# SingleRust/SingleRust

Measured on AMD Instinct MI355X. Metric: cells/sec end-to-end normalise->HVG->50-PC PCA; SpMM achieved HBM GB/s vs peak, higher is better.
Workload: dtype f32

## Files before the change

### include/srx.h

```cpp
#ifndef SRX_H
#define SRX_H

#include <stddef.h>
#include <stdint.h>

#ifdef __cplusplus
extern "C" {
#endif

#define SRX_ABI_VERSION 6

typedef struct srx_ctx srx_ctx;
typedef struct srx_mat srx_mat;

typedef enum srx_status {
    SRX_OK = 0,
    SRX_E_ARG = -1,
    SRX_E_DTYPE = -2,
    SRX_E_FORMAT = -3,
    SRX_E_BOUNDS = -4,
    SRX_E_HIP = -5,
    SRX_E_RCCL = -6,
    SRX_E_OOM = -7,
    SRX_E_NAN = -8,
    SRX_E_SHAPE = -9,
    SRX_E_NOCONV = -10
} srx_status;

typedef enum srx_dtype {
    SRX_I8 = 0, SRX_I16 = 1, SRX_I32 = 2, SRX_U8 = 3, SRX_U16 = 4, SRX_U32 = 5,
    SRX_F32 = 6, SRX_F64 = 7
} srx_dtype;

typedef enum srx_direction { SRX_ROW = 0, SRX_COLUMN = 1 } srx_direction;

typedef struct srx_csr {
    uint64_t n_rows, n_cols, nnz;
    const uint64_t* indptr;
    const uint64_t* indices;
    void* values;
    int32_t dtype;
} srx_csr;

typedef enum srx_store { SRX_STORE_AUTO = 0, SRX_STORE_F32 = 1, SRX_STORE_F64 = 2 } srx_store;

int32_t srx_abi_version(void);
int32_t srx_device_count(int32_t* n_out);
int32_t srx_ctx_create(int32_t device_id, srx_ctx** out);
void    srx_ctx_destroy(srx_ctx* ctx);
int32_t srx_ctx_synchronize(srx_ctx* ctx);
const char* srx_last_error(const srx_ctx* ctx);

#define SRX_UNIQUE_ID_BYTES 128
int32_t srx_comm_unique_id(void* id_out_128);
int32_t srx_comm_init(srx_ctx* ctx, int32_t n_ranks, int32_t rank, const void* id_128);
typedef int32_t (*srx_host_allreduce_fn)(void* user, double* buf, uint64_t count);
int32_t srx_comm_init_host(srx_ctx* ctx, int32_t n_ranks, int32_t rank, srx_host_allreduce_fn fn, void* user);
int32_t srx_comm_destroy(srx_ctx* ctx);
int32_t srx_comm_info(srx_ctx* ctx, int32_t* kind_out, int32_t* n_ranks_out, int32_t* rccl_version_out,
                      int32_t* ranks_seen_out);
int32_t srx_comm_overlap_info(srx_ctx* ctx, int32_t* split_exchanges_out, int32_t* cu_masked_out);
int32_t srx_gram_mode_info(srx_ctx* ctx, int32_t* mode_out);
int32_t srx_gram_exchange_ranges(uint64_t k, uint64_t* offsets_out);
int32_t srx_partition_rows(const uint64_t* indptr, uint64_t n_rows, int32_t n_ranks,
                           uint64_t* cut_out);

int32_t srx_matrix_upload(srx_ctx* ctx, const srx_csr* host, int32_t store, srx_mat** out);
int32_t srx_matrix_upload_csc(srx_ctx* ctx, const srx_csr* host, int32_t store, srx_mat** out);
enum { SRX_FORMAT_CSR = 0, SRX_FORMAT_CSC = 1 };
int32_t srx_matrix_format(const srx_mat* m, int32_t* format_out);
int32_t srx_matrix_to_csr(srx_mat* m, srx_mat** out);
int32_t srx_matrix_to_csc(srx_mat* m, srx_mat** out);
int32_t srx_matrix_alloc(srx_ctx* ctx, uint64_t n_rows, uint64_t n_cols, uint64_t nnz,
                         int32_t dtype, int32_t store, srx_mat** out);
int32_t srx_matrix_device_ptrs(srx_mat* m, void** indptr, void** indices, void** values);
typedef struct srx_mat_info {
    uint64_t n_rows, n_cols, nnz;
    int32_t dtype;
    int32_t store;
    uint64_t row_offset;
    uint64_t n_rows_global;
} srx_mat_info;
int32_t srx_matrix_info(const srx_mat* m, srx_mat_info* out);
int32_t srx_matrix_set_shard(srx_mat* m, uint64_t row_offset);
int32_t srx_matrix_download_values(srx_mat* m, void* values_out, int32_t dtype_out);
int32_t srx_matrix_prepare(srx_mat* m);
int32_t srx_matrix_reserve_results(srx_mat* m, uint64_t n_selected, int32_t n_components);
int32_t srx_matrix_clone(srx_mat* m, srx_mat** out);
int32_t srx_matrix_copy_values(srx_mat* dst, const srx_mat* src);
void    srx_matrix_free(srx_mat* m);

int32_t srx_compute_number(srx_mat* m, int32_t direction, uint32_t* out);
int32_t srx_compute_sum(srx_mat* m, int32_t direction, double* out);
int32_t srx_compute_variance(srx_mat* m, int32_t direction, double* out);
int32_t srx_compute_std_dev(srx_mat* m, int32_t direction, double* out);
int32_t srx_compute_min_max(srx_mat* m, int32_t direction, double* min_out, double* max_out);
int32_t srx_compute_qc_variables(srx_mat* m, uint32_t* num_per_cell, uint32_t* num_per_gene, double* expr_per_gene,
                                 double* expr_per_cell, double* variance_per_gene, double* variance_per_cell,
                                 double* std_dev_per_cell, double* std_dev_per_gene);
int32_t srx_gene_moments(srx_mat* m, uint64_t* cnt, double* sum, double* sumsq);

enum { SRX_FLEX_NONE = 0, SRX_FLEX_ABSOLUTE = 1, SRX_FLEX_RELATIVE = 2 };
typedef struct srx_flex {
    int32_t kind;
    uint32_t absolute;
    double relative;
} srx_flex;
int32_t srx_filter_cells(srx_mat* m, srx_flex lower, srx_flex upper, srx_mat** out, uint8_t* mask_out);
int32_t srx_filter_genes(srx_mat* m, srx_flex lower, srx_flex upper, srx_mat** out, uint8_t* mask_out);
int32_t srx_subset(srx_mat* m, const uint8_t* row_mask, const uint8_t* col_mask, srx_mat** out);
int32_t srx_matrix_download_pattern(srx_mat* m, uint64_t* indptr_out, uint64_t* indices_out);

int32_t srx_normalize_total_inplace(srx_mat* m, double target_sum, int32_t direction);
int32_t srx_log1p_inplace(srx_mat* m);
int32_t srx_normalize_log1p_inplace(srx_mat* m, double target_sum, double* row_sums_out);

int32_t srx_select_hvg(srx_mat* m, uint64_t n, uint64_t* idx_out, uint64_t* n_out);

typedef enum srx_pca_solver {
    SRX_SOLVER_AUTO = 0,
    SRX_SOLVER_GRAM = 1,
    SRX_SOLVER_SPMM = 2
} srx_pca_solver;

typedef struct srx_pca_opts {
    int32_t n_components;
    int32_t center;
    int32_t scale;
    int32_t n_threads;
    int32_t block;
    int32_t max_iter;
    int32_t solver;
    double  tol;
    uint64_t seed;
} srx_pca_opts;

typedef struct srx_pca_info {
    uint64_t n_cells_global;
    uint32_t k;
    uint32_t n_pc;
    uint32_t block;
    uint32_t n_iter;
    double residual;
    uint64_t nnz_selected;
    uint32_t solver;
    uint32_t reserved_;
} srx_pca_info;

int32_t srx_pca(srx_mat* m, const uint64_t* sel, uint64_t k, const srx_pca_opts* opts,
                double* scores, double* components, double* evr, double* mean, double* std_,
                srx_pca_info* info);
int32_t srx_pca_loadings(const double* components, const double* std_, const uint64_t* sel,
                         uint64_t k, uint64_t n_pc, uint64_t n_vars, double* out);

typedef struct srx_pca_model srx_pca_model;
int32_t srx_pca_model_from_result(srx_mat* m, srx_pca_model** out);
int32_t srx_pca_model_create(srx_ctx* ctx, uint64_t k, uint64_t n_pc, const double* components, const double* mean,
                             const double* std_, const uint64_t* sel, int32_t center, int32_t scale, srx_pca_model** out);
int32_t srx_pca_model_info(const srx_pca_model* p, uint64_t* k_out, uint64_t* n_pc_out, uint64_t* sel_out);
void    srx_pca_model_free(srx_pca_model* p);
int32_t srx_pca_transform(srx_pca_model* p, srx_mat* q, const uint64_t* feat, double target_sum, int32_t transform,
                          double* scores_out);

#define SRX_KNN_MAX_DIMS 128
typedef struct srx_knn_opts {
    int32_t k;
    int32_t n_dims;
    int32_t include_self;
    int32_t reserved_;
} srx_knn_opts;
typedef struct srx_knn_info {
    uint64_t n_ref, n_query;
    uint32_t d, k;
    uint32_t n_candidates;
    uint32_t reserved_;
    uint64_t rows_certified;
    uint64_t rows_recomputed;
} srx_knn_info;
int32_t srx_knn_result(srx_mat* m, const srx_knn_opts* opts, uint32_t* indices_out, double* distances_out,
                       srx_knn_info* info);
int32_t srx_knn_points(srx_ctx* ctx, const double* ref, uint64_t n_ref, const double* query, uint64_t n_query,
                       uint64_t d, const srx_knn_opts* opts, uint32_t* indices_out, double* distances_out,
                       srx_knn_info* info);

typedef struct srx_graph srx_graph;
typedef struct srx_graph_info {
    uint64_t n;
    uint32_t k, reserved_;
    uint64_t nnz_distances, nnz_connectivities;
    uint64_t n_mutual;
    uint64_t rows_no_root, rows_clamped, rows_all_zero;
    uint64_t entries_dropped;
    uint64_t max_row_nnz;
} srx_graph_info;
int32_t srx_neighbors_result(srx_mat* m, const srx_knn_opts* opts, srx_knn_info* knn_info, srx_graph** out);
int32_t srx_neighbors_from_knn(srx_ctx* ctx, const uint32_t* indices, const double* distances, uint64_t n, uint32_t k,
                               srx_graph** out);
int32_t srx_graph_info_get(const srx_graph* g, srx_graph_info* info);
enum { SRX_GRAPH_DISTANCES = 0, SRX_GRAPH_CONNECTIVITIES = 1 };
int32_t srx_graph_fetch(srx_graph* g, int32_t which, uint64_t* indptr, uint32_t* indices, double* data);
int32_t srx_graph_fetch_scales(srx_graph* g, double* rho, double* sigma);
void    srx_graph_free(srx_graph* g);

int32_t srx_spmm(srx_mat* m, const uint64_t* sel, uint64_t k, const double* panel, double* y_out,
                 double* t_out, double* gram_out);

typedef struct srx_pipeline_result {
    srx_pca_info pca;
    double ms_normalize, ms_moments, ms_select, ms_compact, ms_pca;
} srx_pipeline_result;
int32_t srx_pipeline(srx_mat* m, double target_sum, uint64_t n_hvg, const srx_pca_opts* opts,
                     srx_pipeline_result* res);
int32_t srx_result_fetch(srx_mat* m, double* scores, double* components, double* evr,
                         double* mean, double* std_, uint64_t* hvg_idx);

typedef struct srx_backed srx_backed;
enum { SRX_BACKED_NORMALIZE = 1, SRX_BACKED_LOG1P = 2 };
int32_t srx_backed_create(srx_ctx* ctx, uint64_t n_cols, int32_t store, srx_backed** out);
void    srx_backed_destroy(srx_backed* b);
int32_t srx_backed_stats_tile(srx_backed* b, const srx_csr* tile, double target_sum, int32_t transform,
                              uint32_t* row_number_out, double* row_sum_out);
int32_t srx_backed_moments(srx_backed* b, uint64_t* cnt, double* sum, double* sumsq, uint64_t* n_rows_global);
int32_t srx_backed_select(srx_backed* b, uint64_t n_hvg, const uint64_t* sel, uint64_t n_sel,
                          const srx_pca_opts* opts, uint64_t* sel_out, uint64_t* n_out);
int32_t srx_backed_gram_tile(srx_backed* b, const srx_csr* tile, double target_sum, int32_t transform);
int32_t srx_backed_solve(srx_backed* b, srx_pca_info* info);
int32_t srx_backed_fetch(srx_backed* b, double* scores, double* components, double* evr, double* mean,
                         double* std_, uint64_t* sel);

typedef enum srx_kernel_class {
    SRX_K_NORMALIZE = 0,
    SRX_K_MOMENTS = 1,
    SRX_K_COMPACT = 2,
    SRX_K_SPMM_FWD = 3,
    SRX_K_SPMM_T = 4,
    SRX_K_GRAM = 5,
    SRX_K_DENSE = 6,
    SRX_K_ROWSUM = 7,
    SRX_K_ITERATE = 8,
    SRX_K_SELECT = 9,
    SRX_K_BUCKET = 10,
    SRX_K_KNN = 11,
    SRX_K_GRAPH = 12,
    SRX_K_COUNT_ = 13
} srx_kernel_class;
int32_t srx_prof_enable(srx_ctx* ctx, uint32_t class_mask);
int32_t srx_prof_reset(srx_ctx* ctx);
int32_t srx_prof_get(srx_ctx* ctx, int32_t kernel_class, double* total_ms, uint64_t* launches,
                     double* algorithmic_bytes);
int32_t srx_prof_get_aux(srx_ctx* ctx, int32_t kernel_class, double* aux_bytes);

#ifdef __cplusplus
}
#endif
#endif
```

### rust/srx_sys.rs

```rust
#![allow(non_camel_case_types, dead_code)]
use std::os::raw::{c_char, c_void};

pub const SRX_ABI_VERSION: i32 = 6;
pub const SRX_UNIQUE_ID_BYTES: usize = 128;
pub const SRX_KNN_MAX_DIMS: i32 = 128;
pub const SRX_OK: i32 = 0;
pub const SRX_E_ARG: i32 = -1;
pub const SRX_E_DTYPE: i32 = -2;
pub const SRX_E_FORMAT: i32 = -3;
pub const SRX_E_BOUNDS: i32 = -4;
pub const SRX_E_HIP: i32 = -5;
pub const SRX_E_RCCL: i32 = -6;
pub const SRX_E_OOM: i32 = -7;
pub const SRX_E_NAN: i32 = -8;
pub const SRX_E_SHAPE: i32 = -9;
pub const SRX_E_NOCONV: i32 = -10;
pub const SRX_I8: i32 = 0;
pub const SRX_I16: i32 = 1;
pub const SRX_I32: i32 = 2;
pub const SRX_U8: i32 = 3;
pub const SRX_U16: i32 = 4;
pub const SRX_U32: i32 = 5;
pub const SRX_F32: i32 = 6;
pub const SRX_F64: i32 = 7;
// ... 101 lines not shown
    pub k: i32,
    pub n_dims: i32,
    pub include_self: i32,
    pub reserved: i32,
}

#[repr(C)]
#[derive(Clone, Copy)]
pub struct SrxKnnInfo {
    pub n_ref: u64,
    pub n_query: u64,
    pub d: u32,
    pub k: u32,
    pub n_candidates: u32,
    pub reserved: u32,
    pub rows_certified: u64,
    pub rows_recomputed: u64,
}

#[repr(C)]
#[derive(Clone, Copy)]
pub struct SrxGraphInfo {
    pub n: u64,
    pub k: u32,
    pub reserved: u32,
    pub nnz_distances: u64,
    pub nnz_connectivities: u64,
    pub n_mutual: u64,
    pub rows_no_root: u64,
    pub rows_clamped: u64,
    pub rows_all_zero: u64,
    pub entries_dropped: u64,
    pub max_row_nnz: u64,
}

#[repr(C)]
#[derive(Clone, Copy)]
pub struct SrxPipelineResult {
    pub pca: SrxPcaInfo,
    pub ms_normalize: f64,
    pub ms_moments: f64,
    pub ms_select: f64,
    pub ms_compact: f64,
    pub ms_pca: f64,
}

pub type SrxHostAllreduceFn = extern "C" fn(user: *mut c_void, buf: *mut f64, count: u64) -> i32;

#[link(name = "srx_hip")]
extern "C" {
    pub fn srx_abi_version() -> i32;
    pub fn srx_device_count(n_out: *mut i32) -> i32;
    pub fn srx_ctx_create(device_id: i32, out: *mut *mut SrxCtx) -> i32;
    pub fn srx_ctx_destroy(ctx: *mut SrxCtx);
    pub fn srx_ctx_synchronize(ctx: *mut SrxCtx) -> i32;
    pub fn srx_last_error(ctx: *const SrxCtx) -> *const c_char;
    pub fn srx_comm_unique_id(id_out_128: *mut c_void) -> i32;
    pub fn srx_comm_init(ctx: *mut SrxCtx, n_ranks: i32, rank: i32, id_128: *const c_void) -> i32;
    pub fn srx_comm_init_host(ctx: *mut SrxCtx, n_ranks: i32, rank: i32, fn_: SrxHostAllreduceFn, user: *mut c_void) -> i32;
    pub fn srx_comm_destroy(ctx: *mut SrxCtx) -> i32;
    pub fn srx_comm_info(ctx: *mut SrxCtx, kind_out: *mut i32, n_ranks_out: *mut i32, rccl_version_out: *mut i32,
                         ranks_seen_out: *mut i32) -> i32;
    pub fn srx_comm_overlap_info(ctx: *mut SrxCtx, split_exchanges_out: *mut i32, cu_masked_out: *mut i32) -> i32;
    pub fn srx_gram_mode_info(ctx: *mut SrxCtx, mode_out: *mut i32) -> i32;
    pub fn srx_gram_exchange_ranges(k: u64, offsets_out: *mut u64) -> i32;
    pub fn srx_partition_rows(indptr: *const u64, n_rows: u64, n_ranks: i32, cut_out: *mut u64) -> i32;
    pub fn srx_matrix_upload(ctx: *mut SrxCtx, host: *const SrxCsr, store: i32, out: *mut *mut SrxMat) -> i32;
    pub fn srx_matrix_upload_csc(ctx: *mut SrxCtx, host: *const SrxCsr, store: i32, out: *mut *mut SrxMat) -> i32;
    pub fn srx_matrix_format(m: *const SrxMat, format_out: *mut i32) -> i32;
    pub fn srx_matrix_to_csr(m: *mut SrxMat, out: *mut *mut SrxMat) -> i32;
    pub fn srx_matrix_to_csc(m: *mut SrxMat, out: *mut *mut SrxMat) -> i32;
    pub fn srx_matrix_alloc(ctx: *mut SrxCtx, n_rows: u64, n_cols: u64, nnz: u64, dtype: i32, store: i32,
                            out: *mut *mut SrxMat) -> i32;
    pub fn srx_matrix_device_ptrs(m: *mut SrxMat, indptr: *mut *mut c_void, indices: *mut *mut c_void,
                                  values: *mut *mut c_void) -> i32;
    pub fn srx_matrix_info(m: *const SrxMat, out: *mut SrxMatInfo) -> i32;
    pub fn srx_matrix_set_shard(m: *mut SrxMat, row_offset: u64) -> i32;
    pub fn srx_matrix_download_values(m: *mut SrxMat, values_out: *mut c_void, dtype_out: i32) -> i32;
    pub fn srx_matrix_prepare(m: *mut SrxMat) -> i32;
    pub fn srx_matrix_reserve_results(m: *mut SrxMat, n_selected: u64, n_components: i32) -> i32;
    pub fn srx_matrix_clone(m: *mut SrxMat, out: *mut *mut SrxMat) -> i32;
    pub fn srx_matrix_copy_values(dst: *mut SrxMat, src: *const SrxMat) -> i32;
    pub fn srx_matrix_free(m: *mut SrxMat);
    pub fn srx_compute_number(m: *mut SrxMat, direction: i32, out: *mut u32) -> i32;
    pub fn srx_compute_sum(m: *mut SrxMat, direction: i32, out: *mut f64) -> i32;
    pub fn srx_compute_variance(m: *mut SrxMat, direction: i32, out: *mut f64) -> i32;
    pub fn srx_compute_std_dev(m: *mut SrxMat, direction: i32, out: *mut f64) -> i32;
    pub fn srx_compute_min_max(m: *mut SrxMat, direction: i32, min_out: *mut f64, max_out: *mut f64) -> i32;
    pub fn srx_compute_qc_variables(m: *mut SrxMat, num_per_cell: *mut u32, num_per_gene: *mut u32,
                                    expr_per_gene: *mut f64, expr_per_cell: *mut f64, variance_per_gene: *mut f64,
                                    variance_per_cell: *mut f64, std_dev_per_cell: *mut f64,
                                    std_dev_per_gene: *mut f64) -> i32;
    pub fn srx_gene_moments(m: *mut SrxMat, cnt: *mut u64, sum: *mut f64, sumsq: *mut f64) -> i32;
    pub fn srx_filter_cells(m: *mut SrxMat, lower: SrxFlex, upper: SrxFlex, out: *mut *mut SrxMat, mask_out: *mut u8) -> i32;
    pub fn srx_filter_genes(m: *mut SrxMat, lower: SrxFlex, upper: SrxFlex, out: *mut *mut SrxMat, mask_out: *mut u8) -> i32;
    pub fn srx_subset(m: *mut SrxMat, row_mask: *const u8, col_mask: *const u8, out: *mut *mut SrxMat) -> i32;
    pub fn srx_matrix_download_pattern(m: *mut SrxMat, indptr_out: *mut u64, indices_out: *mut u64) -> i32;
    pub fn srx_normalize_total_inplace(m: *mut SrxMat, target_sum: f64, direction: i32) -> i32;
    pub fn srx_log1p_inplace(m: *mut SrxMat) -> i32;
    pub fn srx_normalize_log1p_inplace(m: *mut SrxMat, target_sum: f64, row_sums_out: *mut f64) -> i32;
    pub fn srx_select_hvg(m: *mut SrxMat, n: u64, idx_out: *mut u64, n_out: *mut u64) -> i32;
    pub fn srx_pca(m: *mut SrxMat, sel: *const u64, k: u64, opts: *const SrxPcaOpts, scores: *mut f64,
                   components: *mut f64, evr: *mut f64, mean: *mut f64, std: *mut f64, info: *mut SrxPcaInfo) -> i32;
    pub fn srx_pca_loadings(components: *const f64, std: *const f64, sel: *const u64, k: u64, n_pc: u64,
                            n_vars: u64, out: *mut f64) -> i32;
    pub fn srx_pca_model_from_result(m: *mut SrxMat, out: *mut *mut SrxPcaModel) -> i32;
    pub fn srx_pca_model_create(ctx: *mut SrxCtx, k: u64, n_pc: u64, components: *const f64, mean: *const f64,
                                std: *const f64, sel: *const u64, center: i32, scale: i32,
                                out: *mut *mut SrxPcaModel) -> i32;
    pub fn srx_pca_model_info(p: *const SrxPcaModel, k_out: *mut u64, n_pc_out: *mut u64, sel_out: *mut u64) -> i32;
    pub fn srx_pca_model_free(p: *mut SrxPcaModel);
    pub fn srx_pca_transform(p: *mut SrxPcaModel, q: *mut SrxMat, feat: *const u64, target_sum: f64,
                             transform: i32, scores_out: *mut f64) -> i32;
    pub fn srx_knn_result(m: *mut SrxMat, opts: *const SrxKnnOpts, indices_out: *mut u32, distances_out: *mut f64,
                          info: *mut SrxKnnInfo) -> i32;
    pub fn srx_knn_points(ctx: *mut SrxCtx, ref_: *const f64, n_ref: u64, query: *const f64, n_query: u64, d: u64,
                          opts: *const SrxKnnOpts, indices_out: *mut u32, distances_out: *mut f64,
                          info: *mut SrxKnnInfo) -> i32;
    pub fn srx_neighbors_result(m: *mut SrxMat, opts: *const SrxKnnOpts, knn_info: *mut SrxKnnInfo,
                                out: *mut *mut SrxGraph) -> i32;
    pub fn srx_neighbors_from_knn(ctx: *mut SrxCtx, indices: *const u32, distances: *const f64, n: u64, k: u32,
                                  out: *mut *mut SrxGraph) -> i32;
    pub fn srx_graph_info_get(g: *const SrxGraph, info: *mut SrxGraphInfo) -> i32;
    pub fn srx_graph_fetch(g: *mut SrxGraph, which: i32, indptr: *mut u64, indices: *mut u32, data: *mut f64) -> i32;
    pub fn srx_graph_fetch_scales(g: *mut SrxGraph, rho: *mut f64, sigma: *mut f64) -> i32;
    pub fn srx_graph_free(g: *mut SrxGraph);
    pub fn srx_spmm(m: *mut SrxMat, sel: *const u64, k: u64, panel: *const f64, y_out: *mut f64, t_out: *mut f64,
                    gram_out: *mut f64) -> i32;
    pub fn srx_pipeline(m: *mut SrxMat, target_sum: f64, n_hvg: u64, opts: *const SrxPcaOpts,
                        res: *mut SrxPipelineResult) -> i32;
    pub fn srx_result_fetch(m: *mut SrxMat, scores: *mut f64, components: *mut f64, evr: *mut f64, mean: *mut f64,
                            std: *mut f64, hvg_idx: *mut u64) -> i32;
    pub fn srx_backed_create(ctx: *mut SrxCtx, n_cols: u64, store: i32, out: *mut *mut SrxBacked) -> i32;
    pub fn srx_backed_destroy(b: *mut SrxBacked);
    pub fn srx_backed_stats_tile(b: *mut SrxBacked, tile: *const SrxCsr, target_sum: f64, transform: i32,
                                 row_number_out: *mut u32, row_sum_out: *mut f64) -> i32;
    pub fn srx_backed_moments(b: *mut SrxBacked, cnt: *mut u64, sum: *mut f64, sumsq: *mut f64,
                              n_rows_global: *mut u64) -> i32;
    pub fn srx_backed_select(b: *mut SrxBacked, n_hvg: u64, sel: *const u64, n_sel: u64, opts: *const SrxPcaOpts,
                             sel_out: *mut u64, n_out: *mut u64) -> i32;
    pub fn srx_backed_gram_tile(b: *mut SrxBacked, tile: *const SrxCsr, target_sum: f64, transform: i32) -> i32;
    pub fn srx_backed_solve(b: *mut SrxBacked, info: *mut SrxPcaInfo) -> i32;
    pub fn srx_backed_fetch(b: *mut SrxBacked, scores: *mut f64, components: *mut f64, evr: *mut f64,
                            mean: *mut f64, std: *mut f64, sel: *mut u64) -> i32;
    pub fn srx_prof_enable(ctx: *mut SrxCtx, class_mask: u32) -> i32;
    pub fn srx_prof_reset(ctx: *mut SrxCtx) -> i32;
    pub fn srx_prof_get(ctx: *mut SrxCtx, kernel_class: i32, total_ms: *mut f64, launches: *mut u64,
                        algorithmic_bytes: *mut f64) -> i32;
    pub fn srx_prof_get_aux(ctx: *mut SrxCtx, kernel_class: i32, aux_bytes: *mut f64) -> i32;
}
```

### singlerust_amd/_ffi.py

```python
from __future__ import annotations

import ctypes as C
import os

_HERE = os.path.dirname(os.path.abspath(__file__))
LIB_PATH = os.path.join(_HERE, "lib", "libsrx_hip.so")

OK, E_ARG, E_DTYPE, E_FORMAT, E_BOUNDS, E_HIP, E_RCCL, E_OOM, E_NAN, E_SHAPE, E_NOCONV = (
    0, -1, -2, -3, -4, -5, -6, -7, -8, -9, -10)
STATUS_NAMES = {0: "SRX_OK", -1: "SRX_E_ARG", -2: "SRX_E_DTYPE", -3: "SRX_E_FORMAT",
                -4: "SRX_E_BOUNDS", -5: "SRX_E_HIP", -6: "SRX_E_RCCL", -7: "SRX_E_OOM",
                -8: "SRX_E_NAN", -9: "SRX_E_SHAPE", -10: "SRX_E_NOCONV"}
I8, I16, I32, U8, U16, U32, F32, F64 = range(8)
ROW, COLUMN = 0, 1
STORE_AUTO, STORE_F32, STORE_F64 = 0, 1, 2
K_NORMALIZE, K_MOMENTS, K_COMPACT, K_SPMM_FWD, K_SPMM_T, K_GRAM, K_DENSE, K_ROWSUM, K_ITERATE, K_SELECT, K_BUCKET = range(11)
K_KNN = 11
K_GRAPH = 12
GRAPH_DISTANCES, GRAPH_CONNECTIVITIES = 0, 1
KNN_MAX_DIMS = 128
SOLVER_AUTO, SOLVER_GRAM, SOLVER_SPMM = 0, 1, 2
UNIQUE_ID_BYTES = 128


# ... 47 lines not shown
    _fields_ = [("n", C.c_uint64), ("k", C.c_uint32), ("reserved_", C.c_uint32), ("nnz_distances", C.c_uint64),
                ("nnz_connectivities", C.c_uint64), ("n_mutual", C.c_uint64), ("rows_no_root", C.c_uint64),
                ("rows_clamped", C.c_uint64), ("rows_all_zero", C.c_uint64), ("entries_dropped", C.c_uint64),
                ("max_row_nnz", C.c_uint64)]


class SynthParams(C.Structure):
    _fields_ = [("seed", C.c_uint64), ("n_rows_global", C.c_uint64), ("n_cols", C.c_uint64),
                ("density", C.c_double), ("lib_sigma", C.c_double), ("type_decay", C.c_double),
                ("n_types", C.c_uint32), ("marker_genes", C.c_uint32), ("expr_boost", C.c_uint32),
                ("value_boost", C.c_uint32), ("skew", C.c_uint32), ("reserved_", C.c_uint32)]


class Flex(C.Structure):
    _fields_ = [("kind", C.c_int32), ("absolute", C.c_uint32), ("relative", C.c_double)]


HOST_ALLREDUCE_FN = C.CFUNCTYPE(C.c_int32, C.c_void_p, C.POINTER(C.c_double), C.c_uint64)
FLEX_NONE, FLEX_ABSOLUTE, FLEX_RELATIVE = 0, 1, 2
BACKED_NORMALIZE, BACKED_LOG1P = 1, 2
P = C.c_void_p
_SIGS = {
    "srx_abi_version": (C.c_int32, []),
    "srx_device_count": (C.c_int32, [C.POINTER(C.c_int32)]),
    "srx_ctx_create": (C.c_int32, [C.c_int32, C.POINTER(P)]),
    "srx_ctx_destroy": (None, [P]),
    "srx_ctx_synchronize": (C.c_int32, [P]),
    "srx_last_error": (C.c_char_p, [P]),
    "srx_comm_unique_id": (C.c_int32, [P]),
    "srx_comm_init": (C.c_int32, [P, C.c_int32, C.c_int32, P]),
    "srx_comm_init_host": (C.c_int32, [P, C.c_int32, C.c_int32, C.c_void_p, P]),
    "srx_comm_destroy": (C.c_int32, [P]),
    "srx_comm_info": (C.c_int32, [P, C.POINTER(C.c_int32), C.POINTER(C.c_int32), C.POINTER(C.c_int32), C.POINTER(C.c_int32)]),
    "srx_comm_overlap_info": (C.c_int32, [P, C.POINTER(C.c_int32), C.POINTER(C.c_int32)]),
    "srx_gram_mode_info": (C.c_int32, [P, C.POINTER(C.c_int32)]),
    "srx_gram_exchange_ranges": (C.c_int32, [C.c_uint64, P]),
    "srx_partition_rows": (C.c_int32, [P, C.c_uint64, C.c_int32, P]),
    "srx_matrix_upload": (C.c_int32, [P, C.POINTER(Csr), C.c_int32, C.POINTER(P)]),
    "srx_matrix_upload_csc": (C.c_int32, [P, C.POINTER(Csr), C.c_int32, C.POINTER(P)]),
    "srx_matrix_format": (C.c_int32, [P, C.POINTER(C.c_int32)]),
    "srx_matrix_to_csr": (C.c_int32, [P, C.POINTER(P)]),
    "srx_matrix_to_csc": (C.c_int32, [P, C.POINTER(P)]),
    "srx_matrix_alloc": (C.c_int32, [P, C.c_uint64, C.c_uint64, C.c_uint64, C.c_int32, C.c_int32, C.POINTER(P)]),
    "srx_matrix_device_ptrs": (C.c_int32, [P, C.POINTER(P), C.POINTER(P), C.POINTER(P)]),
    "srx_matrix_info": (C.c_int32, [P, C.POINTER(MatInfo)]),
    "srx_matrix_set_shard": (C.c_int32, [P, C.c_uint64]),
    "srx_matrix_download_values": (C.c_int32, [P, P, C.c_int32]),
    "srx_matrix_prepare": (C.c_int32, [P]),
    "srx_matrix_reserve_results": (C.c_int32, [P, C.c_uint64, C.c_int32]),
    "srx_matrix_clone": (C.c_int32, [P, C.POINTER(P)]),
    "srx_matrix_copy_values": (C.c_int32, [P, P]),
    "srx_matrix_free": (None, [P]),
    "srx_compute_number": (C.c_int32, [P, C.c_int32, P]),
    "srx_compute_sum": (C.c_int32, [P, C.c_int32, P]),
    "srx_compute_variance": (C.c_int32, [P, C.c_int32, P]),
    "srx_compute_std_dev": (C.c_int32, [P, C.c_int32, P]),
    "srx_compute_min_max": (C.c_int32, [P, C.c_int32, P, P]),
    "srx_compute_qc_variables": (C.c_int32, [P, P, P, P, P, P, P, P, P]),
    "srx_filter_cells": (C.c_int32, [P, Flex, Flex, C.POINTER(C.c_void_p), P]),
    "srx_filter_genes": (C.c_int32, [P, Flex, Flex, C.POINTER(C.c_void_p), P]),
    "srx_subset": (C.c_int32, [P, P, P, C.POINTER(C.c_void_p)]),
    "srx_matrix_download_pattern": (C.c_int32, [P, P, P]),
    "srx_gene_moments": (C.c_int32, [P, P, P, P]),
    "srx_normalize_total_inplace": (C.c_int32, [P, C.c_double, C.c_int32]),
    "srx_log1p_inplace": (C.c_int32, [P]),
    "srx_normalize_log1p_inplace": (C.c_int32, [P, C.c_double, P]),
    "srx_select_hvg": (C.c_int32, [P, C.c_uint64, P, C.POINTER(C.c_uint64)]),
    "srx_pca": (C.c_int32, [P, P, C.c_uint64, C.POINTER(PcaOpts), P, P, P, P, P, C.POINTER(PcaInfo)]),
    "srx_pca_loadings": (C.c_int32, [P, P, P, C.c_uint64, C.c_uint64, C.c_uint64, P]),
    "srx_pca_model_from_result": (C.c_int32, [P, C.POINTER(P)]),
    "srx_pca_model_create": (C.c_int32, [P, C.c_uint64, C.c_uint64, P, P, P, P, C.c_int32, C.c_int32, C.POINTER(P)]),
    "srx_pca_model_info": (C.c_int32, [P, C.POINTER(C.c_uint64), C.POINTER(C.c_uint64), P]),
    "srx_pca_model_free": (None, [P]),
    "srx_pca_transform": (C.c_int32, [P, P, P, C.c_double, C.c_int32, P]),
    "srx_knn_result": (C.c_int32, [P, C.POINTER(KnnOpts), P, P, C.POINTER(KnnInfo)]),
    "srx_knn_points": (C.c_int32, [P, P, C.c_uint64, P, C.c_uint64, C.c_uint64, C.POINTER(KnnOpts), P, P, C.POINTER(KnnInfo)]),
    "srx_neighbors_result": (C.c_int32, [P, C.POINTER(KnnOpts), C.POINTER(KnnInfo), C.POINTER(P)]),
    "srx_neighbors_from_knn": (C.c_int32, [P, P, P, C.c_uint64, C.c_uint32, C.POINTER(P)]),
    "srx_graph_info_get": (C.c_int32, [P, C.POINTER(GraphInfo)]),
    "srx_graph_fetch": (C.c_int32, [P, C.c_int32, P, P, P]),
    "srx_graph_fetch_scales": (C.c_int32, [P, P, P]),
    "srx_graph_free": (None, [P]),
    "srx_spmm": (C.c_int32, [P, P, C.c_uint64, P, P, P, P]),
    "srx_pipeline": (C.c_int32, [P, C.c_double, C.c_uint64, C.POINTER(PcaOpts), C.POINTER(PipelineResult)]),
    "srx_result_fetch": (C.c_int32, [P, P, P, P, P, P, P]),
    "srx_backed_create": (C.c_int32, [P, C.c_uint64, C.c_int32, C.POINTER(P)]),
    "srx_backed_destroy": (None, [P]),
    "srx_backed_stats_tile": (C.c_int32, [P, C.POINTER(Csr), C.c_double, C.c_int32, P, P]),
    "srx_backed_moments": (C.c_int32, [P, P, P, P, C.POINTER(C.c_uint64)]),
    "srx_backed_select": (C.c_int32, [P, C.c_uint64, P, C.c_uint64, C.POINTER(PcaOpts), P, C.POINTER(C.c_uint64)]),
    "srx_backed_gram_tile": (C.c_int32, [P, C.POINTER(Csr), C.c_double, C.c_int32]),
    "srx_backed_solve": (C.c_int32, [P, C.POINTER(PcaInfo)]),
    "srx_backed_fetch": (C.c_int32, [P, P, P, P, P, P, P]),
    "srx_prof_enable": (C.c_int32, [P, C.c_uint32]),
    "srx_prof_reset": (C.c_int32, [P]),
    "srx_prof_get": (C.c_int32, [P, C.c_int32, C.POINTER(C.c_double), C.POINTER(C.c_uint64), C.POINTER(C.c_double)]),
    "srx_prof_get_aux": (C.c_int32, [P, C.c_int32, C.POINTER(C.c_double)]),
    "srx_synth_defaults": (None, [C.POINTER(SynthParams), C.c_uint64, C.c_uint64, C.c_uint64, C.c_double]),
    "srx_synth_indptr": (C.c_int32, [C.POINTER(SynthParams), C.c_uint64, C.c_uint64, P]),
    "srx_synth_fill_host": (C.c_int32, [C.POINTER(SynthParams), C.c_uint64, C.c_uint64, P, P, P]),
    "srx_synth_generate": (C.c_int32, [P, C.POINTER(SynthParams), C.c_uint64, C.c_uint64, C.c_int32, C.c_int32, C.POINTER(P)]),
}
EXPORTS = tuple(_SIGS)

_lib = None


def lib() -> C.CDLL:
    global _lib
    if _lib is None:
        if not os.path.exists(LIB_PATH):
            raise SrxError(E_HIP, f"{LIB_PATH} is missing: run `python -m singlerust_amd.build` "
                                  "(hipcc --offload-arch=gfx950); there is no CPU fallback")
        l = C.CDLL(LIB_PATH)
        for name, (res, args) in _SIGS.items():
            fn = getattr(l, name)
            fn.restype = res
            fn.argtypes = args
        _lib = l
    return _lib


def check(rc: int, ctx=None) -> None:
    if rc != OK:
        msg = lib().srx_last_error(ctx)
        raise SrxError(rc, msg.decode() if msg else "")


def ptr(a):
    return None if a is None else C.c_void_p(a.ctypes.data)
```

### singlerust_amd/csrc/common.hpp

```cpp
#pragma once

#include <hip/hip_runtime.h>

#include <cstdarg>
#include <cstdint>
#include <cstdio>
#include <cstring>
#include <map>
#include <string>
#include <utility>
#include <vector>

#include "../../include/srx.h"

struct ncclComm;

namespace srx {

constexpr int kWave = 64;

__device__ __forceinline__ int lane_id() { return threadIdx.x & (kWave - 1); }
__device__ __forceinline__ uint64_t global_wave_id() {
    return (uint64_t)blockIdx.x * (blockDim.x / kWave) + (uint32_t)__builtin_amdgcn_readfirstlane((int)(threadIdx.x / kWave));
}

template <typename T>
__device__ __forceinline__ T wave_sum(T v) {
#pragma unroll
    for (int off = kWave / 2; off > 0; off >>= 1) v += __shfl_xor(v, off, kWave);
    return v;
}
__device__ __forceinline__ void wave_lds_sync() {
    __builtin_amdgcn_fence(__ATOMIC_ACQ_REL, "wavefront");
    __builtin_amdgcn_wave_barrier();
}
template <typename T>
__device__ __forceinline__ T wave_min(T v) {
#pragma unroll
    for (int off = kWave / 2; off > 0; off >>= 1) {
        T o = __shfl_xor(v, off, kWave);
        v = o < v ? o : v;
    }
    return v;
}
template <typename T>
__device__ __forceinline__ T wave_max(T v) {
#pragma unroll
    for (int off = kWave / 2; off > 0; off >>= 1) {
        T o = __shfl_xor(v, off, kWave);
        v = o > v ? o : v;
    }
    return v;
}

struct ProfAcc {
    double ms = 0.0;
    uint64_t launches = 0;
    double bytes = 0.0, aux_bytes = 0.0;
    std::vector<std::pair<hipEvent_t, hipEvent_t>> pending;
};

}

struct srx_ctx {
    int device = 0;
    int n_cus = 256;
    hipStream_t stream = nullptr;
    hipStream_t comm_stream = nullptr;
    hipEvent_t comm_fork = nullptr, comm_join = nullptr;
    hipStream_t gram_stream = nullptr;
    bool gram_stream_masked = false;
    uint32_t* d_gram_mode = nullptr;
    int gram_mode_state = 0;
    bool gram_mode_f32 = false;
    uint32_t gram_splits = 0;
    hipEvent_t gram_fork = nullptr, gram_join = nullptr;
    std::string err;
    ncclComm* comm = nullptr;
    int n_ranks = 1, rank = 0;
    srx_host_allreduce_fn host_allreduce = nullptr;
    void* host_allreduce_user = nullptr;
    uint32_t prof_mask = 0;
    srx::ProfAcc prof[SRX_K_COUNT_];
    std::vector<hipEvent_t> event_pool;
    struct Scratch { void* p = nullptr; size_t bytes = 0; };
    std::map<std::string, Scratch> scratch;
    int pool_on = 0;
    std::vector<std::pair<void*, size_t>> pool;
    void* pinned = nullptr;
    size_t pinned_bytes = 0;
    static constexpr int kAsyncSlots = 4;
    std::map<std::string, hipGraphExec_t> graphs;
    bool graphs_off = false;
    bool capturing = false;
    double* pin_async = nullptr;
    struct UpWorker {
        hipStream_t stream = nullptr;
        void* pin[2] = {nullptr, nullptr};
        hipEvent_t ev[2] = {nullptr, nullptr};
    };
    std::vector<UpWorker> up_workers;
    hipStream_t direct_stream = nullptr;
    hipEvent_t async_ev[kAsyncSlots] = {nullptr, nullptr, nullptr, nullptr};
    hipEvent_t d2h_ev = nullptr;
    void* pin_d2h = nullptr;
    bool d2h_pending = false;
};

struct srx_pca_state {
    bool valid = false;
    uint32_t k = 0, n_pc = 0;
    int center = 1, scale = 1;
    std::vector<int> round_counts;
    double* d_scores = nullptr;
    size_t scores_cap = 0;
    std::vector<double> components;
    std::vector<double> evr, mean, std_;
    std::vector<uint64_t> sel;
    srx_pca_info info{};
    double* d_small = nullptr;
    bool host_pending = false;
};

struct srx_mat {
    srx_ctx* ctx = nullptr;
    uint64_t n_rows = 0, n_cols = 0, nnz = 0;
    int32_t dtype = SRX_F32;
    int32_t store = SRX_STORE_F32;
    bool pooled = false;
    bool store_auto = false;
    int64_t* d_indptr = nullptr;
    int32_t* d_indices = nullptr;
    void* d_values = nullptr;
    uint64_t row_offset = 0;
    int n_tiles = 0;
    int tile_genes = 0;
    int64_t* d_tile_ptr = nullptr;
    uint16_t* d_idx16 = nullptr;
    uint32_t* d_cnt_pat = nullptr;
    bool cnt_pat_valid = false;
    uint64_t version = 1;
    uint64_t moments_version = 0;
    uint64_t* d_cnt = nullptr;
    double* d_sum = nullptr;
    double* d_sq = nullptr;
    uint64_t n_rows_global = 0;
    double* d_row_sum = nullptr;
    bool csc = false;
    srx_pca_state pca;
};

namespace srx {

extern thread_local std::string g_tls_err;

inline int32_t fail(srx_ctx* ctx, int32_t code, const char* fmt, ...) {
    char buf[512];
    va_list ap;
    va_start(ap, fmt);
    vsnprintf(buf, sizeof buf, fmt, ap);
    va_end(ap);
    g_tls_err = buf;
    if (ctx) ctx->err = buf;
    return code;
}

#define SRX_HIP(ctx, expr)                                                                   \
    do {                                                                                     \
        hipError_t e__ = (expr);                                                             \
        if (e__ != hipSuccess)                                                               \
            return srx::fail((ctx), e__ == hipErrorOutOfMemory ? SRX_E_OOM : SRX_E_HIP,      \
                             "%s failed: %s (%s:%d)", #expr, hipGetErrorString(e__),         \
                             __FILE__, __LINE__);                                            \
    } while (0)

#define SRX_TRY(expr)                          \
    do {                                       \
        int32_t rc__ = (expr);                 \
        if (rc__ != SRX_OK) return rc__;       \
    } while (0)

int32_t scratch(srx_ctx* ctx, const char* name, size_t bytes, void** out);
int32_t pinned(srx_ctx* ctx, size_t bytes, void** out);
int32_t d2h(srx_ctx* ctx, void* host, const void* dev, size_t bytes);
int32_t d2h_begin(srx_ctx* ctx, const void* dev, size_t bytes);
int32_t d2h_end(srx_ctx* ctx, void* host, size_t bytes);
int32_t h2d(srx_ctx* ctx, void* dev, const void* host, size_t bytes);
int32_t d2h_rows(srx_ctx* ctx, void* host, const void* dev, uint64_t rows, size_t width, size_t dev_pitch);

struct ProfScope {
    srx_ctx* ctx;
    int cls;
    hipStream_t stream;
    hipEvent_t e0 = nullptr, e1 = nullptr;
    ProfScope(srx_ctx* c, int cls_, double alg_bytes, hipStream_t stream_ = nullptr, double aux_bytes = 0.0);
    ~ProfScope();
};

struct Range {
    bool on;
    explicit Range(const char* name);
    ~Range();
};

int32_t allreduce_f64(srx_ctx* ctx, double* d_buf, size_t count);
int32_t allreduce_f64_on(srx_ctx* ctx, double* d_buf, size_t count, hipStream_t stream);
bool comm_is_rccl(const srx_ctx* ctx);

struct RowXf {
    const double* row_sum = nullptr;
    double target = 0.0;
    bool write_back = false;
};
int32_t upload_on(srx_ctx* ctx, const srx_csr* h, int32_t store, hipStream_t stream, srx_mat** out);
int32_t tiles_from_idx16(srx_mat* m, hipStream_t stream);
inline uint64_t at_least_one(uint64_t n) { return n ? n : 1; }
hipError_t dev_malloc(srx_ctx* ctx, void** p, size_t bytes);
void pool_clear(srx_ctx* ctx);
int32_t ensure_tiles(srx_mat* m);
int32_t promote_to_f64(srx_mat* m);
int32_t ensure_pattern_counts(srx_mat* m);
int32_t ensure_moments(srx_mat* m);
int32_t moments_accumulate(srx_mat* m, double* d_acc, RowXf xf);
int32_t moments_install(srx_mat* m, double* d_packed);
int32_t ensure_moments_xf(srx_mat* m, RowXf xf, bool* stored);
void moments_adopt(srx_mat* m);
void moments_retire(srx_mat* m);
int32_t launch_row_apply(srx_mat* m, double target, hipStream_t stream);
int32_t launch_normalize(srx_mat* m, double target, bool do_norm, bool do_log, hipStream_t stream = nullptr,
                         bool precise = false, int wgs_per_cu = 0);
int32_t launch_row_sums(srx_mat* m, double* out = nullptr);
int32_t row_number(srx_mat* m, uint32_t* out);
int32_t row_stat(srx_mat* m, int which, double* out0, double* out1);
int32_t row_qc(srx_mat* m, uint32_t* num, double* sum, double* var);
int32_t scan_exclusive(srx_ctx* ctx, const int64_t* d_in, uint64_t n, int64_t* d_out, int64_t** total_dev);
inline void touch(srx_mat* m) { m->version++; m->pca.valid = false; }

inline bool is_f32(const srx_mat* m) { return m->store == SRX_STORE_F32; }
inline int32_t eff_dir(const srx_mat* m, int32_t d) { return (m->csc && (d == SRX_ROW || d == SRX_COLUMN)) ? 1 - d : d; }
int32_t transpose_device(srx_mat* m, srx_mat** out);
inline size_t val_bytes(const srx_mat* m) { return is_f32(m) ? 4 : 8; }

}
```

### singlerust_amd/csrc/ctx.hip

```cpp
#include "common.hpp"
#include <chrono>

#include <dlfcn.h>

#include <algorithm>
#include <thread>

namespace srx {

thread_local std::string g_tls_err;

int32_t scratch(srx_ctx* ctx, const char* name, size_t bytes, void** out) {
    auto& s = ctx->scratch[name];
    if (s.bytes < bytes) {
        if (s.p) SRX_HIP(ctx, hipFree(s.p));
        s.p = nullptr;
        s.bytes = 0;
        size_t want = bytes + bytes / 8 + 256;
        SRX_HIP(ctx, hipMalloc(&s.p, want));
        s.bytes = want;
    }
    *out = s.p;
    return SRX_OK;
}
// ... 185 lines not shown
        if (lo > hi || lo < 0 || (uint64_t)hi > nnz) { bad = true; continue; }
        for (int64_t p = lo + lane; p + 1 < hi; p += kWave) bad |= !(idx[p] < idx[p + 1]);
    }
    if (bad) atomicOr(flag, 2);
}

static int grid_for(uint64_t n, int block, int cap) {
    uint64_t g = (n + block - 1) / block;
    if (g < 1) g = 1;
    if (g > (uint64_t)cap) g = cap;
    return (int)g;
}

template <typename S>
static int32_t convert_chunked(srx_ctx* ctx, hipStream_t stream, const char* tmp_tag, const void* host, void* d_dst,
                               uint64_t n, bool to_f32) {
    const uint64_t chunk = 32ull << 20;
    void* d_tmp;
    SRX_TRY(scratch(ctx, tmp_tag, (n < chunk ? n : chunk) * sizeof(S) + 16, &d_tmp));
    for (uint64_t off = 0; off < n; off += chunk) {
        uint64_t cnt = n - off < chunk ? n - off : chunk;
        SRX_HIP(ctx, hipMemcpy(d_tmp, (const S*)host + off, cnt * sizeof(S), hipMemcpyHostToDevice));
        int g = grid_for(cnt, 256, 4096);
        if (to_f32)
            hipLaunchKernelGGL((k_convert_values<S, float>), dim3(g), dim3(256), 0, stream,
                               (const S*)d_tmp, (float*)d_dst + off, cnt);
        else
            hipLaunchKernelGGL((k_convert_values<S, double>), dim3(g), dim3(256), 0, stream,
                               (const S*)d_tmp, (double*)d_dst + off, cnt);
        SRX_HIP(ctx, hipStreamSynchronize(stream));
    }
    return SRX_OK;
}

constexpr size_t kPoolCapBytes = 24ull << 30;
static size_t pool_bytes(const srx_ctx* ctx) {
    size_t t = 0;
    for (auto& b : ctx->pool) t += b.second;
    return t;
}
hipError_t dev_malloc(srx_ctx* ctx, void** p, size_t bytes) {
    if (ctx->pool_on) {
        int best = -1;
        for (size_t i = 0; i < ctx->pool.size(); ++i) {
            const size_t cap = ctx->pool[i].second;
            if (cap >= bytes && cap <= bytes + bytes / 4 + (1u << 20) && (best < 0 || cap < ctx->pool[(size_t)best].second)) best = (int)i;
        }
        if (best >= 0) {
            *p = ctx->pool[(size_t)best].first;
            ctx->pool.erase(ctx->pool.begin() + best);
            return hipSuccess;
        }
    }
    const size_t want = (ctx->pool_on && bytes >= (1u << 20)) ? bytes + bytes / 32 + 65536 : bytes;
    hipError_t e = hipMalloc(p, want);
    if (e != hipSuccess && !ctx->pool.empty()) {
        (void)hipGetLastError();
        pool_clear(ctx);
        e = hipMalloc(p, want);
    }
    return e;
}
static void dev_release(srx_mat* m, void* p) {
    if (!p) return;
    srx_ctx* ctx = m->ctx;
    size_t cap = 0;
    if (m->pooled && ctx && ctx->pool_on > 0 && hipMemPtrGetInfo(p, &cap) == hipSuccess && cap > 0) {
        ctx->pool.emplace_back(p, cap);
        while (ctx->pool.size() > 1 && pool_bytes(ctx) > kPoolCapBytes) {
            (void)hipFree(ctx->pool.front().first);
            ctx->pool.erase(ctx->pool.begin());
        }
    } else {
        (void)hipFree(p);
    }
}
void pool_clear(srx_ctx* ctx) {
    for (auto& b : ctx->pool) (void)hipFree(b.first);
    ctx->pool.clear();
}

static void free_mat_buffers(srx_mat* m) {
    if (!m) return;
    dev_release(m, m->d_indptr);
    dev_release(m, m->d_indices);
    dev_release(m, m->d_values);
    dev_release(m, m->d_tile_ptr);
    dev_release(m, m->d_idx16);
    dev_release(m, m->d_cnt);
    dev_release(m, m->d_cnt_pat);
    dev_release(m, m->d_sum);
    dev_release(m, m->d_sq);
    dev_release(m, m->d_row_sum);
    (void)hipFree(m->pca.d_scores);
}

static int32_t resolve_store(int32_t dtype, int32_t store) {
    if (store == SRX_STORE_F32 || store == SRX_STORE_F64) return store;
    switch (dtype) {
        case SRX_I32: case SRX_U32: case SRX_F64: return SRX_STORE_F64;
        default: return SRX_STORE_F32;
    }
}


__global__ void k_rebase_indptr(int64_t* __restrict__ indptr, uint64_t n, int64_t base) {
    uint64_t i = (uint64_t)blockIdx.x * blockDim.x + threadIdx.x;
    if (i < n) indptr[i] -= base;
}

static const int kUpWorkers = [] {
    const char* e = getenv("SRX_UP_WORKERS");
    const int v = e ? atoi(e) : 8;
    return v < 1 ? 1 : v > 64 ? 64 : v;
}();
constexpr size_t kUpChunkBytes = 4u << 20;

static int32_t ensure_up_workers(srx_ctx* ctx) {
    if (!ctx->up_workers.empty()) return SRX_OK;
    std::vector<srx_ctx::UpWorker> ws(kUpWorkers);
    for (auto& w : ws) {
        SRX_HIP(ctx, hipStreamCreateWithFlags(&w.stream, hipStreamNonBlocking));
        for (int b = 0; b < 2; ++b) {
            SRX_HIP(ctx, hipHostMalloc(&w.pin[b], kUpChunkBytes, hipHostMallocDefault));
            SRX_HIP(ctx, hipEventCreateWithFlags(&w.ev[b], hipEventDisableTiming));
        }
    }
    ctx->up_workers = std::move(ws);
    return SRX_OK;
}

static int32_t parallel_h2d(srx_ctx* ctx, const void* src, void* dst, uint64_t n, bool narrow, size_t elem_bytes,
                            uint64_t n_cols, bool* bad) {
    if (n == 0) return SRX_OK;
    SRX_TRY(ensure_up_workers(ctx));
    const int device = ctx->device;
    const uint64_t per_chunk = kUpChunkBytes / elem_bytes;
    int nw = (int)std::min<uint64_t>(kUpWorkers, (n + per_chunk - 1) / per_chunk);
    if (nw < 1) nw = 1;
    const uint64_t share = ((n + nw - 1) / nw + 15) & ~(uint64_t)15;
    std::vector<hipError_t> err(nw, hipSuccess);
    std::vector<int> oob(nw, 0);
    auto run = [&](int t) {
        srx_ctx::UpWorker& w = ctx->up_workers[t];
        hipError_t e = hipSetDevice(device);
        const uint64_t e0 = std::min<uint64_t>(n, (uint64_t)t * share), e1 = std::min<uint64_t>(n, e0 + share);
        int buf = 0;
        bool used[2] = {false, false};
        int bad_local = 0;
        for (uint64_t off = e0; off < e1 && e == hipSuccess; off += per_chunk, buf ^= 1) {
            const uint64_t cnt = std::min<uint64_t>(per_chunk, e1 - off);
            if (used[buf]) e = hipEventSynchronize(w.ev[buf]);
            if (e != hipSuccess) break;
            if (narrow && elem_bytes == sizeof(uint16_t)) {
                const uint64_t* s = static_cast<const uint64_t*>(src) + off;
                uint16_t* d = static_cast<uint16_t*>(w.pin[buf]);
                uint64_t over = 0;
                for (uint64_t i = 0; i < cnt; ++i) {
                    const uint64_t v = s[i];
                    over |= (uint64_t)(v >= n_cols);
                    d[i] = (uint16_t)v;
                }
                bad_local |= (int)over;
            } else if (narrow) {
                const uint64_t* s = static_cast<const uint64_t*>(src) + off;
                int32_t* d = static_cast<int32_t*>(w.pin[buf]);
// ... 589 lines not shown
```

### singlerust_amd/csrc/genes.hip

```cpp
#include "pca_internal.hpp"
#include "log1p64.hpp"

#include <algorithm>
#include <cmath>

namespace srx {

constexpr int kMaxTileGenes = 10000;
constexpr int kMomThreads = 1024;

__device__ __forceinline__ int32_t entry_column(int32_t c) { return c; }
template <typename T>
__device__ __forceinline__ int32_t entry_column(const GramPk<T>& e) { return e.j; }
template <typename E>
__global__ void k_tile_ptr(const int64_t* __restrict__ indptr, const E* __restrict__ idx,
                           uint64_t n_rows, int n_tiles, int tile_genes, int64_t* __restrict__ tp) {
    uint64_t i = (uint64_t)blockIdx.x * blockDim.x + threadIdx.x;
    uint64_t total = (uint64_t)(n_tiles - 1) * n_rows;
    uint64_t stride = (uint64_t)gridDim.x * blockDim.x;
    for (; i < total; i += stride) {
        uint64_t t = i / n_rows + 1, r = i % n_rows;
        int32_t bound = (int32_t)(t * (uint64_t)tile_genes);
        int64_t lo = indptr[r], hi = indptr[r + 1];
        while (lo < hi) {
// ... 247 lines not shown

template <typename I>
__global__ __launch_bounds__(kMomThreads) void k_gene_count(const int64_t* __restrict__ indptr, const int64_t* __restrict__ tp,
                                                            const I* __restrict__ idx, uint64_t n_rows, uint64_t n_cols, int n_tiles,
                                                            int tile_genes, uint64_t rows_per_block, uint32_t* __restrict__ cnt) {
    extern __shared__ double lds[];
    uint32_t* s_cnt = reinterpret_cast<uint32_t*>(lds);
    for (int g = threadIdx.x; g < tile_genes; g += kMomThreads) s_cnt[g] = 0u;
    __syncthreads();
    const int tile = blockIdx.x % n_tiles;
    const uint64_t rb = blockIdx.x / n_tiles;
    const int32_t gbase = tile * tile_genes;
    const uint64_t r0 = rb * rows_per_block;
    const uint64_t r1 = r0 + rows_per_block < n_rows ? r0 + rows_per_block : n_rows;
    const int lane = lane_id();
    const int wave = __builtin_amdgcn_readfirstlane(threadIdx.x / kWave);
    constexpr int kWaves = kMomThreads / kWave;
    constexpr int kU = 2, kR = 4;
    auto load4 = [&](int64_t e0, int32_t (&g)[4]) {
        if constexpr (sizeof(I) == 4) {
            const int4 g4 = *reinterpret_cast<const int4*>(idx + e0);
            g[0] = g4.x; g[1] = g4.y; g[2] = g4.z; g[3] = g4.w;
        } else {
            const uint2 g2 = *reinterpret_cast<const uint2*>(idx + e0);
            g[0] = (int)(g2.x & 0xffffu); g[1] = (int)(g2.x >> 16);
            g[2] = (int)(g2.y & 0xffffu); g[3] = (int)(g2.y >> 16);
        }
    };
    auto add4 = [&](int64_t e0, int64_t lo, int64_t hi, const int32_t (&g)[4]) {
#pragma unroll
        for (int j = 0; j < 4; ++j)
            if (e0 + j >= lo && e0 + j < hi)
                __hip_atomic_fetch_add(&s_cnt[g[j] - gbase], 1u, __ATOMIC_RELAXED, __HIP_MEMORY_SCOPE_WORKGROUP);
    };
    for (uint64_t rb4 = r0 + wave; rb4 < r1; rb4 += (uint64_t)kWaves * kR) {
        int64_t lo[kR], hi[kR];
#pragma unroll
        for (int q = 0; q < kR; ++q) {
            const uint64_t r = rb4 + (uint64_t)q * kWaves;
            lo[q] = hi[q] = 0;
            if (r < r1) seg_bounds(indptr, tp, n_rows, n_tiles, tile, r, lo[q], hi[q]);
        }
        int32_t g[kR][kU][4];
#pragma unroll
        for (int q = 0; q < kR; ++q)
#pragma unroll
            for (int u = 0; u < kU; ++u) {
                const int64_t b0 = lo[q] & ~(int64_t)3, e0 = b0 + 4 * (u * kWave + lane);
                load4(e0 < hi[q] ? e0 : b0, g[q][u]);
            }
#pragma unroll
        for (int q = 0; q < kR; ++q) {
            const int64_t b0 = lo[q] & ~(int64_t)3;
#pragma unroll
            for (int u = 0; u < kU; ++u) {
                const int64_t e0 = b0 + 4 * (u * kWave + lane);
                if (e0 < hi[q]) add4(e0, lo[q], hi[q], g[q][u]);
            }
            for (int64_t e0 = b0 + 4 * (kU * kWave + lane); e0 < hi[q]; e0 += 4 * kWave) {
                int32_t gt[4];
                load4(e0, gt);
                add4(e0, lo[q], hi[q], gt);
            }
        }
    }
    __syncthreads();
    for (int g = threadIdx.x; g < tile_genes; g += kMomThreads) {
        const uint64_t gene = (uint64_t)gbase + g;
        if (gene < n_cols) cnt[rb * n_cols + gene] = s_cnt[g];
    }
}
__global__ void k_gene_count_reduce(const uint32_t* __restrict__ part, uint64_t n_cols, uint64_t n_blocks, uint32_t* __restrict__ cnt) {
    const uint64_t j = (uint64_t)blockIdx.x * blockDim.x + threadIdx.x;
    if (j >= n_cols) return;
    uint32_t c = 0;
    for (uint64_t b = 0; b < n_blocks; ++b) c += part[b * n_cols + j];
    cnt[j] = c;
}

constexpr int kRedSlices = 8;
__global__ __launch_bounds__(64 * kRedSlices) void k_moments_reduce(
    const double* __restrict__ part_sum, const double* __restrict__ part_sq, uint64_t n_cols, uint64_t n_blocks, uint64_t n_rows,
    const uint32_t* __restrict__ cnt, double inv_fx_sum, double inv_fx_sq, const uint32_t* __restrict__ poison,
    double* __restrict__ packed) {
    __shared__ unsigned long long red[2][kRedSlices][64];
    const int lane = threadIdx.x & 63, slice = threadIdx.x >> 6;
    const uint64_t j = (uint64_t)blockIdx.x * 64 + lane;
    if (blockIdx.x == 0 && threadIdx.x == 0) packed[3 * n_cols] = (double)n_rows;
    const bool live = j < n_cols;
    double s = 0.0, q = 0.0;
    if (inv_fx_sum != 0.0) {
        unsigned long long is = 0, iq = 0;
        if (live) {
            uint64_t b = slice;
            for (; b + 3 * kRedSlices < n_blocks; b += 4 * kRedSlices) {
                unsigned long long xs[4], xq[4];
#pragma unroll
                for (int u = 0; u < 4; ++u) {
                    xs[u] = (unsigned long long)__double_as_longlong(part_sum[(b + u * kRedSlices) * n_cols + j]);
                    xq[u] = (unsigned long long)__double_as_longlong(part_sq[(b + u * kRedSlices) * n_cols + j]);
                }
#pragma unroll
                for (int u = 0; u < 4; ++u) {
                    is += xs[u];
                    iq += xq[u];
                }
            }
            for (; b < n_blocks; b += kRedSlices) {
                is += (unsigned long long)__double_as_longlong(part_sum[b * n_cols + j]);
                iq += (unsigned long long)__double_as_longlong(part_sq[b * n_cols + j]);
            }
        }
        red[0][slice][lane] = is;
        red[1][slice][lane] = iq;
        __syncthreads();
        if (slice != 0 || !live) return;
#pragma unroll
        for (int u = 1; u < kRedSlices; ++u) {
            is += red[0][u][lane];
            iq += red[1][u][lane];
        }
        const unsigned long long cn = (unsigned long long)cnt[j];
        const unsigned long long magic_bits = (unsigned long long)__double_as_longlong(6755399441055744.0);
        s = (double)(long long)(is - cn * magic_bits) * inv_fx_sum;
        q = (double)(long long)(iq - cn * magic_bits) * inv_fx_sq;
        if (poison[j]) s = q = __builtin_nan("");
    } else {
        if (slice != 0 || !live) return;
        for (uint64_t b = 0; b < n_blocks; ++b) {
            s += part_sum[b * n_cols + j];
            q += part_sq[b * n_cols + j];
        }
    }
    packed[j] = (double)cnt[j];
    packed[n_cols + j] = s;
    packed[2 * n_cols + j] = q;
}

__global__ void k_moments_unpack(const double* __restrict__ packed, uint64_t n_cols, uint64_t* __restrict__ cnt,
                                 double* __restrict__ sum, double* __restrict__ sq) {
    uint64_t j = (uint64_t)blockIdx.x * blockDim.x + threadIdx.x;
    if (j >= n_cols) return;
    cnt[j] = (uint64_t)packed[j];
    sum[j] = packed[n_cols + j];
    sq[j] = packed[2 * n_cols + j];
}

__device__ __host__ __forceinline__ uint64_t f64_key(double x) {
    uint64_t b;
    memcpy(&b, &x, 8);
    return (b >> 63) ? ~b : (b | 0x8000000000000000ull);
}
__device__ __host__ __forceinline__ double key_f64(uint64_t k) {
    uint64_t b = (k >> 63) ? (k & 0x7fffffffffffffffull) : ~k;
    double x;
    memcpy(&x, &b, 8);
    return x;
}

template <typename T>
__global__ __launch_bounds__(kMomThreads) void k_gene_minmax(
    const int64_t* __restrict__ indptr, const int64_t* __restrict__ tp, const int32_t* __restrict__ idx,
    const T* __restrict__ vals, uint64_t n_rows, uint64_t n_cols, int n_tiles, int tile_genes,
    uint64_t rows_per_block, unsigned long long* __restrict__ g_min, unsigned long long* __restrict__ g_max) {
    extern __shared__ double lds[];
    unsigned long long* s_min = reinterpret_cast<unsigned long long*>(lds);
    unsigned long long* s_max = s_min + tile_genes;
    const unsigned long long kInf = f64_key(INFINITY), kNinf = f64_key(-INFINITY);
    for (int g = threadIdx.x; g < tile_genes; g += kMomThreads) { s_min[g] = kInf; s_max[g] = kNinf; }
    __syncthreads();
    const int tile = blockIdx.x % n_tiles;
    const uint64_t rb = blockIdx.x / n_tiles;
    const int32_t gbase = tile * tile_genes;
    const uint64_t r0 = rb * rows_per_block;
    const uint64_t r1 = r0 + rows_per_block < n_rows ? r0 + rows_per_block : n_rows;
    const int lane = lane_id();
    const int wave = __builtin_amdgcn_readfirstlane(threadIdx.x / kWave);
    constexpr int kWaves = kMomThreads / kWave;
    for (uint64_t r = r0 + wave; r < r1; r += kWaves) {
        int64_t lo, hi;
        seg_bounds(indptr, tp, n_rows, n_tiles, tile, r, lo, hi);
        for (int64_t p = lo + lane; p < hi; p += kWave) {
            double x = (double)vals[p];
            if (x != x) continue;
            int32_t g = idx[p] - gbase;
            unsigned long long k = f64_key(x);
            atomicMin(&s_min[g], k);
            atomicMax(&s_max[g], k);
        }
    }
    __syncthreads();
    for (int g = threadIdx.x; g < tile_genes; g += kMomThreads) {
        uint64_t gene = (uint64_t)gbase + g;
        if (gene < n_cols) {
            if (s_min[g] != kInf) atomicMin(&g_min[gene], s_min[g]);
            if (s_max[g] != kNinf) atomicMax(&g_max[gene], s_max[g]);
        }
    }
}

__global__ void k_fill_u64(unsigned long long* p, uint64_t n, unsigned long long v) {
    uint64_t i = (uint64_t)blockIdx.x * blockDim.x + threadIdx.x;
    if (i < n) p[i] = v;
}

template <typename T>
__global__ void k_col_scale(const int32_t* __restrict__ idx, T* __restrict__ vals, uint64_t nnz,
                            const double* __restrict__ sum, double target) {
    uint64_t i = (uint64_t)blockIdx.x * blockDim.x + threadIdx.x;
    uint64_t stride = (uint64_t)gridDim.x * blockDim.x;
    for (; i < nnz; i += stride) {
        double s = sum[idx[i]];
        double sc = s == 0.0 ? 0.0 : target / s;
        vals[i] = (T)((double)vals[i] * sc);
    }
}

static void tile_geometry(const srx_mat* m, int& n_tiles, int& tile_genes) {
    const uint64_t G = at_least_one(m->n_cols);
// ... 92 lines not shown
        }
        return SRX_OK;
    };
    int32_t rc;
    switch (nt - 1) {
        case 0: rc = go(std::integral_constant<int, 0>{}); break;
        case 1: rc = go(std::integral_constant<int, 1>{}); break;
        case 2: rc = go(std::integral_constant<int, 2>{}); break;
        case 3: rc = go(std::integral_constant<int, 3>{}); break;
        case 4: rc = go(std::integral_constant<int, 4>{}); break;
        case 5: rc = go(std::integral_constant<int, 5>{}); break;
        case 6: rc = go(std::integral_constant<int, 6>{}); break;
        case 7: rc = go(std::integral_constant<int, 7>{}); break;
        default: rc = go(std::integral_constant<int, 8>{}); break;
    }
    SRX_TRY(rc);
    if (count) {
        hipLaunchKernelGGL(k_gene_count_reduce, dim3((unsigned)((m->n_cols + 255) / 256)), dim3(256), 0, stream, (const uint32_t*)part, m->n_cols,
                           (uint64_t)g, m->d_cnt_pat);
        m->cnt_pat_valid = true;
    }
    SRX_HIP(ctx, hipGetLastError());
    return SRX_OK;
}

int32_t tiles_from_idx16(srx_mat* m, hipStream_t stream) {
    srx_ctx* ctx = m->ctx;
    int nt, tg;
    tile_geometry(m, nt, tg);
    if (nt > 9 || !m->d_idx16 || m->d_tile_ptr) return fail(ctx, SRX_E_ARG, "tiles_from_idx16: %d gene tiles", nt);
    if (m->n_rows == 0) return SRX_OK;
    if (nt > 1) SRX_HIP(ctx, dev_malloc(ctx, (void**)&m->d_tile_ptr, (size_t)(nt - 1) * m->n_rows * sizeof(int64_t)));
    SRX_TRY(launch_narrow16_tiles<true>(m, nt, tg, stream));
    m->n_tiles = nt;
    m->tile_genes = tg;
    return SRX_OK;
}

int32_t ensure_tiles(srx_mat* m) {
    srx_ctx* ctx = m->ctx;
    if (m->n_tiles) return SRX_OK;
    int nt, tg;
    tile_geometry(m, nt, tg);
    if (nt > 1) SRX_HIP(ctx, dev_malloc(ctx, (void**)&m->d_tile_ptr, (size_t)(nt - 1) * at_least_one(m->n_rows) * sizeof(int64_t)));
    if (m->n_rows > 0 && m->n_cols <= 65536) {
        SRX_HIP(ctx, dev_malloc(ctx, (void**)&m->d_idx16, (m->nnz + 16) * sizeof(uint16_t)));
        SRX_TRY(launch_narrow16_tiles<false>(m, nt, tg, ctx->stream));
    } else if (m->n_rows > 0) {
        SRX_TRY(launch_tile_ptr(ctx, m->d_indptr, m->d_indices, m->n_rows, nt, tg, m->d_tile_ptr));
    }
    m->n_tiles = nt;
    m->tile_genes = tg;
    return SRX_OK;
}

static int32_t block_geometry(const srx_mat* m, uint64_t& n_blocks, uint64_t& rows_per_block) {
    uint64_t want = (uint64_t)(4 * m->ctx->n_cus) / (uint64_t)m->n_tiles;
    if (want < 1) want = 1;
    uint64_t by_rows = (m->n_rows + 63) / 64;
    if (by_rows < 1) by_rows = 1;
    n_blocks = want < by_rows ? want : by_rows;
    rows_per_block = (m->n_rows + n_blocks - 1) / n_blocks;
    if (rows_per_block < 1) rows_per_block = 1;
    const uint64_t cap = std::max<uint64_t>(1, 0x7fffffffull / std::max<uint64_t>(m->n_cols, 1));
    if (rows_per_block > cap) {
        rows_per_block = cap;
        n_blocks = (m->n_rows + rows_per_block - 1) / rows_per_block;
        if ((double)n_blocks * (double)std::max<uint64_t>(m->n_cols, 1) * 16.0 > 8.0 * 1024 * 1024 * 1024)
            return fail(m->ctx, SRX_E_ARG, "gene statistics: %llu columns x %llu row blocks exceed the partial-sum budget (matrix too wide)",
                        (unsigned long long)m->n_cols, (unsigned long long)n_blocks);
    }
    return SRX_OK;
}

template <typename F>
static int32_t by_values(const srx_mat* m, F&& f) {
    return is_f32(m) ? f((float*)m->d_values) : f((double*)m->d_values);
}
template <typename F>
static int32_t by_indices(const srx_mat* m, F&& f) {
    return m->d_idx16 ? f((const uint16_t*)m->d_idx16) : f((const int32_t*)m->d_indices);
}

static int32_t local_moments(srx_mat* m, double** packed_out, RowXf xf = RowXf{}) {
    srx_ctx* ctx = m->ctx;
    SRX_TRY(ensure_tiles(m));
    const uint64_t G = m->n_cols;
    uint64_t nb, rpb;
    SRX_TRY(block_geometry(m, nb, rpb));
    double *p_sum, *p_sq, *packed;
    SRX_TRY(scratch(ctx, "mom_part_sum", nb * at_least_one(G) * sizeof(double), (void**)&p_sum));
    SRX_TRY(scratch(ctx, "mom_part_sq", nb * at_least_one(G) * sizeof(double), (void**)&p_sq));
    SRX_TRY(scratch(ctx, "mom_packed", (3 * G + 1) * sizeof(double), (void**)&packed));
    SRX_TRY(ensure_pattern_counts(m));
    const size_t lds = (size_t)m->tile_genes * 16 + (xf.row_sum ? (size_t)kLog1pTabBytes : 0);
    const double bytes = (double)m->nnz * ((m->n_cols <= 65536 ? 2.0 : 4.0) + val_bytes(m)) + (double)(m->n_rows + 1) * 8.0 +
                         (double)G * 24.0 + (xf.row_sum ? (double)m->n_rows * 8.0 : 0.0) +
                         (xf.write_back ? (double)m->nnz * val_bytes(m) : 0.0);
    double fx_sum = 0.0, fx_sq = 0.0;
    if (xf.row_sum) {
        int lg = 0;
        while ((1ull << lg) < at_least_one(m->n_rows)) ++lg;
        fx_sum = std::ldexp(1.0, std::min(62 - 6 - lg, 44));
        fx_sq = std::ldexp(1.0, std::min(62 - 12 - lg, 38));
    }
    uint32_t* d_poison = nullptr;
    if (xf.row_sum) {
        SRX_TRY(scratch(ctx, "mom_poison", at_least_one(G) * sizeof(uint32_t), (void**)&d_poison));
        SRX_HIP(ctx, hipMemsetAsync(d_poison, 0, at_least_one(G) * sizeof(uint32_t), ctx->stream));
    }
    {
        ProfScope ps(ctx, SRX_K_MOMENTS, bytes);
        dim3 grid((unsigned)(nb * m->n_tiles));
        auto launch = [&](auto kern, const auto* idxp, auto* valp) -> int32_t {
            SRX_HIP(ctx, hipFuncSetAttribute((const void*)kern, hipFuncAttributeMaxDynamicSharedMemorySize, (int)lds));
            hipLaunchKernelGGL(kern, grid, dim3(kMomThreads), lds, ctx->stream, m->d_indptr, m->d_tile_ptr, idxp, valp,
                               m->n_rows, G, m->n_tiles, m->tile_genes, rpb, xf.row_sum, xf.target, fx_sum, fx_sq, d_poison, p_sum, p_sq);
            return SRX_OK;
        };
        SRX_TRY(by_values(m, [&](auto* vals) {
            return by_indices(m, [&](const auto* idx) {
                using T = std::remove_pointer_t<decltype(vals)>;
                using I = std::remove_cv_t<std::remove_pointer_t<decltype(idx)>>;
                if (xf.row_sum && xf.write_back) return launch(k_gene_moments<T, I, true, true>, idx, vals);
                if (xf.row_sum) return launch(k_gene_moments<T, I, true>, idx, (const T*)vals);
                return launch(k_gene_moments<T, I, false>, idx, (const T*)vals);
            });
        }));
        hipLaunchKernelGGL(k_moments_reduce, dim3((unsigned)at_least_one((G + 63) / 64)), dim3(64 * kRedSlices), 0, ctx->stream, p_sum, p_sq, G, nb,
                           m->n_rows, (const uint32_t*)m->d_cnt_pat, fx_sum != 0.0 ? 1.0 / fx_sum : 0.0,
                           fx_sq != 0.0 ? 1.0 / fx_sq : 0.0, (const uint32_t*)d_poison, packed);
    }
    SRX_HIP(ctx, hipGetLastError());
    *packed_out = packed;
    return SRX_OK;
}

int32_t ensure_pattern_counts(srx_mat* m) {
    if (m->cnt_pat_valid && m->d_cnt_pat) return SRX_OK;
    srx_ctx* ctx = m->ctx;
    SRX_TRY(ensure_tiles(m));
    const uint64_t G = m->n_cols;
    if (!m->d_cnt_pat) SRX_HIP(ctx, dev_malloc(ctx, (void**)&m->d_cnt_pat, at_least_one(G) * sizeof(uint32_t)));
    SRX_HIP(ctx, hipMemsetAsync(m->d_cnt_pat, 0, at_least_one(G) * sizeof(uint32_t), ctx->stream));
    if (m->n_rows && m->nnz) {
        uint64_t nb, rpb;
        SRX_TRY(block_geometry(m, nb, rpb));
        uint32_t* part;
        SRX_TRY(scratch(ctx, "mom_part_cnt", nb * G * sizeof(uint32_t), (void**)&part));
        const dim3 grid((unsigned)(nb * m->n_tiles));
        const size_t lds = (size_t)m->tile_genes * 4;
        ProfScope ps(ctx, SRX_K_MOMENTS, (double)m->nnz * (m->d_idx16 ? 2.0 : 4.0) + (double)(m->n_rows + 1) * 8.0 + (double)G * 4.0);
        by_indices(m, [&](const auto* idx) {
            using I = std::remove_cv_t<std::remove_pointer_t<decltype(idx)>>;
            hipLaunchKernelGGL(k_gene_count<I>, grid, dim3(kMomThreads), lds, ctx->stream, m->d_indptr, m->d_tile_ptr, idx, m->n_rows, G,
                               m->n_tiles, m->tile_genes, rpb, part);
            return SRX_OK;
        });
        hipLaunchKernelGGL(k_gene_count_reduce, dim3((unsigned)((G + 255) / 256)), dim3(256), 0, ctx->stream, (const uint32_t*)part, G, nb,
                           m->d_cnt_pat);
        SRX_HIP(ctx, hipGetLastError());
    }
    m->cnt_pat_valid = true;
    return SRX_OK;
}

__global__ void k_add_f64(double* __restrict__ acc, const double* __restrict__ x, uint64_t n) {
    uint64_t i = (uint64_t)blockIdx.x * blockDim.x + threadIdx.x;
    if (i < n) acc[i] += x[i];
}

int32_t moments_accumulate(srx_mat* m, double* d_acc, RowXf xf) {
    srx_ctx* ctx = m->ctx;
    SRX_HIP(ctx, hipSetDevice(ctx->device));
    double* packed;
    SRX_TRY(local_moments(m, &packed, xf));
    const uint64_t n = 3 * m->n_cols + 1;
    hipLaunchKernelGGL(k_add_f64, dim3((unsigned)((n + 255) / 256)), dim3(256), 0, ctx->stream, d_acc, packed, n);
    SRX_HIP(ctx, hipGetLastError());
    return SRX_OK;
}

static int32_t alloc_moments(srx_mat* m) {
    srx_ctx* ctx = m->ctx;
    SRX_HIP(ctx, hipSetDevice(ctx->device));
    const uint64_t G = at_least_one(m->n_cols);
    if (!m->d_cnt) {
        SRX_HIP(ctx, hipMalloc((void**)&m->d_cnt, G * sizeof(uint64_t)));
        SRX_HIP(ctx, hipMalloc((void**)&m->d_sum, G * sizeof(double)));
        SRX_HIP(ctx, hipMalloc((void**)&m->d_sq, G * sizeof(double)));
    }
    return SRX_OK;
}

static int32_t reduce_unpack_moments(srx_mat* m, double* d_packed, bool n_is_local) {
    srx_ctx* ctx = m->ctx;
    const uint64_t G = m->n_cols;
    SRX_TRY(allreduce_f64(ctx, d_packed, 3 * G + 1));
    hipLaunchKernelGGL(k_moments_unpack, dim3((unsigned)((G + 255) / 256 + 1)), dim3(256), 0, ctx->stream, d_packed, G,
                       m->d_cnt, m->d_sum, m->d_sq);
    SRX_HIP(ctx, hipGetLastError());
    if (n_is_local && !ctx->comm && !ctx->host_allreduce) {
        m->n_rows_global = m->n_rows;
    } else {
        double ng = 0.0;
        SRX_TRY(d2h(ctx, &ng, d_packed + 3 * G, sizeof(double)));
        m->n_rows_global = (uint64_t)ng;
    }
    return SRX_OK;
}

void moments_adopt(srx_mat* m) { m->moments_version = m->version; }
void moments_retire(srx_mat* m) { m->moments_version = 0; }

int32_t moments_install(srx_mat* m, double* d_packed) {
    SRX_TRY(alloc_moments(m));
    SRX_TRY(reduce_unpack_moments(m, d_packed, false));
    moments_adopt(m);
    return SRX_OK;
}

int32_t ensure_moments(srx_mat* m) {
    if (m->moments_version == m->version) return SRX_OK;
    SRX_TRY(alloc_moments(m));
    double* packed;
    SRX_TRY(local_moments(m, &packed));
    SRX_TRY(reduce_unpack_moments(m, packed, true));
    moments_adopt(m);
    return SRX_OK;
}

int32_t ensure_moments_xf(srx_mat* m, RowXf xf, bool* stored) {
    *stored = false;
    SRX_TRY(alloc_moments(m));
    double* packed;
    SRX_TRY(local_moments(m, &packed, xf));
    if (xf.write_back) {
        m->dtype = SRX_F64;
        touch(m);
        *stored = true;
    }
    return reduce_unpack_moments(m, packed, true);
}

static int32_t fetch_moments(srx_mat* m, uint64_t* cnt, double* sum, double* sq) {
    SRX_TRY(ensure_moments(m));
    const uint64_t G = m->n_cols;
    if (cnt) SRX_TRY(d2h(m->ctx, cnt, m->d_cnt, G * sizeof(uint64_t)));
    if (sum) SRX_TRY(d2h(m->ctx, sum, m->d_sum, G * sizeof(double)));
    if (sq) SRX_TRY(d2h(m->ctx, sq, m->d_sq, G * sizeof(double)));
    return SRX_OK;
}

#pragma clang fp contract(off)
void finalize_variance(const uint64_t* cnt, const double* sum, const double* sq, uint64_t G, double* out) {
    for (uint64_t j = 0; j < G; ++j) {
        out[j] = 0.0;
        if (cnt[j] > 0) {
            double c = (double)(uint32_t)cnt[j];
            double mean = sum[j] / c;
            out[j] = sq[j] / c - mean * mean;
        }
    }
}

int32_t gene_variances(srx_mat* m, std::vector<double>& var) {
    const uint64_t G = m->n_cols;
    std::vector<uint64_t> cnt(G);
    std::vector<double> sum(G), sq(G);
    SRX_TRY(fetch_moments(m, cnt.data(), sum.data(), sq.data()));
    var.resize(G);
    finalize_variance(cnt.data(), sum.data(), sq.data(), G, var.data());
    return SRX_OK;
}

}

using namespace srx;

extern "C" {

int32_t srx_gene_moments(srx_mat* m, uint64_t* cnt, double* sum, double* sumsq) {
    if (!m) return fail(nullptr, SRX_E_ARG, "null matrix");
    if (m->csc) return fail(m->ctx, SRX_E_FORMAT, "srx_gene_moments walks cells: convert the CSC matrix with srx_matrix_to_csr");
    return fetch_moments(m, cnt, sum, sumsq);
}

int32_t srx_compute_number(srx_mat* m, int32_t direction, uint32_t* out) {
    if (!m || !out) return fail(m ? m->ctx : nullptr, SRX_E_ARG, "null argument");
    SRX_HIP(m->ctx, hipSetDevice(m->ctx->device));
    direction = eff_dir(m, direction);
    if (direction == SRX_ROW) return row_number(m, out);
    if (direction != SRX_COLUMN) return fail(m->ctx, SRX_E_ARG, "bad direction %d", direction);
    std::vector<uint64_t> cnt(m->n_cols);
    SRX_TRY(fetch_moments(m, cnt.data(), nullptr, nullptr));
    for (uint64_t j = 0; j < m->n_cols; ++j) out[j] = (uint32_t)cnt[j];
    return SRX_OK;
}

int32_t srx_compute_sum(srx_mat* m, int32_t direction, double* out) {
    if (!m || !out) return fail(m ? m->ctx : nullptr, SRX_E_ARG, "null argument");
    SRX_HIP(m->ctx, hipSetDevice(m->ctx->device));
    direction = eff_dir(m, direction);
    if (direction == SRX_ROW) return row_stat(m, 0, out, nullptr);
    if (direction != SRX_COLUMN) return fail(m->ctx, SRX_E_ARG, "bad direction %d", direction);
    return fetch_moments(m, nullptr, out, nullptr);
}

int32_t srx_compute_variance(srx_mat* m, int32_t direction, double* out) {
    if (!m || !out) return fail(m ? m->ctx : nullptr, SRX_E_ARG, "null argument");
    SRX_HIP(m->ctx, hipSetDevice(m->ctx->device));
    direction = eff_dir(m, direction);
    if (direction == SRX_ROW) return row_stat(m, 1, out, nullptr);
    if (direction != SRX_COLUMN) return fail(m->ctx, SRX_E_ARG, "bad direction %d", direction);
    std::vector<double> var;
    SRX_TRY(gene_variances(m, var));
    memcpy(out, var.data(), var.size() * sizeof(double));
    return SRX_OK;
}

int32_t srx_compute_std_dev(srx_mat* m, int32_t direction, double* out) {
    SRX_TRY(srx_compute_variance(m, direction, out));
    uint64_t n = eff_dir(m, direction) == SRX_ROW ? m->n_rows : m->n_cols;
    for (uint64_t i = 0; i < n; ++i) out[i] = std::sqrt(out[i]);
    return SRX_OK;
}

int32_t srx_compute_qc_variables(srx_mat* m, uint32_t* num_per_cell, uint32_t* num_per_gene, double* expr_per_gene,
                                 double* expr_per_cell, double* variance_per_gene, double* variance_per_cell,
                                 double* std_dev_per_cell, double* std_dev_per_gene) {
    if (!m) return fail(nullptr, SRX_E_ARG, "null matrix");
    srx_ctx* ctx = m->ctx;
    SRX_HIP(ctx, hipSetDevice(ctx->device));
    if (m->csc) {
        std::swap(num_per_cell, num_per_gene);
        std::swap(expr_per_cell, expr_per_gene);
        std::swap(variance_per_cell, variance_per_gene);
        std::swap(std_dev_per_cell, std_dev_per_gene);
    }
    if (num_per_cell || expr_per_cell || variance_per_cell || std_dev_per_cell) {
        std::vector<double> var;
        double* vp = variance_per_cell;
        if (!vp && std_dev_per_cell) { var.resize(m->n_rows); vp = var.data(); }
        SRX_TRY(row_qc(m, num_per_cell, expr_per_cell, vp));
        if (std_dev_per_cell)
            for (uint64_t i = 0; i < m->n_rows; ++i) std_dev_per_cell[i] = std::sqrt(vp[i]);
    }
    if (num_per_gene || expr_per_gene || variance_per_gene || std_dev_per_gene) {
        const uint64_t G = m->n_cols;
        std::vector<uint64_t> cnt(G);
        std::vector<double> sum(G), sq(G);
        SRX_TRY(fetch_moments(m, cnt.data(), sum.data(), sq.data()));
        if (num_per_gene) for (uint64_t j = 0; j < G; ++j) num_per_gene[j] = (uint32_t)cnt[j];
        if (expr_per_gene) memcpy(expr_per_gene, sum.data(), G * sizeof(double));
        if (variance_per_gene || std_dev_per_gene) {
            std::vector<double> var(G);
            finalize_variance(cnt.data(), sum.data(), sq.data(), G, var.data());
            if (variance_per_gene) memcpy(variance_per_gene, var.data(), G * sizeof(double));
            if (std_dev_per_gene) for (uint64_t j = 0; j < G; ++j) std_dev_per_gene[j] = std::sqrt(var[j]);
        }
    }
    return SRX_OK;
}

int32_t srx_compute_min_max(srx_mat* m, int32_t direction, double* mn, double* mx) {
    if (!m || !mn || !mx) return fail(m ? m->ctx : nullptr, SRX_E_ARG, "null argument");
    srx_ctx* ctx = m->ctx;
    SRX_HIP(ctx, hipSetDevice(ctx->device));
// ... 56 lines not shown
```

### singlerust_amd/csrc/pca_form.hip

```cpp
#include "pca_internal.hpp"
#include "log1p64.hpp"

namespace srx {

#include "compact.inl"

#include "gram.inl"

static void gram_stripes_of(int k, GramPlan& g) {
    g.k = k;
    int sr = 8;
    while (sr > 1 && (size_t)sr * (size_t)(k + sr) * 8 > 65536) sr >>= 1;
    g.sr_shift = sr == 8 ? 3 : sr == 4 ? 2 : sr == 2 ? 1 : 0;
    g.n_stripes = (k + sr - 1) / sr;
    g.n_stripes += g.n_stripes & 1;
    g.n_wg = g.n_stripes / 2;
}
static void gram_exchange_rows(const GramPlan& g, int& r_lo, int& r_hi) {
    const int SR = 1 << g.sr_shift, h = g.n_wg / 2;
    r_lo = std::min(g.k, h * SR);
    r_hi = std::min(g.k, std::max(r_lo, (g.n_stripes - h) * SR));
}
static size_t packed_row_offset(int row, int k) { return (size_t)row * (size_t)k - (size_t)row * (size_t)(row - 1) / 2; }

int32_t gram_plan(srx_ctx* ctx, int k, uint64_t n_rows, GramPlan& g, double entries_per_cell, int entry_bytes) {
    gram_stripes_of(k, g);
    const int sr = 1 << g.sr_shift;
    size_t widest = 0;
    for (int w = 0; w < g.n_wg; ++w) {
        const int a0 = w * sr, b0 = (g.n_stripes - 1 - w) * sr;
        const size_t wd = (size_t)(k - a0) + (size_t)(k - b0 > 0 ? k - b0 : 0);
        widest = std::max(widest, wd);
    }
    g.lds_bytes = (size_t)sr * widest * 8;
    if (g.lds_bytes > 163840) return fail(ctx, SRX_E_ARG, "pca: %d selected features exceed the Gram kernel's LDS stripes", k);
    g.rblk = 512u;
    if ((uint64_t)g.rblk * (uint64_t)k * 16u >= (1ull << 31))
        return fail(ctx, SRX_E_ARG, "pca: %d selected features exceed the owner records' 32-bit offsets", k);
    g.n_rblk = (n_rows + g.rblk - 1) / g.rblk;
    const int per_cu = g.lds_bytes <= 65536 ? 2 : 1;
    uint64_t chunk = 16384 / g.rblk;
    if (entries_per_cell > 0.0 && entry_bytes > 0) {
        const double m = entries_per_cell;
        double cells = 9.0e7 / (0.5 * m * (m + 1.0));
        cells = std::min(cells, 18.9e6 / (m * (double)entry_bytes));
        chunk = (uint64_t)(cells / g.rblk + 0.5);
        if (chunk > 65536 / g.rblk) chunk = 65536 / g.rblk;
    }
    static_assert(65536ull * (1ull << 47) <= (1ull << 63), "chunk cap x product bound must fit the accumulator");
    if (chunk * g.rblk > 65536) chunk = 65536 / g.rblk;
    chunk = std::max<uint64_t>(chunk, kGramWaves);
    const uint64_t want_wgs = (uint64_t)ctx->n_cus * per_cu;
    while (chunk > kGramWaves && ((g.n_rblk + chunk - 1) / chunk) * (uint64_t)g.n_wg < want_wgs) chunk /= 2;
    g.n_chunk = (uint32_t)chunk;
    int z = (int)((g.n_rblk + chunk - 1) / chunk);
    if (z < 1) z = 1;
    g.n_z = z;
    return SRX_OK;
}
int grid_rows(const srx_ctx* ctx, uint64_t n_rows, int rows_per_block) {
    uint64_t want = (n_rows + rows_per_block - 1) / rows_per_block;
    uint64_t cap = (uint64_t)ctx->n_cus * 8;
    if (want < 1) want = 1;
    return (int)(want < cap ? want : cap);
}

int32_t scan_exclusive(srx_ctx* ctx, const int64_t* d_in, uint64_t n, int64_t* d_out, int64_t** total_dev) {
    const uint64_t per_block = (uint64_t)kScanBlock * kScanItems;
    const uint64_t nb = (n + per_block - 1) / per_block > 0 ? (n + per_block - 1) / per_block : 1;
    int64_t* d_bsum;
    SRX_TRY(scratch(ctx, "scan_bsum", (nb + 1) * sizeof(int64_t), (void**)&d_bsum));
    int64_t* d_total = d_bsum + nb;
    hipLaunchKernelGGL(k_scan_block_sums, dim3((unsigned)nb), dim3(kScanBlock), 0, ctx->stream, d_in, n, d_bsum);
    hipLaunchKernelGGL(k_scan_serial, dim3(1), dim3(kScanBlock), 0, ctx->stream, d_bsum, nb, d_total);
    hipLaunchKernelGGL(k_scan_apply, dim3((unsigned)nb), dim3(kScanBlock), 0, ctx->stream, d_in, n, d_bsum, d_total,
                       d_out);
    SRX_HIP(ctx, hipGetLastError());
    if (total_dev) *total_dev = d_total;
    return SRX_OK;
}

int32_t retile(srx_mat* m, const RowMajor& rm, Tiled& t) {
    srx_ctx* ctx = m->ctx;
    const uint64_t N = rm.n_rows;
    t.n_rows = N;
    t.nnz = rm.nnz;
    t.k = rm.k;
    t.nt = (rm.k + KT - 1) / KT;
    int64_t* d_tp = nullptr;
    if (t.nt > 1) {
        SRX_TRY(scratch(ctx, "pca_tp", (size_t)(t.nt - 1) * (N ? N : 1) * sizeof(int64_t), (void**)&d_tp));
        if (is_f32(m)) SRX_TRY(launch_tile_ptr(ctx, rm.ptr, (const GramPk<float>*)rm.pk, N, t.nt, KT, d_tp));
        else SRX_TRY(launch_tile_ptr(ctx, rm.ptr, (const GramPk<double>*)rm.pk, N, t.nt, KT, d_tp));
    }
    const uint64_t nseg = (uint64_t)t.nt * N;
    int64_t* d_seglen;
    SRX_TRY(scratch(ctx, "pca_seglen", (nseg ? nseg : 1) * sizeof(int64_t), (void**)&d_seglen));
    SRX_TRY(scratch(ctx, "pca_t256_ptr", (nseg + 1) * sizeof(int64_t), (void**)&t.tptr));
    uint64_t g = (nseg + 255) / 256;
    if (g < 1) g = 1;
    if (g > 16384) g = 16384;
    hipLaunchKernelGGL(k_seglen, dim3((unsigned)g), dim3(256), 0, ctx->stream, rm.ptr, d_tp, N, t.nt, d_seglen);
    SRX_TRY(scan_exclusive(ctx, d_seglen, nseg, t.tptr, nullptr));
    const size_t pb = is_f32(m) ? sizeof(GramPk<float>) : sizeof(GramPk<double>);
    SRX_TRY(scratch(ctx, "pca_t256_pk", (rm.nnz + 64) * pb, &t.tpk));
    SRX_HIP(ctx, hipMemsetAsync((char*)t.tpk + rm.nnz * pb, 0, 64 * pb, ctx->stream));
    if (is_f32(m))
        hipLaunchKernelGGL((k_retile<float>), dim3(grid_rows(ctx, N, 4)), dim3(256), 0, ctx->stream, rm.ptr, d_tp,
                           (const GramPk<float>*)rm.pk, N, t.nt, t.tptr, (GramPk<float>*)t.tpk);
    else
        hipLaunchKernelGGL((k_retile<double>), dim3(grid_rows(ctx, N, 4)), dim3(256), 0, ctx->stream, rm.ptr, d_tp,
                           (const GramPk<double>*)rm.pk, N, t.nt, t.tptr, (GramPk<double>*)t.tpk);
    SRX_HIP(ctx, hipGetLastError());
    return SRX_OK;
}

int32_t compact_selection(srx_mat* m, const uint32_t* d_sel, int n_words, int k, RowMajor& rm, RowXf xf, bool want_recs) {
    srx_ctx* ctx = m->ctx;
    const uint64_t N = m->n_rows;
    int64_t *cntrow, *d_total;
    const size_t sel_lds = 2 * (size_t)n_words * sizeof(uint32_t);
    const bool sel_in_lds = sel_lds <= 60000;
    SRX_TRY(scratch(ctx, "pca_cntrow", (N ? N : 1) * sizeof(int64_t), (void**)&cntrow));
    SRX_TRY(scratch(ctx, "pca_rm_ptr", (N + 1) * sizeof(int64_t), (void**)&rm.ptr));
    const double s_i = m->d_idx16 ? 2.0 : 4.0;
    const size_t pb = is_f32(m) ? sizeof(GramPk<float>) : sizeof(GramPk<double>);
    const bool list = m->n_cols <= 65536 && m->d_idx16 && k < 0xffff + 1;
    ProfScope ps(ctx, SRX_K_COMPACT, (double)m->nnz * s_i * (list ? 1.0 : 2.0) + (double)(N + 1) * 8.0 * 2.0);
    uint32_t* kept = nullptr;
    if (list) {
        SRX_TRY(scratch(ctx, "pca_keptlist", (m->nnz + 64) * sizeof(uint32_t), (void**)&kept));
        const size_t col_lds = ((size_t)n_words * 32 + 1) * sizeof(uint16_t);
        const int per_cu = std::max(1, std::min(2, (int)(160 * 1024 / (col_lds + 1024))));
        const uint64_t visits = (N + (uint64_t)kCompactRows * (kCountThreads / kWave) - 1) / ((uint64_t)kCompactRows * (kCountThreads / kWave));
        const unsigned cgrid = (unsigned)std::max<uint64_t>(1, std::min<uint64_t>(visits, (uint64_t)ctx->n_cus * per_cu));
        SRX_HIP(ctx, hipFuncSetAttribute((const void*)k_rowcount_list, hipFuncAttributeMaxDynamicSharedMemorySize, (int)col_lds));
        hipLaunchKernelGGL(k_rowcount_list, dim3(cgrid), dim3(kCountThreads), col_lds, ctx->stream, m->d_indptr,
                           (const uint16_t*)m->d_idx16, d_sel, d_sel + n_words, n_words, N, m->nnz, k, cntrow, kept);
    } else {
        auto count = [&](auto kern, const auto* idxp, size_t lds) {
            hipLaunchKernelGGL(kern, dim3(grid_rows(ctx, N, 4)), dim3(256), lds, ctx->stream, m->d_indptr, idxp, d_sel, n_words, N, cntrow);
        };
        const size_t bits_lds = (size_t)n_words * sizeof(uint32_t);
        if (m->d_idx16) {
            if (sel_in_lds) count(k_rowcount<uint16_t, true>, (const uint16_t*)m->d_idx16, bits_lds);
            else count(k_rowcount<uint16_t, false>, (const uint16_t*)m->d_idx16, 0);
        } else {
            if (sel_in_lds) count(k_rowcount<int32_t, true>, (const int32_t*)m->d_indices, bits_lds);
            else count(k_rowcount<int32_t, false>, (const int32_t*)m->d_indices, 0);
        }
    }
    SRX_TRY(scan_exclusive(ctx, cntrow, N, rm.ptr, &d_total));
    int64_t* d_nrecs = nullptr;
    rm.n_recs = -1;
    if (want_recs && N > 0) {
        GramPlan g;
        SRX_TRY(gram_plan(ctx, k, N, g));
        int64_t *blk_total, *rec_base;
        SRX_TRY(scratch(ctx, "pca_brtot", g.n_rblk * sizeof(int64_t), (void**)&blk_total));
        SRX_TRY(scratch(ctx, "pca_brbase", (g.n_rblk + 4) * sizeof(int64_t), (void**)&rec_base));
        hipLaunchKernelGGL(k_rec_count, dim3((unsigned)g.n_rblk), dim3(256), 0, ctx->stream, (const int64_t*)rm.ptr, N, g.rblk, blk_total);
        hipLaunchKernelGGL(k_rec_scan, dim3(1), dim3(1024), 0, ctx->stream, (const int64_t*)blk_total, g.n_rblk, rec_base,
                           (const int64_t*)d_total);
        SRX_HIP(ctx, hipGetLastError());
        d_nrecs = rec_base + g.n_rblk;
    }
    int64_t total = 0;
    {
        int64_t both[2] = {0, 0};
        SRX_TRY(d2h_begin(ctx, d_nrecs ? (const void*)d_nrecs : (const void*)d_total, d_nrecs ? sizeof both : sizeof(int64_t)));
        rm.n_rows = N;
        SRX_TRY(build_row_order(ctx, rm));
        SRX_TRY(d2h_end(ctx, both, d_nrecs ? sizeof both : sizeof(int64_t)));
        if (d_nrecs) {
            rm.n_recs = both[0];
            total = both[1];
        } else {
            total = both[0];
        }
    }
    SRX_TRY(scratch(ctx, "pca_rm_pk", ((size_t)total + 64) * pb, &rm.pk));
    if (!list) SRX_HIP(ctx, hipMemsetAsync((char*)rm.pk + (size_t)total * pb, 0, 64 * pb, ctx->stream));
    rm.nnz = (uint64_t)total;
    rm.k = k;
    auto fill = [&](auto kern, const auto* idxp, const auto* valp, auto* rmp) {
        hipLaunchKernelGGL(kern, dim3(grid_rows(ctx, N, 4)), dim3(256), sel_in_lds ? sel_lds : 0, ctx->stream, m->d_indptr, idxp,
                           valp, d_sel, d_sel + n_words, n_words, N, k, rm.ptr, xf.row_sum, xf.target, rmp);
    };
    auto fill_t = [&](auto tval, auto* rmp) {
        using T = decltype(tval);
        const T* valp = (const T*)m->d_values;
        auto by_sel = [&](auto xf_tag, const auto* ip) {
            constexpr bool XF = decltype(xf_tag)::value;
            using I = std::remove_cv_t<std::remove_pointer_t<decltype(ip)>>;
            if (sel_in_lds) fill(k_tfill<T, I, XF, true>, ip, valp, rmp);
            else fill(k_tfill<T, I, XF, false>, ip, valp, rmp);
        };
        auto by_xf = [&](const auto* ip) {
            if (xf.row_sum) by_sel(std::true_type{}, ip);
            else by_sel(std::false_type{}, ip);
        };
        if (m->d_idx16) by_xf((const uint16_t*)m->d_idx16);
        else by_xf((const int32_t*)m->d_indices);
    };
    if (list) {
        const unsigned g2 = (unsigned)grid_rows(ctx, N, 8);
        if (is_f32(m)) {
            if (xf.row_sum) hipLaunchKernelGGL((k_tfill_list<float, true>), dim3(g2), dim3(256), 0, ctx->stream, m->d_indptr, (const float*)m->d_values, kept, N, rm.ptr, xf.row_sum, xf.target, (GramPk<float>*)rm.pk);
            else hipLaunchKernelGGL((k_tfill_list<float, false>), dim3(g2), dim3(256), 0, ctx->stream, m->d_indptr, (const float*)m->d_values, kept, N, rm.ptr, xf.row_sum, xf.target, (GramPk<float>*)rm.pk);
        } else {
            if (xf.row_sum) hipLaunchKernelGGL((k_tfill_list<double, true>), dim3(g2), dim3(256), 0, ctx->stream, m->d_indptr, (const double*)m->d_values, kept, N, rm.ptr, xf.row_sum, xf.target, (GramPk<double>*)rm.pk);
            else hipLaunchKernelGGL((k_tfill_list<double, false>), dim3(g2), dim3(256), 0, ctx->stream, m->d_indptr, (const double*)m->d_values, kept, N, rm.ptr, xf.row_sum, xf.target, (GramPk<double>*)rm.pk);
        }
    } else if (is_f32(m)) fill_t(float{}, (GramPk<float>*)rm.pk);
    else fill_t(double{}, (GramPk<double>*)rm.pk);
    SRX_HIP(ctx, hipGetLastError());
    if (ctx->prof_mask & (1u << SRX_K_COMPACT))
    {
        ctx->prof[SRX_K_COMPACT].bytes += (double)total * (val_bytes(m) + (double)pb);
        if (list) ctx->prof[SRX_K_COMPACT].aux_bytes += (double)total * 4.0 * 2.0;
    }
    return SRX_OK;
}

constexpr int kCommFreeCus = 16;
static int32_t ensure_comm_streams(srx_ctx* ctx) {
    if (!ctx->comm_stream) {
        SRX_HIP(ctx, hipStreamCreateWithFlags(&ctx->comm_stream, hipStreamNonBlocking));
        SRX_HIP(ctx, hipEventCreateWithFlags(&ctx->comm_fork, hipEventDisableTiming));
        SRX_HIP(ctx, hipEventCreateWithFlags(&ctx->comm_join, hipEventDisableTiming));
    }
    if (!ctx->gram_stream) {
        uint32_t mask[8];
        const int n_cus = ctx->n_cus > 256 ? 256 : ctx->n_cus;
        for (int w = 0; w < 8; ++w) mask[w] = 0u;
        for (int c = 0; c < n_cus; ++c)
            if (c >= kCommFreeCus) mask[c >> 5] |= 1u << (c & 31);
        if (n_cus <= 2 * kCommFreeCus ||
            hipExtStreamCreateWithCUMask(&ctx->gram_stream, (uint32_t)((n_cus + 31) / 32), mask) != hipSuccess) {
            (void)hipGetLastError();
            SRX_HIP(ctx, hipStreamCreateWithFlags(&ctx->gram_stream, hipStreamNonBlocking));
            ctx->gram_stream_masked = false;
        } else {
            ctx->gram_stream_masked = true;
        }
        SRX_HIP(ctx, hipEventCreateWithFlags(&ctx->gram_fork, hipEventDisableTiming));
        SRX_HIP(ctx, hipEventCreateWithFlags(&ctx->gram_join, hipEventDisableTiming));
    }
    return SRX_OK;
}

template <typename VT>
int32_t launch_gram(srx_ctx* ctx, const RowMajor& rm, double* Gp, bool* reduce, bool zero_first) {
    if (reduce) *reduce = false;
    GramPlan g;
// ... 17 lines not shown
        if (rm.n_recs >= 0) {
            n_recs = rm.n_recs;
        } else {
            hipLaunchKernelGGL(k_rec_count, dim3((unsigned)g.n_rblk), dim3(256), 0, ctx->stream, rm.ptr, rm.n_rows, g.rblk, blk_total);
            hipLaunchKernelGGL(k_rec_scan, dim3(1), dim3(1024), 0, ctx->stream, blk_total, g.n_rblk, rec_base);
            SRX_HIP(ctx, hipGetLastError());
            SRX_TRY(d2h(ctx, &n_recs, rec_base + g.n_rblk, sizeof(int64_t)));
        }
        SRX_TRY(scratch(ctx, "pca_brecs", ((size_t)n_recs + kGramUnroll) * sizeof(GramRec<VT>), (void**)&recs));
        if (ctx->prof_mask & (1u << SRX_K_BUCKET)) ctx->prof[SRX_K_BUCKET].bytes += (double)n_recs * sizeof(GramRec<VT>);
        hipLaunchKernelGGL((k_bucket<VT>), dim3((unsigned)g.n_rblk), dim3(kBucketThreads),
                           (size_t)(g.n_wg + 1 + g.rblk + 1 + kBucketGroup) * sizeof(uint32_t), ctx->stream, rm.ptr,
                           (const GramPk<VT>*)rm.pk, rm.n_rows, g.rblk, rm.k, g.sr_shift, g.n_wg, g.n_stripes, rec_base, boff, recs,
                           reinterpret_cast<uint32_t*>(rec_base + g.n_rblk + 2), n_recs, zero_first ? Gp : (double*)nullptr,
                           (uint64_t)rm.k * (rm.k + 1) / 2);
        SRX_HIP(ctx, hipGetLastError());
    }
    if (stat_exchange) {
        constexpr int EB = sizeof(VT) == 4 ? 8 : 11;
        constexpr int n_bins = gstat_bins<EB>();
        double* bins = nullptr;
        SRX_TRY(scratch(ctx, "pca_gstat_bins", gstat_bins<11>() * sizeof(double), (void**)&bins));
        SRX_HIP(ctx, hipMemsetAsync(bins, 0, n_bins * sizeof(double), ctx->stream));
        uint32_t* gs = empty ? nullptr : reinterpret_cast<uint32_t*>(rec_base + g.n_rblk + 2);
        if (gs) hipLaunchKernelGGL(k_gstat_onehot<EB>, dim3(1), dim3(64), 0, ctx->stream, (const uint32_t*)gs, bins);
        SRX_TRY(allreduce_f64(ctx, bins, n_bins));
        if (gs) hipLaunchKernelGGL(k_gstat_decode<EB>, dim3(1), dim3(64), 0, ctx->stream, (const double*)bins, gs);
        SRX_HIP(ctx, hipGetLastError());
    }
    if (empty && !split) return SRX_OK;
    const bool force_f64 = getenv("SRX_GRAM_F64_ATOMICS") && atoi(getenv("SRX_GRAM_F64_ATOMICS"));
    ctx->gram_mode_state = empty ? 0 : (force_f64 ? 1 : 2);
    if (!empty && !force_f64) {
        if (!ctx->d_gram_mode) SRX_HIP(ctx, hipMalloc((void**)&ctx->d_gram_mode, 4 * sizeof(uint32_t)));
        SRX_HIP(ctx, hipMemcpyAsync(ctx->d_gram_mode, rec_base + g.n_rblk + 2, 3 * sizeof(uint32_t), hipMemcpyDeviceToDevice, ctx->stream));
        ctx->gram_mode_f32 = sizeof(VT) == 4;
    }
    ProfScope ps(ctx, SRX_K_GRAM, (double)rm.nnz * sizeof(GramPk<VT>) + (double)(rm.n_rows + 1) * 8.0 + (double)rm.k * (rm.k + 1) / 2 * 8.0,
                 nullptr, (double)n_recs * sizeof(GramRec<VT>) + (double)g.n_rblk * (g.n_wg + 1) * 4.0);
    if (!empty) SRX_HIP(ctx, hipFuncSetAttribute((const void*)k_gram_stripes<VT>, hipFuncAttributeMaxDynamicSharedMemorySize, (int)g.lds_bytes));
    auto launch = [&](int w0, int n_w, hipStream_t st) {
        if (empty) return;
        hipLaunchKernelGGL((k_gram_stripes<VT>), dim3((unsigned)(n_w * g.n_z)), dim3(kGramWaves * kWave), g.lds_bytes, st,
                           rm.ptr, (const GramPk<VT>*)rm.pk, boff, rec_base, recs, g.n_rblk, g.rblk, rm.k, g.sr_shift, g.n_wg,
                           g.n_stripes, g.n_chunk, w0, n_w, Gp,
                           (const uint32_t*)(rec_base && !force_f64 ? reinterpret_cast<uint32_t*>(rec_base + g.n_rblk + 2) : nullptr));
    };
    if (split) {
        SRX_TRY(ensure_comm_streams(ctx));
        const int k = rm.k;
        int r_lo, r_hi;
        gram_exchange_rows(g, r_lo, r_hi);
        auto off = [&](int row) { return packed_row_offset(row, k); };
        launch(0, h, ctx->stream);
        SRX_HIP(ctx, hipGetLastError());
        SRX_HIP(ctx, hipEventRecord(ctx->comm_fork, ctx->stream));
        SRX_HIP(ctx, hipStreamWaitEvent(ctx->comm_stream, ctx->comm_fork, 0));
        SRX_TRY(allreduce_f64_on(ctx, Gp, off(r_lo), ctx->comm_stream));
        SRX_TRY(allreduce_f64_on(ctx, Gp + off(r_hi), off(k) - off(r_hi), ctx->comm_stream));
        SRX_HIP(ctx, hipEventRecord(ctx->gram_fork, ctx->stream));
        SRX_HIP(ctx, hipStreamWaitEvent(ctx->gram_stream, ctx->gram_fork, 0));
        launch(h, g.n_wg - h, ctx->gram_stream);
        SRX_HIP(ctx, hipGetLastError());
        SRX_HIP(ctx, hipEventRecord(ctx->gram_join, ctx->gram_stream));
        SRX_HIP(ctx, hipStreamWaitEvent(ctx->stream, ctx->gram_join, 0));
        SRX_HIP(ctx, hipStreamWaitEvent(ctx->comm_stream, ctx->gram_join, 0));
        SRX_TRY(allreduce_f64_on(ctx, Gp + off(r_lo), off(r_hi) - off(r_lo), ctx->comm_stream));
        SRX_HIP(ctx, hipEventRecord(ctx->comm_join, ctx->comm_stream));
        SRX_HIP(ctx, hipStreamWaitEvent(ctx->stream, ctx->comm_join, 0));
        *reduce = true;
        ctx->gram_splits++;
        return SRX_OK;
    }
    launch(0, g.n_wg, ctx->stream);
    SRX_HIP(ctx, hipGetLastError());
    return SRX_OK;
}

template int32_t launch_gram<float>(srx_ctx*, const RowMajor&, double*, bool*, bool);
template int32_t launch_gram<double>(srx_ctx*, const RowMajor&, double*, bool*, bool);

}

extern "C" int32_t srx_gram_mode_info(srx_ctx* ctx, int32_t* mode_out) {
    using namespace srx;
    if (!ctx || !mode_out) return fail(ctx, SRX_E_ARG, "srx_gram_mode_info: null argument");
    *mode_out = 0;
    if (ctx->gram_mode_state == 0) return SRX_OK;
    if (ctx->gram_mode_state == 1) {
        *mode_out = 1;
        return SRX_OK;
    }
    uint32_t w[3] = {0, 0, 0};
    SRX_TRY(d2h(ctx, w, ctx->d_gram_mode, sizeof w));
    int kq;
    *mode_out = (ctx->gram_mode_f32 ? gram_fixed_point_mode(w[0], w[1], w[2], kq) : gram_fixed_point_mode64(w[0], w[1], w[2], kq)) ? 2 : 1;
    return SRX_OK;
}

extern "C" int32_t srx_gram_exchange_ranges(uint64_t k, uint64_t* offsets_out) {
    using namespace srx;
    if (!offsets_out || k < 1 || k > 16384) return fail(nullptr, SRX_E_ARG, "srx_gram_exchange_ranges: bad arguments");
    GramPlan g;
    gram_stripes_of((int)k, g);
    int r_lo, r_hi;
    gram_exchange_rows(g, r_lo, r_hi);
    offsets_out[0] = 0;
    offsets_out[1] = packed_row_offset(r_lo, (int)k);
    offsets_out[2] = packed_row_offset(r_hi, (int)k);
    offsets_out[3] = packed_row_offset((int)k, (int)k);
    return SRX_OK;
}
```

### singlerust_amd/csrc/pca_internal.hpp

```cpp
#pragma once

#include <algorithm>
#include <cmath>
#include <numeric>
#include <string>
#include <type_traits>
#include <vector>

#include "common.hpp"
#include "pca_result.hpp"

namespace srx {

constexpr int L = 64;
constexpr int kTThreads = 1024;

constexpr int KT = 256;
constexpr uint64_t kDevSelMaxK = 8192;

template <typename VT> struct GramPk;
template <> struct __attribute__((aligned(8))) GramPk<float> { int32_t j; float v; };
template <> struct __attribute__((aligned(16))) GramPk<double> { int32_t j; int32_t pad_; double v; };

constexpr int kGramWaves = 16;
// ... 49 lines not shown
}
template <int S>
__device__ __forceinline__ float ror16(float x) {
    return __builtin_bit_cast(float, ror16<S>(__builtin_bit_cast(int, x)));
}
template <int S>
__device__ __forceinline__ double ror16(double x) {
    long long b = __builtin_bit_cast(long long, x);
    int lo = ror16<S>((int)(b & 0xffffffffll)), hi = ror16<S>((int)(b >> 32));
    return __builtin_bit_cast(double, ((long long)hi << 32) | (unsigned int)lo);
}
__device__ __forceinline__ int64_t readlane64(int64_t x, int l) {
    int lo = __builtin_amdgcn_readlane((int)(x & 0xffffffffll), l);
    int hi = __builtin_amdgcn_readlane((int)(x >> 32), l);
    return ((int64_t)hi << 32) | (uint32_t)lo;
}
__device__ __forceinline__ float readlane_v(float x, int l) {
    return __builtin_bit_cast(float, __builtin_amdgcn_readlane(__builtin_bit_cast(int, x), l));
}
__device__ __forceinline__ double readlane_v(double x, int l) {
    return __builtin_bit_cast(double, readlane64(__builtin_bit_cast(long long, x), l));
}

struct Tiled {
    uint64_t n_rows = 0, nnz = 0;
    int k = 0, nt = 0;
    int64_t* tptr = nullptr;
    void* tpk = nullptr;
};
struct GramPlan {
    int k = 0, sr_shift = 0, n_stripes = 0, n_wg = 0;
    int n_z = 1;
    uint32_t rblk = 512;
    uint32_t n_chunk = 0;
    uint64_t n_rblk = 0;
    size_t lds_bytes = 0;
};
struct RowMajor {
    uint64_t n_rows = 0, nnz = 0;
    int k = 0;
    int64_t* ptr = nullptr;
    void* pk = nullptr;
    uint32_t* perm = nullptr;
    int64_t n_recs = -1;
};
struct Resolved {
    int n_pc, center, scale, max_iter, solver;
    double bail_ratio = 0.0;
    bool direct = false;
    bool robust = false;
    int power = 1;
    int warm = 0;
    double tol;
    uint64_t seed;
};


int32_t hvg_list_host(srx_mat* m, uint64_t n, std::vector<uint64_t>& out);
int32_t gene_variances(srx_mat* m, std::vector<double>& var);
constexpr const char* kNanVarianceMsg = "NaN gene variance: called `Option::unwrap()` on a `None` value (partial_cmp)";
struct SelDev {
    int k = 0, n_words = 0;
    int32_t* d_sel_rank = nullptr;
    uint32_t* d_bits = nullptr;
    double *d_mu = nullptr, *d_sd = nullptr, *d_dinv = nullptr, *d_trace = nullptr;
    int* d_status = nullptr;
};
bool hvg_on_device(uint64_t n, uint64_t n_cols);
int32_t select_hvg_device(srx_mat* m, uint64_t n, int center, int scale, SelDev& out);
int32_t select_list(srx_mat* m, const uint64_t* genes, uint64_t k, int center, int scale, SelDev& out, bool vectors = true);
template <typename E>
int32_t launch_tile_ptr(srx_ctx* ctx, const int64_t* indptr, const E* idx, uint64_t n_rows, int n_tiles, int tile_genes,
                        int64_t* tp);

int32_t gram_plan(srx_ctx* ctx, int k, uint64_t n_rows, GramPlan& g, double entries_per_cell = 0.0, int entry_bytes = 0);
int grid_rows(const srx_ctx* ctx, uint64_t n_rows, int rows_per_block);
int32_t compact_selection(srx_mat* m, const uint32_t* d_sel, int n_words, int k, RowMajor& rm, RowXf xf = RowXf{},
                          bool want_recs = false);
int32_t retile(srx_mat* m, const RowMajor& rm, Tiled& t);
template <typename VT>
int32_t launch_gram(srx_ctx* ctx, const RowMajor& rm, double* Gp, bool* reduce = nullptr, bool zero_first = false);
inline size_t gram_packed_count(int k) { return (size_t)k * (size_t)(k + 1) / 2; }

int32_t build_row_order(srx_ctx* ctx, RowMajor& r);
int scores_ld(int n_pc);
void result_layout(uint64_t n_rows, int k, int n_pc, int dim, size_t& score_bytes, size_t& small_doubles,
                   std::vector<int>* plan_a_out = nullptr, std::vector<int>* plan_b_out = nullptr);
int32_t ensure_result_capacity(srx_ctx* ctx, srx_pca_state& st, size_t need);
int32_t resolve_opts(srx_ctx* ctx, const srx_pca_opts* opts, int k, uint64_t Ng, bool f32, Resolved& o, int& l_act);
inline PcaResultLayout result_block(const srx_pca_state& st) { return PcaResultLayout(st.k, L, st.round_counts); }
int32_t solve_and_stash(srx_ctx* ctx, bool f32, const RowMajor* parts, int n_parts, const Tiled* t256p, double* gram_packed,
                        const Resolved& o, const SelDev& sel, int l_act, uint64_t n_cells, uint64_t nnz_selected, srx_pca_state& st);

}
```

### singlerust_amd/csrc/pca_solve.hip

```cpp
#include "pca_internal.hpp"

namespace srx {

#include "spmm.inl"

#include "iterate.inl"

template <typename VT, typename PT>
static int32_t launch_fwd(srx_ctx* ctx, const Tiled& c, const PT* P, const PT* cvec, PT* Y, double* scores = nullptr,
                          int n_pc = 0, int ld = 0) {
    const double out_bytes = scores ? (double)c.n_rows * n_pc * 8.0 : (double)c.n_rows * L * sizeof(PT);
    const double bytes = (double)c.nnz * (4.0 + sizeof(VT)) + (double)((uint64_t)c.nt * c.n_rows + 1) * 8.0 + out_bytes +
                         (double)c.k * L * sizeof(PT);
    const size_t lds = (size_t)KT * L * sizeof(PT);
    constexpr int kRowsPerWg = (kFwdThreads / 16) * FwdCfg<PT>::kRows;
    const uint64_t n_blocks = (c.n_rows + kRowsPerWg - 1) / kRowsPerWg;
    const int per_cu = sizeof(PT) == 4 ? 2 : 1;
    uint64_t grid = (uint64_t)ctx->n_cus * per_cu;
    if (grid > n_blocks) grid = n_blocks;
    if (grid < 1) grid = 1;
    ProfScope ps(ctx, SRX_K_SPMM_FWD, bytes);
    SRX_HIP(ctx, hipFuncSetAttribute((const void*)k_spmm_fwd<VT, PT>, hipFuncAttributeMaxDynamicSharedMemorySize,
                                     (int)lds));
    hipLaunchKernelGGL((k_spmm_fwd<VT, PT>), dim3((unsigned)grid), dim3(kFwdThreads), lds, ctx->stream, c.tptr,
                       (const GramPk<VT>*)c.tpk, c.n_rows, c.nt, c.k, P, cvec, Y, scores, n_pc, ld ? ld : n_pc);
    SRX_HIP(ctx, hipGetLastError());
    return SRX_OK;
}

template <typename PT>
static int fwd_rows_q(int k) {
    const size_t budget = 163840 - 64;
    for (int q = sizeof(PT) == 4 ? 4 : 2; q >= 1; q >>= 1)
        if ((size_t)k * 4 * q * sizeof(PT) <= budget) return q;
    return 0;
}

template <typename VT, typename PT>
static int32_t launch_fwd_rows(srx_ctx* ctx, const RowMajor& r, const PT* P, const PT* cvec, int n_cols, double* scores, PT* Y,
                               int ld) {
    const int Qr = fwd_rows_q<PT>(r.k);
    auto go = [&](auto qtag, auto rtag, auto cltag, int k_lo, int k_hi, int accumulate) -> int32_t {
        constexpr int Q = decltype(qtag)::value;
        constexpr bool RANGE = decltype(rtag)::value;
        constexpr int CL = decltype(cltag)::value;
        constexpr int C = CL * Q;
        const int n_slices = (n_cols + C - 1) / C;
        const int ldp = C;
        const size_t lds = (size_t)(k_hi - k_lo) * ldp * sizeof(PT);
        const uint64_t groups = kFwdRowsThreads / Q;
        uint64_t n_wg = (r.n_rows + groups - 1) / groups;
        uint64_t cap = std::max<uint64_t>(1, (uint64_t)ctx->n_cus * 8 / n_slices);
        if (cap > 8) cap &= ~(uint64_t)7;
        if (n_wg > cap) n_wg = cap;
        if (n_wg < 1) n_wg = 1;
        const double out_bytes = scores ? (double)r.n_rows * n_cols * 8.0 : (double)r.n_rows * L * sizeof(PT);
        ProfScope ps(ctx, SRX_K_SPMM_FWD, (double)r.nnz * sizeof(GramPk<VT>) + (double)(r.n_rows + 1) * 8.0 + out_bytes +
                                              (double)(k_hi - k_lo) * L * sizeof(PT) + (r.perm ? (double)r.n_rows * 4.0 : 0.0));
        SRX_HIP(ctx, hipFuncSetAttribute((const void*)k_spmm_rows<VT, PT, Q, RANGE, CL>, hipFuncAttributeMaxDynamicSharedMemorySize, (int)lds));
        hipLaunchKernelGGL((k_spmm_rows<VT, PT, Q, RANGE, CL>), dim3((unsigned)(n_wg * n_slices)), dim3(kFwdRowsThreads), lds, ctx->stream,
                           r.ptr, (const GramPk<VT>*)r.pk, (const uint32_t*)r.perm, r.n_rows, r.k, P, cvec, n_cols, scores, Y, ld, ldp,
                           k_lo, k_hi, accumulate, 0);
        SRX_HIP(ctx, hipGetLastError());
        return SRX_OK;
    };
    using No = std::false_type;
    using Yes = std::true_type;
    using C4 = std::integral_constant<int, 4>;
    using C5 = std::integral_constant<int, 5>;
    constexpr int Qmax = sizeof(PT) == 4 ? 4 : 2;
    const int wide_slices = (n_cols + 5 * Qmax - 1) / (5 * Qmax), narrow_slices = (n_cols + 4 * Qmax - 1) / (4 * Qmax);
    const bool wide = Qr == Qmax && (size_t)r.k * 5 * Qmax * sizeof(PT) <= (size_t)163840 && wide_slices < narrow_slices &&
                      wide_slices * 5 * Qmax <= L && sizeof(PT) == 8;
    if (wide) return go(std::integral_constant<int, Qmax>{}, No{}, C5{}, 0, r.k, 0);
    if (Qr == 4) {
        if constexpr (sizeof(PT) == 4) return go(std::integral_constant<int, 4>{}, No{}, C4{}, 0, r.k, 0);
        else return SRX_E_ARG;
    }
    if (Qr == 2) return go(std::integral_constant<int, 2>{}, No{}, C4{}, 0, r.k, 0);
    if (Qr == 1) return go(std::integral_constant<int, 1>{}, No{}, C4{}, 0, r.k, 0);
    const int per = (int)((163840 - 64) / (4 * sizeof(PT)));
    for (int k_lo = 0, i = 0; k_lo < r.k; k_lo += per, ++i)
        SRX_TRY(go(std::integral_constant<int, 1>{}, Yes{}, C4{}, k_lo, std::min(r.k, k_lo + per), i > 0 ? 1 : 0));
    return SRX_OK;
}

int32_t build_row_order(srx_ctx* ctx, RowMajor& r) {
    uint32_t* hist;
    SRX_TRY(scratch(ctx, "pca_rm_lenhist", kLenBins * sizeof(uint32_t), (void**)&hist));
    SRX_TRY(scratch(ctx, "pca_rm_perm", (r.n_rows ? r.n_rows : 1) * sizeof(uint32_t), (void**)&r.perm));
    SRX_HIP(ctx, hipMemsetAsync(hist, 0, kLenBins * sizeof(uint32_t), ctx->stream));
    const unsigned g = (unsigned)((r.n_rows + kLenRowsPerWg - 1) / kLenRowsPerWg + (r.n_rows ? 0 : 1));
    hipLaunchKernelGGL(k_len_hist, dim3(g), dim3(256), 0, ctx->stream, r.ptr, r.n_rows, hist);
    hipLaunchKernelGGL(k_len_scan, dim3(1), dim3(kLenBins), 0, ctx->stream, hist);
    hipLaunchKernelGGL(k_len_scatter, dim3(g), dim3(256), 0, ctx->stream, r.ptr, r.n_rows, hist, r.perm);
    SRX_HIP(ctx, hipGetLastError());
    return SRX_OK;
}

template <typename VT, typename YT>
static int32_t launch_t(srx_ctx* ctx, const Tiled& c, const YT* Y, double* T ) {
    uint64_t want = (uint64_t)(2 * ctx->n_cus) / (uint64_t)c.nt;
    if (want < 1) want = 1;
    uint64_t by_rows = (c.n_rows + 255) / 256;
    if (by_rows < 1) by_rows = 1;
    const uint64_t n_rb = want < by_rows ? want : by_rows;
    const uint64_t rpb = (c.n_rows + n_rb - 1) / n_rb > 0 ? (c.n_rows + n_rb - 1) / n_rb : 1;
    double *part, *part_s;
    SRX_TRY(scratch(ctx, "pca_tpart", n_rb * (size_t)c.k * L * sizeof(double), (void**)&part));
    SRX_TRY(scratch(ctx, "pca_tpart_s", n_rb * L * sizeof(double), (void**)&part_s));
    const size_t lds = (size_t)KT * L * sizeof(double);
    const double bytes = (double)c.nnz * (4.0 + sizeof(VT)) + (double)((uint64_t)c.nt * c.n_rows + 1) * 8.0 +
                         (double)c.n_rows * L * sizeof(YT) + (double)c.k * L * 8.0;
    {
        ProfScope ps(ctx, SRX_K_SPMM_T, bytes);
        SRX_HIP(ctx, hipFuncSetAttribute((const void*)k_spmm_t<VT, YT, double>,
                                         hipFuncAttributeMaxDynamicSharedMemorySize, (int)lds));
        hipLaunchKernelGGL((k_spmm_t<VT, YT, double>), dim3((unsigned)(n_rb * c.nt)), dim3(kTThreads), lds, ctx->stream,
                           c.tptr, (const GramPk<VT>*)c.tpk, c.n_rows, c.k, c.nt, rpb, Y, part, part_s);
        uint64_t tot = (uint64_t)c.k * L + L;
        hipLaunchKernelGGL((k_t_reduce<double>), dim3((unsigned)((tot + 255) / 256)), dim3(256), 0, ctx->stream, part,
                           part_s, c.k, n_rb, T);
    }
    SRX_HIP(ctx, hipGetLastError());
    return SRX_OK;
}

static uint64_t mix64(uint64_t x) {
    x += 0x9E3779B97F4A7C15ull;
    x = (x ^ (x >> 30)) * 0xBF58476D1CE4E5B9ull;
    x = (x ^ (x >> 27)) * 0x94D049BB133111EBull;
    return x ^ (x >> 31);
}

struct Work {
    double *W, *Wp, *T, *A1, *A2, *small, *mu, *d, *gpart;
    double *dHG, *dM, *dM2, *dTheta, *dRho, *dColmax, *dSgn, *dDinv, *dXi;
};

static int32_t alloc_work(srx_ctx* ctx, int k, Work& w) {
    const size_t kl = (size_t)k * L;
    SRX_TRY(scratch(ctx, "pca_W", kl * 8, (void**)&w.W));
    SRX_TRY(scratch(ctx, "pca_Wp", kl * 8, (void**)&w.Wp));
    SRX_TRY(scratch(ctx, "pca_T", (kl + L) * 8, (void**)&w.T));
    SRX_TRY(scratch(ctx, "pca_A1", kl * 8, (void**)&w.A1));
    SRX_TRY(scratch(ctx, "pca_A2", kl * 8, (void**)&w.A2));
    SRX_TRY(scratch(ctx, "pca_small", (6 * L * L + 8 * L + 4 * 16 * 16) * 8, (void**)&w.small));
    SRX_TRY(scratch(ctx, "pca_mu", (size_t)k * 8, (void**)&w.mu));
    SRX_TRY(scratch(ctx, "pca_d", (size_t)k * 8, (void**)&w.d));
    SRX_TRY(scratch(ctx, "pca_g2part", (size_t)kGram2Blocks * 2 * L * L * 8, (void**)&w.gpart));
    w.dHG = w.small;
    w.dM = w.small + 2 * L * L;
    w.dM2 = w.small + 3 * L * L;
    w.dTheta = w.small + 4 * L * L;
    w.dRho = w.dTheta + L;
    w.dColmax = w.dRho + L;
    w.dSgn = w.dColmax + L;
    w.dDinv = w.dSgn + L;
    w.dXi = w.small + 6 * L * L + 8 * L;
    return SRX_OK;
}

static int32_t gram2(srx_ctx* ctx, const Work& w, const double* A, const double* B, int k) {
    int nb = (k + 31) / 32;
    if (nb > kGram2Blocks) nb = kGram2Blocks;
    if (nb < 1) nb = 1;
    hipLaunchKernelGGL(k_gram2_part, dim3(nb), dim3(1024), 0, ctx->stream, A, B, k, w.gpart);
    hipLaunchKernelGGL(k_gram2_reduce, dim3((2 * L * L + 255) / 256), dim3(256), 0, ctx->stream, w.gpart, nb, w.dHG);
    SRX_HIP(ctx, hipGetLastError());
    return SRX_OK;
}

template <typename Fn>
static int32_t graphed(srx_ctx* ctx, bool enable, const std::string& key, Fn&& enqueue) {
    if (!enable || ctx->graphs_off) return enqueue();
    auto it = ctx->graphs.find(key);
    if (it == ctx->graphs.end()) {
        if (ctx->graphs.size() >= 32) {
            for (auto& kv : ctx->graphs) (void)hipGraphExecDestroy(kv.second);
// ... 753 lines not shown
```

### singlerust_amd/csrc/rows.hip

```cpp
#include "common.hpp"
#include "log1p64.hpp"

namespace srx {

constexpr int kRowCache = 32;

template <typename T>
struct alignas(16) RowVec {
    T x[16 / sizeof(T)];
};

template <typename T, bool NORM, bool LOG, bool PRECISE = false>
__global__ __launch_bounds__(256) void k_row_pass(const int64_t* __restrict__ indptr, T* __restrict__ vals,
                                                  uint64_t n_rows, double target,
                                                  double* __restrict__ row_sum_out) {
    __shared__ Log1pTabEntry s_tab[PRECISE ? 128 : 1];
    if constexpr (PRECISE) {
        stage_log1p_table(s_tab);
        __syncthreads();
    }
    constexpr int V = 16 / sizeof(T);
    constexpr int NV = kRowCache / V;
    using Vec = RowVec<T>;
    const uint64_t wave = global_wave_id();
    const uint64_t n_waves = ((uint64_t)gridDim.x * blockDim.x) / kWave;
    const int lane = lane_id();
    for (uint64_t r = wave; r < n_rows; r += n_waves) {
        const int64_t lo = indptr[r], hi = indptr[r + 1];
        const int64_t base = lo & ~(int64_t)(V - 1);
        const int64_t tail = base + (int64_t)NV * kWave * V;
        Vec c[NV];
        double s = 0.0;
#pragma unroll
        for (int t = 0; t < NV; ++t) {
            const int64_t e0 = base + ((int64_t)t * kWave + lane) * V;
            if (e0 < hi) c[t] = *reinterpret_cast<const Vec*>(vals + e0);
            else {
#pragma unroll
                for (int j = 0; j < V; ++j) c[t].x[j] = T(0);
            }
        }
        if (NORM) {
#pragma unroll
            for (int t = 0; t < NV; ++t) {
                const int64_t e0 = base + ((int64_t)t * kWave + lane) * V;
#pragma unroll
                for (int j = 0; j < V; ++j) {
                    const int64_t pos = e0 + j;
                    s += (pos >= lo && pos < hi) ? (double)c[t].x[j] : 0.0;
                }
            }
            for (int64_t p = tail + lane; p < hi; p += kWave) s += (double)vals[p];
            s = wave_sum(s);
            if (row_sum_out && lane == 0) row_sum_out[r] = s;
        }
        const double scale = NORM ? (s == 0.0 ? 0.0 : target / s) : 1.0;
        double row_table = 0.0;
        if constexpr (PRECISE) row_table = xf_row_table(scale, s_tab);
        auto f = [&](T v) -> T {
            if constexpr (PRECISE) return (T)xf_apply<T>(v, scale, row_table, s_tab);
            T x = NORM ? (T)((double)v * scale) : v;
            return LOG ? apply_log1p<T>(x) : x;
        };
#pragma unroll
        for (int t = 0; t < NV; ++t) {
            const int64_t e0 = base + ((int64_t)t * kWave + lane) * V;
            Vec o;
            if constexpr (PRECISE) {
                if (__any(e0 < hi)) {
#pragma unroll
                    for (int j = 0; j < V; ++j) o.x[j] = f(c[t].x[j]);
                }
            }
            if (e0 < hi && e0 + V > lo) {
                if constexpr (!PRECISE) {
#pragma unroll
                    for (int j = 0; j < V; ++j) o.x[j] = f(c[t].x[j]);
                }
                if (e0 >= lo && e0 + V <= hi) {
                    *reinterpret_cast<Vec*>(vals + e0) = o;
                } else {
#pragma unroll
                    for (int j = 0; j < V; ++j) {
                        const int64_t pos = e0 + j;
                        if (pos >= lo && pos < hi) vals[pos] = o.x[j];
                    }
                }
            }
        }
        if constexpr (PRECISE) {
            for (int64_t p0 = tail; p0 < hi; p0 += kWave) {
                const int64_t p = p0 + lane;
                const T y = f(p < hi ? vals[p] : T(0));
                if (p < hi) vals[p] = y;
            }
        } else {
            for (int64_t p = tail + lane; p < hi; p += kWave) vals[p] = f(vals[p]);
        }
    }
}

template <typename T>
__global__ __launch_bounds__(256) void k_row_sum(const int64_t* __restrict__ indptr, const T* __restrict__ vals,
                                                 uint64_t n_rows, double* __restrict__ out) {
    const uint64_t wave = global_wave_id();
    const uint64_t n_waves = ((uint64_t)gridDim.x * blockDim.x) / kWave;
    const int lane = lane_id();
    for (uint64_t r = wave; r < n_rows; r += n_waves) {
        const int64_t lo = indptr[r], hi = indptr[r + 1];
        double s = 0.0;
        if constexpr (sizeof(T) == 4) {
            typedef float f4u __attribute__((ext_vector_type(4), aligned(4)));
            const int64_t n4 = (hi - lo) >> 2;
            int64_t q = lane;
            for (; q + kWave < n4; q += 2 * kWave) {
                const f4u a = *reinterpret_cast<const f4u*>(vals + lo + 4 * q), b = *reinterpret_cast<const f4u*>(vals + lo + 4 * (q + kWave));
                s += ((double)a.x + (double)a.y) + ((double)a.z + (double)a.w);
                s += ((double)b.x + (double)b.y) + ((double)b.z + (double)b.w);
            }
            if (q < n4) {
                const f4u a = *reinterpret_cast<const f4u*>(vals + lo + 4 * q);
                s += ((double)a.x + (double)a.y) + ((double)a.z + (double)a.w);
            }
            const int64_t t = lo + 4 * n4 + lane;
            if (t < hi) s += (double)vals[t];
        } else {
            int64_t p = lo + lane;
            for (; p + 3 * kWave < hi; p += 4 * kWave) {
                T a = vals[p], b = vals[p + kWave], c = vals[p + 2 * kWave], d = vals[p + 3 * kWave];
                s += (double)a; s += (double)b; s += (double)c; s += (double)d;
            }
            for (; p < hi; p += kWave) s += (double)vals[p];
        }
        s = wave_sum(s);
        if (lane == 0) out[r] = s;
    }
}

template <typename T>
__global__ __launch_bounds__(256) void k_row_var(const int64_t* __restrict__ indptr, const T* __restrict__ vals,
                                                 uint64_t n_rows, double* __restrict__ out) {
    const uint64_t wave = global_wave_id();
    const uint64_t n_waves = ((uint64_t)gridDim.x * blockDim.x) / kWave;
    const int lane = lane_id();
    for (uint64_t r = wave; r < n_rows; r += n_waves) {
        const int64_t lo = indptr[r], hi = indptr[r + 1];
        double s = 0.0;
        for (int64_t p = lo + lane; p < hi; p += kWave) s += (double)vals[p];
        s = wave_sum(s);
        const double cnt = (double)(uint32_t)(hi - lo);
        const double mean = s / cnt;
        double a = 0.0;
        for (int64_t p = lo + lane; p < hi; p += kWave) {
            double d = (double)vals[p] - mean;
            a += d * d;
        }
        a = wave_sum(a);
        if (lane == 0) out[r] = a / cnt;
    }
}

template <typename T>
__global__ __launch_bounds__(256) void k_row_qc(const int64_t* __restrict__ indptr, const T* __restrict__ vals,
                                                uint64_t n_rows, uint32_t* __restrict__ num, double* __restrict__ sum,
                                                double* __restrict__ var) {
    constexpr int V = 16 / sizeof(T);
    constexpr int NV = kRowCache / V;
    using Vec = RowVec<T>;
    const uint64_t wave = global_wave_id();
    const uint64_t n_waves = ((uint64_t)gridDim.x * blockDim.x) / kWave;
    const int lane = lane_id();
    for (uint64_t r = wave; r < n_rows; r += n_waves) {
        const int64_t lo = indptr[r], hi = indptr[r + 1];
        const int64_t base = lo & ~(int64_t)(V - 1);
        const int64_t tail = base + (int64_t)NV * kWave * V;
        Vec c[NV];
#pragma unroll
        for (int t = 0; t < NV; ++t) {
            const int64_t e0 = base + ((int64_t)t * kWave + lane) * V;
            if (e0 < hi) c[t] = *reinterpret_cast<const Vec*>(vals + e0);
            else {
#pragma unroll
                for (int j = 0; j < V; ++j) c[t].x[j] = T(0);
            }
        }
        double s = 0.0;
#pragma unroll
        for (int t = 0; t < NV; ++t) {
            const int64_t e0 = base + ((int64_t)t * kWave + lane) * V;
#pragma unroll
// ... 85 lines not shown
                const int64_t e0 = b0 + (int64_t)t * kWave * V;
                if (e0 >= hi) continue;
                Vec o;
#pragma unroll
                for (int j = 0; j < V; ++j) o.x[j] = xf_stored(c[t].x[j], scale, s_tab);
                if (e0 >= lo && e0 + V <= hi) {
                    *reinterpret_cast<Vec*>(vals + e0) = o;
                } else {
#pragma unroll
                    for (int j = 0; j < V; ++j)
                        if (e0 + j >= lo && e0 + j < hi) vals[e0 + j] = o.x[j];
                }
            }
        }
    }
}

static int row_grid(const srx_mat* m) {
    uint64_t want = (m->n_rows + 3) / 4;
    uint64_t cap = (uint64_t)m->ctx->n_cus * 8;
    if (want < 1) want = 1;
    return (int)(want < cap ? want : cap);
}

int32_t launch_normalize(srx_mat* m, double target, bool do_norm, bool do_log, hipStream_t stream, bool precise, int wgs_per_cu) {
    srx_ctx* ctx = m->ctx;
    SRX_HIP(ctx, hipSetDevice(ctx->device));
    if (!stream) stream = ctx->stream;
    if (do_norm && !m->d_row_sum) SRX_HIP(ctx, dev_malloc(ctx, (void**)&m->d_row_sum, (m->n_rows ? m->n_rows : 1) * sizeof(double)));
    int g = row_grid(m);
    if (wgs_per_cu > 0 && g > ctx->n_cus * wgs_per_cu) g = ctx->n_cus * wgs_per_cu;
    const double bytes = (double)m->nnz * 2.0 * val_bytes(m) + (double)(m->n_rows + 1) * 8.0;
    {
        ProfScope ps(ctx, SRX_K_NORMALIZE, bytes, stream);
#define SRX_LAUNCH_ROW(T, N, L, P)                                                                  \
    hipLaunchKernelGGL((k_row_pass<T, N, L, P>), dim3(g), dim3(256), 0, stream, m->d_indptr,         \
                       (T*)m->d_values, m->n_rows, target, (N) ? m->d_row_sum : (double*)nullptr)
        if (is_f32(m)) {
            if (do_norm && do_log && precise) SRX_LAUNCH_ROW(float, true, true, true);
            else if (do_norm && do_log) SRX_LAUNCH_ROW(float, true, true, false);
            else if (do_norm) SRX_LAUNCH_ROW(float, true, false, false);
            else if (do_log) SRX_LAUNCH_ROW(float, false, true, false);
        } else {
            if (do_norm && do_log && precise) SRX_LAUNCH_ROW(double, true, true, true);
            else if (do_norm && do_log) SRX_LAUNCH_ROW(double, true, true, false);
            else if (do_norm) SRX_LAUNCH_ROW(double, true, false, false);
            else if (do_log) SRX_LAUNCH_ROW(double, false, true, false);
        }
#undef SRX_LAUNCH_ROW
    }
    SRX_HIP(ctx, hipGetLastError());
    if (do_norm) m->dtype = SRX_F64;
    if (do_log && m->dtype != SRX_F32) m->dtype = SRX_F64;
    touch(m);
    return SRX_OK;
}

int32_t launch_row_apply(srx_mat* m, double target, hipStream_t stream) {
    srx_ctx* ctx = m->ctx;
    SRX_HIP(ctx, hipSetDevice(ctx->device));
    if (!m->d_row_sum) return fail(ctx, SRX_E_ARG, "row write-back without row sums");
    if (!stream) stream = ctx->stream;
    {
        ProfScope ps(ctx, SRX_K_NORMALIZE, (double)m->nnz * 2.0 * val_bytes(m) + (double)(m->n_rows + 1) * 8.0 + (double)m->n_rows * 8.0, stream);
        if (is_f32(m))
            hipLaunchKernelGGL((k_row_apply<float>), dim3(row_grid(m)), dim3(256), 0, stream, m->d_indptr, (float*)m->d_values,
                               m->n_rows, target, m->d_row_sum);
        else
            hipLaunchKernelGGL((k_row_apply<double>), dim3(row_grid(m)), dim3(256), 0, stream, m->d_indptr, (double*)m->d_values,
                               m->n_rows, target, m->d_row_sum);
    }
    SRX_HIP(ctx, hipGetLastError());
    m->dtype = SRX_F64;
    touch(m);
    return SRX_OK;
}

int32_t launch_row_sums(srx_mat* m, double* out) {
    srx_ctx* ctx = m->ctx;
    SRX_HIP(ctx, hipSetDevice(ctx->device));
    if (!out && !m->d_row_sum) SRX_HIP(ctx, dev_malloc(ctx, (void**)&m->d_row_sum, (m->n_rows ? m->n_rows : 1) * sizeof(double)));
    double* const dst = out ? out : m->d_row_sum;
    const int g = row_grid(m);
    ProfScope ps(ctx, SRX_K_ROWSUM, (double)m->nnz * val_bytes(m) + (double)(m->n_rows + 1) * 8.0 + (double)m->n_rows * 8.0);
    if (is_f32(m))
        hipLaunchKernelGGL((k_row_sum<float>), dim3(g), dim3(256), 0, ctx->stream, m->d_indptr, (const float*)m->d_values,
                           m->n_rows, dst);
    else
        hipLaunchKernelGGL((k_row_sum<double>), dim3(g), dim3(256), 0, ctx->stream, m->d_indptr, (const double*)m->d_values,
                           m->n_rows, dst);
    SRX_HIP(ctx, hipGetLastError());
    return SRX_OK;
}

int32_t row_qc(srx_mat* m, uint32_t* num, double* sum, double* var) {
    srx_ctx* ctx = m->ctx;
    const uint64_t N = m->n_rows ? m->n_rows : 1;
    uint32_t* d_num;
    double* d_f;
    SRX_TRY(scratch(ctx, "row_u32", N * sizeof(uint32_t), (void**)&d_num));
    SRX_TRY(scratch(ctx, "row_f64", 2 * N * sizeof(double), (void**)&d_f));
    const int g = row_grid(m);
    if (is_f32(m))
        hipLaunchKernelGGL((k_row_qc<float>), dim3(g), dim3(256), 0, ctx->stream, m->d_indptr, (const float*)m->d_values,
                           m->n_rows, d_num, d_f, d_f + N);
    else
        hipLaunchKernelGGL((k_row_qc<double>), dim3(g), dim3(256), 0, ctx->stream, m->d_indptr, (const double*)m->d_values,
                           m->n_rows, d_num, d_f, d_f + N);
    SRX_HIP(ctx, hipGetLastError());
    if (num) SRX_TRY(d2h(ctx, num, d_num, m->n_rows * sizeof(uint32_t)));
    if (sum) SRX_TRY(d2h(ctx, sum, d_f, m->n_rows * sizeof(double)));
    if (var) SRX_TRY(d2h(ctx, var, d_f + N, m->n_rows * sizeof(double)));
    return SRX_OK;
}

}

using namespace srx;

extern "C" {

int32_t srx_log1p_inplace(srx_mat* m) {
    if (!m) return fail(nullptr, SRX_E_ARG, "null matrix");
    if (m->dtype != SRX_F32) SRX_TRY(promote_to_f64(m));
    return launch_normalize(m, 0.0, false, true);
}

int32_t srx_normalize_log1p_inplace(srx_mat* m, double target_sum, double* row_sums_out) {
    if (!m) return fail(nullptr, SRX_E_ARG, "null matrix");
    if (m->csc) {
        if (row_sums_out) SRX_TRY(srx_compute_sum(m, SRX_ROW, row_sums_out));
        SRX_TRY(srx_normalize_total_inplace(m, target_sum, SRX_ROW));
        return srx_log1p_inplace(m);
    }
    SRX_TRY(promote_to_f64(m));
    SRX_TRY(launch_normalize(m, target_sum, true, true));
    if (row_sums_out) SRX_TRY(d2h(m->ctx, row_sums_out, m->d_row_sum, m->n_rows * sizeof(double)));
    return SRX_OK;
}

}

namespace srx {

int32_t row_number(srx_mat* m, uint32_t* out) {
    srx_ctx* ctx = m->ctx;
    uint32_t* d;
    SRX_TRY(scratch(ctx, "row_u32", (m->n_rows ? m->n_rows : 1) * sizeof(uint32_t), (void**)&d));
    uint64_t g = (m->n_rows + 255) / 256;
    if (g < 1) g = 1;
    if (g > 4096) g = 4096;
    hipLaunchKernelGGL(k_row_number, dim3((int)g), dim3(256), 0, ctx->stream, m->d_indptr, m->n_rows, d);
    SRX_HIP(ctx, hipGetLastError());
    return d2h(ctx, out, d, m->n_rows * sizeof(uint32_t));
}

int32_t row_stat(srx_mat* m, int which, double* out0, double* out1) {
    srx_ctx* ctx = m->ctx;
    double* d;
    SRX_TRY(scratch(ctx, "row_f64", 2 * (m->n_rows ? m->n_rows : 1) * sizeof(double), (void**)&d));
    double* d1 = d + m->n_rows;
    const int g = row_grid(m);
#define SRX_ROW_K(K, ...)                                                                          \
    do {                                                                                           \
        if (is_f32(m))                                                                             \
            hipLaunchKernelGGL((K<float>), dim3(g), dim3(256), 0, ctx->stream, m->d_indptr,         \
                               (const float*)m->d_values, m->n_rows, __VA_ARGS__);                  \
        else                                                                                       \
            hipLaunchKernelGGL((K<double>), dim3(g), dim3(256), 0, ctx->stream, m->d_indptr,        \
                               (const double*)m->d_values, m->n_rows, __VA_ARGS__);                 \
    } while (0)
    if (which == 0) SRX_ROW_K(k_row_sum, d);
    else if (which == 1) SRX_ROW_K(k_row_var, d);
    else SRX_ROW_K(k_row_minmax, d, d1);
// ... 9 lines not shown
```

### singlerust_amd/csrc/select.hip

```cpp
#include "pca_internal.hpp"

#include <algorithm>
#include <cmath>

#pragma clang fp contract(off)

namespace srx {


static int32_t select_hvg_host(srx_ctx* ctx, const std::vector<double>& var, uint64_t n, std::vector<uint64_t>& out) {
    for (double v : var)
        if (v != v) return fail(ctx, SRX_E_NAN, "%s", kNanVarianceMsg);
    std::vector<uint64_t> order(var.size());
    for (uint64_t j = 0; j < order.size(); ++j) order[j] = j;
    uint64_t take = n < order.size() ? n : order.size();
    auto before = [&](uint64_t a, uint64_t b) { return var[a] > var[b] || (var[a] == var[b] && a < b); };
    std::nth_element(order.begin(), order.begin() + (take ? take - 1 : 0), order.end(), before);
    std::sort(order.begin(), order.begin() + take, before);
    out.assign(order.begin(), order.begin() + take);
    return SRX_OK;
}

__global__ void k_gene_var(const uint64_t* __restrict__ cnt, const double* __restrict__ sum, const double* __restrict__ sq,
                           uint64_t G, double* __restrict__ var, uint32_t* __restrict__ rank, uint32_t rank_init) {
// ... 15 lines not shown
    const uint32_t j = bx * 256 + threadIdx.x;
    const uint32_t base = by * kRankTile;
    for (uint32_t e = threadIdx.x; e < kRankTile; e += 256) tile[e] = base + e < G ? var[base + e] : -INFINITY;
    __syncthreads();
    if (j < G) {
        const double mine = var[j];
        const uint32_t j_lo = bx * 256, j_hi = j_lo + 255;
        uint32_t rank = 0;
        if (base + kRankTile - 1 < j_lo) {
#pragma unroll 8
            for (int e = 0; e < kRankTile; ++e) rank += tile[e] >= mine ? 1u : 0u;
        } else if (base > j_hi) {
#pragma unroll 8
            for (int e = 0; e < kRankTile; ++e) rank += tile[e] > mine ? 1u : 0u;
        } else {
#pragma unroll 4
            for (int e = 0; e < kRankTile; ++e) {
                const double o = tile[e];
                rank += (o > mine || (o == mine && base + e < j)) ? 1u : 0u;
            }
        }
        atomicAdd(&rank_out[j], rank);
    }
    __syncthreads();
}
__global__ __launch_bounds__(256) void k_hvg_rank(const double* __restrict__ var, uint32_t G, uint32_t* __restrict__ rank_out) {
    __shared__ double tile[kRankTile];
    full_rank_pair(var, G, rank_out, blockIdx.x, blockIdx.y, tile);
}

constexpr int kRankSample = 512;
constexpr int kSelThreads = 1024;
__global__ __launch_bounds__(kSelThreads) void k_hvg_candidates(const double* __restrict__ var, uint32_t G, uint32_t n, uint32_t cap,
                                                                uint32_t* __restrict__ counter, uint32_t* __restrict__ cand,
                                                                uint32_t* __restrict__ rank_out,
                                                                int force_miss ) {
    __shared__ double sv[kRankSample];
    __shared__ double s_thr;
    __shared__ uint32_t s_cnt;
    const uint32_t S = G < (uint32_t)kRankSample ? G : (uint32_t)kRankSample;
    const uint32_t t = threadIdx.x, lane = t & 63;
    if (t < (uint32_t)kRankSample) sv[t] = t < S ? var[(uint64_t)t * G / S] : -INFINITY;
    if (t == 0) {
        s_thr = force_miss ? INFINITY : -INFINITY;
        s_cnt = 0u;
    }
    __syncthreads();
    if (!force_miss && S == (uint32_t)kRankSample) {
        const double q = (double)n / (double)G;
        const double kq = (q + 4.0 * sqrt(q * (1.0 - q) / (double)S)) * (double)S + 1.0;
        for (uint32_t size = 2; size <= (uint32_t)kRankSample; size <<= 1)
            for (uint32_t stride = size >> 1; stride > 0; stride >>= 1) {
                if (t < (uint32_t)kRankSample / 2) {
                    const uint32_t lo = 2 * t - (t & (stride - 1)), hi = lo + stride;
                    const bool desc = (lo & size) == 0;
                    const double a = sv[lo], b = sv[hi];
                    if (desc ? a < b : a > b) {
                        sv[lo] = b;
                        sv[hi] = a;
                    }
                }
                __syncthreads();
            }
        if (t == 0 && kq < (double)(S - 1)) s_thr = sv[(uint32_t)kq];
    }
    __syncthreads();
    const double thr = s_thr;
    constexpr int kAhead = 8;
    for (uint32_t base = 0; base < G; base += kSelThreads * kAhead) {
        double v[kAhead];
#pragma unroll
        for (int a = 0; a < kAhead; ++a) {
            const uint32_t j = base + a * kSelThreads + t;
            v[a] = j < G ? var[j] : -INFINITY;
        }
#pragma unroll
        for (int a = 0; a < kAhead; ++a) {
            const uint32_t j = base + a * kSelThreads + t;
            const bool in = j < G && v[a] >= thr;
            const unsigned long long m = __ballot(in);
            uint32_t at = 0;
            if (lane == 0 && m) at = atomicAdd(&s_cnt, (uint32_t)__popcll(m));
            at = __shfl(at, 0, 64);
            if (in) {
                cand[at + (uint32_t)__popcll(m & ((1ull << lane) - 1ull))] = j;
                rank_out[j] = 0u;
            }
        }
    }
    __syncthreads();
    const uint32_t M = s_cnt;
    const bool ok = M >= n && M <= cap;
    if (!ok)
        for (uint32_t j = t; j < G; j += kSelThreads) rank_out[j] = 0u;
    if (t == 0) *counter = ok ? M : 0xffffffffu;
}
constexpr int kCandTile = 128;
__global__ __launch_bounds__(256) void k_rank_selected(const double* __restrict__ var, uint32_t G, const uint32_t* __restrict__ counter,
                                                       const uint32_t* __restrict__ cand, uint32_t* __restrict__ rank_out) {
    __shared__ double tile[kRankTile];
    const uint32_t M = *counter;
    if (M == 0xffffffffu) {
        const uint32_t gb = (G + 255) / 256, gy = (G + kRankTile - 1) / kRankTile;
        for (uint32_t p = blockIdx.y * gridDim.x + blockIdx.x; p < gb * gy; p += gridDim.x * gridDim.y)
            full_rank_pair(var, G, rank_out, p % gb, p / gb, tile);
        return;
    }
    double* tv = tile;
    uint32_t* ti = reinterpret_cast<uint32_t*>(tile + kCandTile);
    const uint32_t base = blockIdx.y * kCandTile;
    if (blockIdx.x * 256 >= M || base >= M) return;
    for (uint32_t e = threadIdx.x; e < kCandTile; e += 256) {
        const uint32_t g = base + e < M ? cand[base + e] : 0xffffffffu;
        ti[e] = g;
        tv[e] = g != 0xffffffffu ? var[g] : -INFINITY;
    }
    __syncthreads();
    const uint32_t i = blockIdx.x * 256 + threadIdx.x;
    if (i >= M) return;
    const uint32_t gi = cand[i];
    const double mine = var[gi];
    uint32_t rank = 0;
#pragma unroll 4
    for (int e = 0; e < kCandTile; ++e) {
        const double o = tv[e];
        rank += (o > mine || (o == mine && ti[e] < gi)) ? 1u : 0u;
    }
    if (rank) atomicAdd(&rank_out[gi], rank);
}

constexpr int kSelLdsWords = 2048;
template <bool LDS>
__global__ __launch_bounds__(1024) void k_sel_finish(const uint32_t* __restrict__ rank, const double* __restrict__ gene_var,
                                                     const double* __restrict__ sum,
                                                     const double* __restrict__ sq, uint32_t G, uint32_t take, int n_words,
                                                     double n_cells, int center, int scale, int32_t* __restrict__ sel_rank,
                                                     int* __restrict__ status, uint32_t* __restrict__ bits,
                                                     uint32_t* __restrict__ prefix, double* __restrict__ mu,
                                                     double* __restrict__ sd, double* __restrict__ dinv,
                                                     double* __restrict__ trace) {
    __shared__ uint32_t s_bits[LDS ? kSelLdsWords : 1], s_pre[LDS ? kSelLdsWords : 1], s_wave[16];
    __shared__ double s_tr[1024];
    __shared__ int s_nan;
    uint32_t* const wbits = LDS ? s_bits : bits;
    uint32_t* const wpre = LDS ? s_pre : prefix;
    const int t = threadIdx.x, lane = t & 63, wv = t >> 6;
    if (t == 0) s_nan = 0;
    __syncthreads();
    bool nan = false;
    constexpr int kAhead = 8;
    for (uint32_t base = 0; base < (uint32_t)n_words * 32; base += 1024 * kAhead) {
        uint32_t rk[kAhead];
        double v[kAhead];
#pragma unroll
        for (int a = 0; a < kAhead; ++a) {
            const uint32_t g = base + a * 1024 + t;
            rk[a] = g < G ? rank[g] : 0xffffffffu;
            v[a] = g < G && gene_var ? gene_var[g] : 0.0;
        }
#pragma unroll
        for (int a = 0; a < kAhead; ++a) {
            const uint32_t g = base + a * 1024 + t;
            nan |= v[a] != v[a];
            const bool in = rk[a] < take;
            if (in) sel_rank[rk[a]] = (int32_t)g;
            const unsigned long long m = __ballot(in);
            if (lane == 0 && (g >> 5) < (uint32_t)n_words) wbits[g >> 5] = (uint32_t)m;
            if (lane == 32 && (g >> 5) < (uint32_t)n_words) wbits[g >> 5] = (uint32_t)(m >> 32);
        }
    }
// ... 21 lines not shown
        if (w + 1 < n_words) wpre[w + 1] = excl + c0;
        for (int q = 0; q < 16; ++q) carry += s_wave[q];
        __syncthreads();
    }
    for (int w = t; w < n_words; w += 1024) {
        uint32_t b_ = wbits[w];
        const uint32_t e = wpre[w], room = e < take ? take - e : 0u;
        while ((uint32_t)__popc(b_) > room) b_ &= ~(1u << (31 - __clz((int)b_)));
        wbits[w] = b_;
    }
    __syncthreads();
    if constexpr (LDS)
        for (int w = t; w < n_words; w += 1024) {
            bits[w] = s_bits[w];
            prefix[w] = s_pre[w];
        }
    double tr = 0.0;
    for (uint32_t g = t; sum && g < G; g += 1024) {
        const uint32_t w = wbits[g >> 5], bit = 1u << (g & 31);
        if (!(w & bit)) continue;
        const uint32_t s = wpre[g >> 5] + (uint32_t)__popc(w & (bit - 1u));
        const double mean = sum[g] / n_cells;
        double var = sq[g] / n_cells - mean * mean;
        if (var < 0) var = 0;
        const double std_ = sqrt(var);
        mu[s] = (center || scale) ? mean : 0.0;
        sd[s] = scale ? std_ : 1.0;
        const double di = (scale && std_ > 0) ? 1.0 / std_ : 1.0;
        dinv[s] = di;
        double ss = center ? (sq[g] - n_cells * mean * mean) : sq[g];
        if (ss < 0) ss = 0;
        tr += di * di * ss;
    }
    s_tr[t] = tr;
    __syncthreads();
    for (int half = 512; half > 0; half >>= 1) {
        if (t < half) s_tr[t] += s_tr[t + half];
        __syncthreads();
    }
    if (t == 0) {
        *trace = s_tr[0];
        *status = s_nan;
    }
}

static int32_t sel_buffers(srx_ctx* ctx, uint64_t G, uint64_t take, SelDev& out, uint32_t** d_rank) {
    const int n_words = (int)((G + 31) / 32);
    double* d_f;
    SRX_TRY(scratch(ctx, "hvg_rankv", at_least_one(G) * sizeof(uint32_t), (void**)d_rank));
    SRX_TRY(scratch(ctx, "hvg_rank", at_least_one(take) * sizeof(int32_t), (void**)&out.d_sel_rank));
    SRX_TRY(scratch(ctx, "pca_selbits", at_least_one(2 * n_words) * sizeof(uint32_t), (void**)&out.d_bits));
    SRX_TRY(scratch(ctx, "hvg_f", (3 * at_least_one(take) + 8) * sizeof(double), (void**)&d_f));
    SRX_TRY(scratch(ctx, "hvg_status", 256, (void**)&out.d_status));
    out.d_mu = d_f;
    out.d_sd = d_f + take;
    out.d_dinv = d_f + 2 * take;
    out.d_trace = d_f + 3 * take;
    out.k = (int)take;
    out.n_words = n_words;
    return SRX_OK;
}

static int32_t launch_sel_finish(srx_mat* m, const uint32_t* d_rank, const double* d_var, bool vectors, int center, int scale,
                                 const SelDev& out) {
    srx_ctx* ctx = m->ctx;
    auto kern = out.n_words <= kSelLdsWords ? k_sel_finish<true> : k_sel_finish<false>;
    hipLaunchKernelGGL(kern, dim3(1), dim3(1024), 0, ctx->stream, d_rank, d_var, vectors ? m->d_sum : nullptr, m->d_sq,
                       (uint32_t)m->n_cols, (uint32_t)out.k, out.n_words, (double)m->n_rows_global, center, scale, out.d_sel_rank,
                       out.d_status, out.d_bits, out.d_bits + out.n_words, out.d_mu, out.d_sd, out.d_dinv, out.d_trace);
    SRX_HIP(ctx, hipGetLastError());
    return SRX_OK;
}

bool hvg_on_device(uint64_t n, uint64_t n_cols) {
    return n > 0 && std::min(n, n_cols) <= kDevSelMaxK && n_cols <= 65536;
}

int32_t select_hvg_device(srx_mat* m, uint64_t n, int center, int scale, SelDev& out) {
    srx_ctx* ctx = m->ctx;
    const uint64_t G = m->n_cols;
    const uint64_t take = n < G ? n : G;
    double* d_var;
    uint32_t* d_rank;
    SRX_TRY(scratch(ctx, "hvg_var", at_least_one(G) * sizeof(double), (void**)&d_var));
    SRX_TRY(sel_buffers(ctx, G, take, out, &d_rank));
    const unsigned gb = (unsigned)at_least_one((G + 255) / 256);
    const unsigned gy = (unsigned)at_least_one((G + kRankTile - 1) / kRankTile);
    static const bool full_rank = getenv("SRX_HVG_FULL_RANK") != nullptr;
    const bool all = full_rank || take == 0 || G < (uint64_t)kRankSample;
    hipLaunchKernelGGL(k_gene_var, dim3(gb), dim3(256), 0, ctx->stream, m->d_cnt, m->d_sum, m->d_sq, G, d_var, d_rank, all ? 0u : 0xffffffffu);
    if (all) {
        hipLaunchKernelGGL(k_hvg_rank, dim3(gb, gy), dim3(256), 0, ctx->stream, d_var, (uint32_t)G, d_rank);
    } else {
        uint32_t* d_cand;
        SRX_TRY(scratch(ctx, "hvg_cand", (at_least_one(G) + 8) * sizeof(uint32_t), (void**)&d_cand));
        uint32_t* d_counter = d_cand + G + 4;
        static const int force_miss = getenv("SRX_HVG_FORCE_MISS") ? 1 : 0;
        const uint32_t cap = (uint32_t)std::min<uint64_t>(G, std::max<uint64_t>(4 * take, 4096));
        hipLaunchKernelGGL(k_hvg_candidates, dim3(1), dim3(kSelThreads), 0, ctx->stream, d_var, (uint32_t)G, (uint32_t)take, cap, d_counter, d_cand,
                           d_rank, force_miss);
        hipLaunchKernelGGL(k_rank_selected, dim3((cap + 255) / 256, (cap + kCandTile - 1) / kCandTile), dim3(256), 0, ctx->stream, d_var,
                           (uint32_t)G, d_counter, d_cand, d_rank);
    }
    return launch_sel_finish(m, d_rank, d_var, true, center, scale, out);
}

int32_t select_list(srx_mat* m, const uint64_t* genes, uint64_t k, int center, int scale, SelDev& out, bool vectors) {
    srx_ctx* ctx = m->ctx;
    const uint64_t G = m->n_cols;
    std::vector<uint32_t> rank(G, 0xffffffffu);
    for (uint64_t s = 0; s < k; ++s) {
        const uint64_t g = genes ? genes[s] : s;
        if (g >= G) return fail(ctx, SRX_E_BOUNDS, "selected feature index %llu out of bounds (n_vars = %llu)",
                                (unsigned long long)g, (unsigned long long)G);
        if (rank[g] != 0xffffffffu) return fail(ctx, SRX_E_ARG, "selected feature index %llu appears twice", (unsigned long long)g);
        rank[g] = (uint32_t)s;
    }
    uint32_t* d_rank;
    SRX_TRY(sel_buffers(ctx, G, k, out, &d_rank));
    SRX_TRY(h2d(ctx, d_rank, rank.data(), G * sizeof(uint32_t)));
    return launch_sel_finish(m, d_rank, nullptr, vectors, center, scale, out);
}

int32_t hvg_list_host(srx_mat* m, uint64_t n, std::vector<uint64_t>& out) {
    std::vector<double> var;
    if (m->csc) {
        var.resize(m->n_rows);
        SRX_TRY(row_stat(m, 1, var.data(), nullptr));
    } else {
        SRX_TRY(gene_variances(m, var));
    }
    return select_hvg_host(m->ctx, var, n, out);
}

}

using namespace srx;

extern "C" {

int32_t srx_select_hvg(srx_mat* m, uint64_t n, uint64_t* idx_out, uint64_t* n_out) {
    if (!m || !n_out) return fail(m ? m->ctx : nullptr, SRX_E_ARG, "null argument");
    SRX_HIP(m->ctx, hipSetDevice(m->ctx->device));
    std::vector<uint64_t> sel;
    SRX_TRY(hvg_list_host(m, n, sel));
    if (idx_out) memcpy(idx_out, sel.data(), sel.size() * sizeof(uint64_t));
    *n_out = sel.size();
    return SRX_OK;
}

}
```

Baseline: 133.3 million.

## Fuse moments unpack, gene variance, poison clearing, chained scan, and row-order histogram reuse

```diff
diff --git a/include/srx.h b/include/srx.h
--- a/include/srx.h
+++ b/include/srx.h
@@ -90,6 +90,7 @@
 int32_t srx_matrix_copy_values(srx_mat* dst, const srx_mat* src);
 void    srx_matrix_free(srx_mat* m);
 
+int32_t srx_gene_moments_transformed(srx_mat* m, double target_sum, uint64_t* cnt, double* sum, double* sumsq, double* nz_var);
 int32_t srx_compute_number(srx_mat* m, int32_t direction, uint32_t* out);
 int32_t srx_compute_sum(srx_mat* m, int32_t direction, double* out);
 int32_t srx_compute_variance(srx_mat* m, int32_t direction, double* out);
@@ -204,6 +205,10 @@
 
 int32_t srx_spmm(srx_mat* m, const uint64_t* sel, uint64_t k, const double* panel, double* y_out,
                  double* t_out, double* gram_out);
+
+int32_t srx_scan_counts(srx_ctx* ctx, const int64_t* counts, uint64_t n, uint32_t rblk, uint32_t spin_limit, int64_t* ptr_out,
+                        int64_t* rec_base_out);
+int32_t srx_row_order_last(srx_ctx* ctx, uint64_t n_rows, uint32_t* hist_out, uint32_t* perm_out);
 
 typedef struct srx_pipeline_result {
     srx_pca_info pca;
diff --git a/rust/srx_sys.rs b/rust/srx_sys.rs
--- a/rust/srx_sys.rs
+++ b/rust/srx_sys.rs
@@ -207,6 +207,8 @@
     pub fn srx_matrix_clone(m: *mut SrxMat, out: *mut *mut SrxMat) -> i32;
     pub fn srx_matrix_copy_values(dst: *mut SrxMat, src: *const SrxMat) -> i32;
     pub fn srx_matrix_free(m: *mut SrxMat);
+    pub fn srx_gene_moments_transformed(m: *mut SrxMat, target_sum: f64, cnt: *mut u64, sum: *mut f64,
+                                        sumsq: *mut f64, nz_var: *mut f64) -> i32;
     pub fn srx_compute_number(m: *mut SrxMat, direction: i32, out: *mut u32) -> i32;
     pub fn srx_compute_sum(m: *mut SrxMat, direction: i32, out: *mut f64) -> i32;
     pub fn srx_compute_variance(m: *mut SrxMat, direction: i32, out: *mut f64) -> i32;
@@ -252,6 +254,9 @@
     pub fn srx_graph_free(g: *mut SrxGraph);
     pub fn srx_spmm(m: *mut SrxMat, sel: *const u64, k: u64, panel: *const f64, y_out: *mut f64, t_out: *mut f64,
                     gram_out: *mut f64) -> i32;
+    pub fn srx_scan_counts(ctx: *mut SrxCtx, counts: *const i64, n: u64, rblk: u32, spin_limit: u32,
+                           ptr_out: *mut i64, rec_base_out: *mut i64) -> i32;
+    pub fn srx_row_order_last(ctx: *mut SrxCtx, n_rows: u64, hist_out: *mut u32, perm_out: *mut u32) -> i32;
     pub fn srx_pipeline(m: *mut SrxMat, target_sum: f64, n_hvg: u64, opts: *const SrxPcaOpts,
                         res: *mut SrxPipelineResult) -> i32;
     pub fn srx_result_fetch(m: *mut SrxMat, scores: *mut f64, components: *mut f64, evr: *mut f64, mean: *mut f64,
diff --git a/singlerust_amd/_ffi.py b/singlerust_amd/_ffi.py
--- a/singlerust_amd/_ffi.py
+++ b/singlerust_amd/_ffi.py
@@ -153,6 +153,9 @@
     "srx_graph_fetch_scales": (C.c_int32, [P, P, P]),
     "srx_graph_free": (None, [P]),
     "srx_spmm": (C.c_int32, [P, P, C.c_uint64, P, P, P, P]),
+    "srx_scan_counts": (C.c_int32, [P, P, C.c_uint64, C.c_uint32, C.c_uint32, P, P]),
+    "srx_row_order_last": (C.c_int32, [P, C.c_uint64, P, P]),
+    "srx_gene_moments_transformed": (C.c_int32, [P, C.c_double, P, P, P, P]),
     "srx_pipeline": (C.c_int32, [P, C.c_double, C.c_uint64, C.POINTER(PcaOpts), C.POINTER(PipelineResult)]),
     "srx_result_fetch": (C.c_int32, [P, P, P, P, P, P, P]),
     "srx_backed_create": (C.c_int32, [P, C.c_uint64, C.c_int32, C.POINTER(P)]),
diff --git a/singlerust_amd/csrc/common.hpp b/singlerust_amd/csrc/common.hpp
--- a/singlerust_amd/csrc/common.hpp
+++ b/singlerust_amd/csrc/common.hpp
@@ -105,6 +105,12 @@
     hipEvent_t d2h_ev = nullptr;
     void* pin_d2h = nullptr;
     bool d2h_pending = false;
+    uint64_t poison_clean_words = 0;
+    const srx_mat* gene_var_of = nullptr;
+    uint64_t gene_var_version = 0;
+    uint32_t scan_epoch = 0;
+    uint32_t len_turn = 0;
+    const uint32_t* len_hist_last = nullptr;
 };
 
 struct srx_pca_state {
@@ -220,6 +226,8 @@
 int32_t ensure_tiles(srx_mat* m);
 int32_t promote_to_f64(srx_mat* m);
 int32_t ensure_pattern_counts(srx_mat* m);
+int32_t poison_buffer(srx_ctx* ctx, uint64_t G, uint32_t** out, bool* clean);
+int32_t gene_var_buffer(srx_ctx* ctx, uint64_t G, double** out);
 int32_t ensure_moments(srx_mat* m);
 int32_t moments_accumulate(srx_mat* m, double* d_acc, RowXf xf);
 int32_t moments_install(srx_mat* m, double* d_packed);
diff --git a/singlerust_amd/csrc/ctx.hip b/singlerust_amd/csrc/ctx.hip
--- a/singlerust_amd/csrc/ctx.hip
+++ b/singlerust_amd/csrc/ctx.hip
@@ -291,6 +291,7 @@
 
 static void free_mat_buffers(srx_mat* m) {
     if (!m) return;
+    if (m->ctx && m->ctx->gene_var_of == m) m->ctx->gene_var_of = nullptr;
     dev_release(m, m->d_indptr);
     dev_release(m, m->d_indices);
     dev_release(m, m->d_values);
diff --git a/singlerust_amd/csrc/genes.hip b/singlerust_amd/csrc/genes.hip
--- a/singlerust_amd/csrc/genes.hip
+++ b/singlerust_amd/csrc/genes.hip
@@ -353,11 +353,12 @@
 __global__ __launch_bounds__(64 * kRedSlices) void k_moments_reduce(
     const double* __restrict__ part_sum, const double* __restrict__ part_sq, uint64_t n_cols, uint64_t n_blocks, uint64_t n_rows,
     const uint32_t* __restrict__ cnt, double inv_fx_sum, double inv_fx_sq, const uint32_t* __restrict__ poison,
-    double* __restrict__ packed) {
+    double* __restrict__ packed, uint64_t* __restrict__ cnt_out = nullptr, double* __restrict__ sum_out = nullptr,
+    double* __restrict__ sq_out = nullptr, double* __restrict__ var_out = nullptr) {
     __shared__ unsigned long long red[2][kRedSlices][64];
     const int lane = threadIdx.x & 63, slice = threadIdx.x >> 6;
     const uint64_t j = (uint64_t)blockIdx.x * 64 + lane;
-    if (blockIdx.x == 0 && threadIdx.x == 0) packed[3 * n_cols] = (double)n_rows;
+    if (packed && blockIdx.x == 0 && threadIdx.x == 0) packed[3 * n_cols] = (double)n_rows;
     const bool live = j < n_cols;
     double s = 0.0, q = 0.0;
     if (inv_fx_sum != 0.0) {
@@ -403,9 +404,23 @@
             q += part_sq[b * n_cols + j];
         }
     }
-    packed[j] = (double)cnt[j];
-    packed[n_cols + j] = s;
-    packed[2 * n_cols + j] = q;
+    if (packed) {
+        packed[j] = (double)cnt[j];
+        packed[n_cols + j] = s;
+        packed[2 * n_cols + j] = q;
+        return;
+    }
+    const uint32_t c32 = cnt[j];
+    cnt_out[j] = (uint64_t)c32;
+    sum_out[j] = s;
+    sq_out[j] = q;
+    double v = 0.0;
+    if (c32 > 0) {
+        const double c = (double)c32;
+        const double mean = __ddiv_rn(s, c);
+        v = __dsub_rn(__ddiv_rn(q, c), __dmul_rn(mean, mean));
+    }
+    var_out[j] = v;
 }
 
 __global__ void k_moments_unpack(const double* __restrict__ packed, uint64_t n_cols, uint64_t* __restrict__ cnt,
@@ -664,7 +679,28 @@
     return m->d_idx16 ? f((const uint16_t*)m->d_idx16) : f((const int32_t*)m->d_indices);
 }
 
-static int32_t local_moments(srx_mat* m, double** packed_out, RowXf xf = RowXf{}) {
+int32_t poison_buffer(srx_ctx* ctx, uint64_t G, uint32_t** out, bool* clean) {
+    const size_t had = ctx->scratch["mom_poison"].bytes;
+    SRX_TRY(scratch(ctx, "mom_poison", at_least_one(G) * sizeof(uint32_t), (void**)out));
+    if (ctx->scratch["mom_poison"].bytes != had) ctx->poison_clean_words = 0;
+    if (clean) *clean = ctx->poison_clean_words >= at_least_one(G);
+    return SRX_OK;
+}
+int32_t gene_var_buffer(srx_ctx* ctx, uint64_t G, double** out) {
+    return scratch(ctx, "hvg_var", at_least_one(G) * sizeof(double), (void**)out);
+}
+static bool single_rank(const srx_ctx* ctx) { return ctx->n_ranks <= 1 && !ctx->comm && !ctx->host_allreduce; }
+static void gene_var_book(srx_mat* m, bool fresh) {
+    srx_ctx* ctx = m->ctx;
+    if (fresh) {
+        ctx->gene_var_of = m;
+        ctx->gene_var_version = m->version;
+    } else if (ctx->gene_var_of == m) {
+        ctx->gene_var_of = nullptr;
+    }
+}
+
+static int32_t local_moments(srx_mat* m, double** packed_out, RowXf xf = RowXf{}, bool direct = false) {
     srx_ctx* ctx = m->ctx;
     SRX_TRY(ensure_tiles(m));
     const uint64_t G = m->n_cols;
@@ -688,9 +724,13 @@
     }
     uint32_t* d_poison = nullptr;
     if (xf.row_sum) {
-        SRX_TRY(scratch(ctx, "mom_poison", at_least_one(G) * sizeof(uint32_t), (void**)&d_poison));
-        SRX_HIP(ctx, hipMemsetAsync(d_poison, 0, at_least_one(G) * sizeof(uint32_t), ctx->stream));
-    }
+        bool clean = false;
+        SRX_TRY(poison_buffer(ctx, G, &d_poison, &clean));
+        if (!clean) SRX_HIP(ctx, hipMemsetAsync(d_poison, 0, at_least_one(G) * sizeof(uint32_t), ctx->stream));
+        ctx->poison_clean_words = 0;
+    }
+    double* d_var = nullptr;
+    if (direct) SRX_TRY(gene_var_buffer(ctx, G, &d_var));
     {
         ProfScope ps(ctx, SRX_K_MOMENTS, bytes);
         dim3 grid((unsigned)(nb * m->n_tiles));
@@ -711,10 +751,12 @@
         }));
         hipLaunchKernelGGL(k_moments_reduce, dim3((unsigned)at_least_one((G + 63) / 64)), dim3(64 * kRedSlices), 0, ctx->stream, p_sum, p_sq, G, nb,
                            m->n_rows, (const uint32_t*)m->d_cnt_pat, fx_sum != 0.0 ? 1.0 / fx_sum : 0.0,
-                           fx_sq != 0.0 ? 1.0 / fx_sq : 0.0, (const uint32_t*)d_poison, packed);
+                           fx_sq != 0.0 ? 1.0 / fx_sq : 0.0, (const uint32_t*)d_poison, direct ? (double*)nullptr : packed,
+                           direct ? m->d_cnt : (uint64_t*)nullptr, direct ? m->d_sum : (double*)nullptr,
+                           direct ? m->d_sq : (double*)nullptr, d_var);
     }
     SRX_HIP(ctx, hipGetLastError());
-    *packed_out = packed;
+    *packed_out = direct ? nullptr : packed;
     return SRX_OK;
 }
 
@@ -778,6 +820,7 @@
 static int32_t reduce_unpack_moments(srx_mat* m, double* d_packed, bool n_is_local) {
     srx_ctx* ctx = m->ctx;
     const uint64_t G = m->n_cols;
+    gene_var_book(m, false);
     SRX_TRY(allreduce_f64(ctx, d_packed, 3 * G + 1));
     hipLaunchKernelGGL(k_moments_unpack, dim3((unsigned)((G + 255) / 256 + 1)), dim3(256), 0, ctx->stream, d_packed, G,
                        m->d_cnt, m->d_sum, m->d_sq);
@@ -806,9 +849,12 @@
     if (m->moments_version == m->version) return SRX_OK;
     SRX_TRY(alloc_moments(m));
     double* packed;
-    SRX_TRY(local_moments(m, &packed));
-    SRX_TRY(reduce_unpack_moments(m, packed, true));
+    const bool direct = single_rank(m->ctx);
+    SRX_TRY(local_moments(m, &packed, RowXf{}, direct));
+    if (direct) m->n_rows_global = m->n_rows;
+    else SRX_TRY(reduce_unpack_moments(m, packed, true));
     moments_adopt(m);
+    gene_var_book(m, direct);
     return SRX_OK;
 }
 
@@ -816,13 +862,17 @@
     *stored = false;
     SRX_TRY(alloc_moments(m));
     double* packed;
-    SRX_TRY(local_moments(m, &packed, xf));
+    const bool direct = single_rank(m->ctx);
+    SRX_TRY(local_moments(m, &packed, xf, direct));
     if (xf.write_back) {
         m->dtype = SRX_F64;
         touch(m);
         *stored = true;
     }
-    return reduce_unpack_moments(m, packed, true);
+    if (!direct) return reduce_unpack_moments(m, packed, true);
+    m->n_rows_global = m->n_rows;
+    gene_var_book(m, true);
+    return SRX_OK;
 }
 
 static int32_t fetch_moments(srx_mat* m, uint64_t* cnt, double* sum, double* sq) {
@@ -866,6 +916,27 @@
     if (!m) return fail(nullptr, SRX_E_ARG, "null matrix");
     if (m->csc) return fail(m->ctx, SRX_E_FORMAT, "srx_gene_moments walks cells: convert the CSC matrix with srx_matrix_to_csr");
     return fetch_moments(m, cnt, sum, sumsq);
+}
+
+int32_t srx_gene_moments_transformed(srx_mat* m, double target_sum, uint64_t* cnt, double* sum, double* sumsq, double* nz_var) {
+    if (!m) return fail(nullptr, SRX_E_ARG, "null matrix");
+    srx_ctx* ctx = m->ctx;
+    if (m->csc) return fail(ctx, SRX_E_FORMAT, "srx_gene_moments_transformed walks cells: convert the CSC matrix with srx_matrix_to_csr");
+    if (!single_rank(ctx)) return fail(ctx, SRX_E_ARG, "srx_gene_moments_transformed: a single-rank context only");
+    SRX_HIP(ctx, hipSetDevice(ctx->device));
+    SRX_TRY(launch_row_sums(m));
+    bool stored = false;
+    SRX_TRY(ensure_moments_xf(m, RowXf{m->d_row_sum, target_sum, false}, &stored));
+    const uint64_t G = m->n_cols;
+    double* d_var;
+    SRX_TRY(gene_var_buffer(ctx, G, &d_var));
+    gene_var_book(m, false);
+    moments_retire(m);
+    if (cnt) SRX_TRY(d2h(ctx, cnt, m->d_cnt, G * sizeof(uint64_t)));
+    if (sum) SRX_TRY(d2h(ctx, sum, m->d_sum, G * sizeof(double)));
+    if (sumsq) SRX_TRY(d2h(ctx, sumsq, m->d_sq, G * sizeof(double)));
+    if (nz_var) SRX_TRY(d2h(ctx, nz_var, d_var, G * sizeof(double)));
+    return SRX_OK;
 }
 
 int32_t srx_compute_number(srx_mat* m, int32_t direction, uint32_t* out) {
diff --git a/singlerust_amd/csrc/pca_form.hip b/singlerust_amd/csrc/pca_form.hip
--- a/singlerust_amd/csrc/pca_form.hip
+++ b/singlerust_amd/csrc/pca_form.hip
@@ -65,19 +65,30 @@
     return (int)(want < cap ? want : cap);
 }
 
-int32_t scan_exclusive(srx_ctx* ctx, const int64_t* d_in, uint64_t n, int64_t* d_out, int64_t** total_dev) {
+int32_t scan_exclusive_recs(srx_ctx* ctx, const int64_t* d_in, uint64_t n, int64_t* d_out, int64_t** total_dev, uint32_t rblk,
+                            uint64_t n_rblk, int64_t* rec_base, uint32_t spin_limit = kScanSpinLimit) {
     const uint64_t per_block = (uint64_t)kScanBlock * kScanItems;
     const uint64_t nb = (n + per_block - 1) / per_block > 0 ? (n + per_block - 1) / per_block : 1;
-    int64_t* d_bsum;
-    SRX_TRY(scratch(ctx, "scan_bsum", (nb + 1) * sizeof(int64_t), (void**)&d_bsum));
-    int64_t* d_total = d_bsum + nb;
-    hipLaunchKernelGGL(k_scan_block_sums, dim3((unsigned)nb), dim3(kScanBlock), 0, ctx->stream, d_in, n, d_bsum);
-    hipLaunchKernelGGL(k_scan_serial, dim3(1), dim3(kScanBlock), 0, ctx->stream, d_bsum, nb, d_total);
-    hipLaunchKernelGGL(k_scan_apply, dim3((unsigned)nb), dim3(kScanBlock), 0, ctx->stream, d_in, n, d_bsum, d_total,
-                       d_out);
+    if (rec_base && (rblk == 0 || rblk % (kWave * kScanItems) != 0 || per_block % rblk != 0))
+        return fail(ctx, SRX_E_ARG, "scan: row blocks of %u rows do not tile the scan's workgroups", rblk);
+    unsigned long long* d_state;
+    const size_t had = ctx->scratch["scan_state"].bytes;
+    SRX_TRY(scratch(ctx, "scan_state", (2 * nb + 1) * sizeof(unsigned long long), (void**)&d_state));
+    if (ctx->scratch["scan_state"].bytes != had || ctx->scan_epoch + 1 >= kScanEpochs) {
+        SRX_HIP(ctx, hipMemsetAsync(d_state, 0, ctx->scratch["scan_state"].bytes, ctx->stream));
+        ctx->scan_epoch = 0;
+    }
+    const uint32_t epoch = ++ctx->scan_epoch;
+    int64_t* d_total;
+    SRX_TRY(scratch(ctx, "scan_total", sizeof(int64_t), (void**)&d_total));
+    hipLaunchKernelGGL(k_scan_chained, dim3((unsigned)nb), dim3(kScanBlock), 0, ctx->stream, d_in, n, d_out, d_total, d_state, epoch,
+                       spin_limit, rblk, n_rblk, rec_base);
     SRX_HIP(ctx, hipGetLastError());
     if (total_dev) *total_dev = d_total;
     return SRX_OK;
+}
+int32_t scan_exclusive(srx_ctx* ctx, const int64_t* d_in, uint64_t n, int64_t* d_out, int64_t** total_dev) {
+    return scan_exclusive_recs(ctx, d_in, n, d_out, total_dev, 0, 0, nullptr);
 }
 
 int32_t retile(srx_mat* m, const RowMajor& rm, Tiled& t) {
@@ -128,15 +139,17 @@
     const bool list = m->n_cols <= 65536 && m->d_idx16 && k < 0xffff + 1;
     ProfScope ps(ctx, SRX_K_COMPACT, (double)m->nnz * s_i * (list ? 1.0 : 2.0) + (double)(N + 1) * 8.0 * 2.0);
     uint32_t* kept = nullptr;
+    uint32_t* len_set[2];
+    SRX_TRY(len_sets(ctx, &len_set[0], &len_set[1]));
     if (list) {
         SRX_TRY(scratch(ctx, "pca_keptlist", (m->nnz + 64) * sizeof(uint32_t), (void**)&kept));
         const size_t col_lds = ((size_t)n_words * 32 + 1) * sizeof(uint16_t);
-        const int per_cu = std::max(1, std::min(2, (int)(160 * 1024 / (col_lds + 1024))));
+        const int per_cu = std::max(1, std::min(2, (int)(160 * 1024 / (col_lds + 1024 + kLenBins * sizeof(uint32_t)))));
         const uint64_t visits = (N + (uint64_t)kCompactRows * (kCountThreads / kWave) - 1) / ((uint64_t)kCompactRows * (kCountThreads / kWave));
         const unsigned cgrid = (unsigned)std::max<uint64_t>(1, std::min<uint64_t>(visits, (uint64_t)ctx->n_cus * per_cu));
         SRX_HIP(ctx, hipFuncSetAttribute((const void*)k_rowcount_list, hipFuncAttributeMaxDynamicSharedMemorySize, (int)col_lds));
         hipLaunchKernelGGL(k_rowcount_list, dim3(cgrid), dim3(kCountThreads), col_lds, ctx->stream, m->d_indptr,
-                           (const uint16_t*)m->d_idx16, d_sel, d_sel + n_words, n_words, N, m->nnz, k, cntrow, kept);
+                           (const uint16_t*)m->d_idx16, d_sel, d_sel + n_words, n_words, N, m->nnz, k, cntrow, kept, len_set[0]);
     } else {
         auto count = [&](auto kern, const auto* idxp, size_t lds) {
             hipLaunchKernelGGL(kern, dim3(grid_rows(ctx, N, 4)), dim3(256), lds, ctx->stream, m->d_indptr, idxp, d_sel, n_words, N, cntrow);
@@ -150,27 +163,24 @@
             else count(k_rowcount<int32_t, false>, (const int32_t*)m->d_indices, 0);
         }
     }
-    SRX_TRY(scan_exclusive(ctx, cntrow, N, rm.ptr, &d_total));
     int64_t* d_nrecs = nullptr;
     rm.n_recs = -1;
     if (want_recs && N > 0) {
         GramPlan g;
         SRX_TRY(gram_plan(ctx, k, N, g));
-        int64_t *blk_total, *rec_base;
-        SRX_TRY(scratch(ctx, "pca_brtot", g.n_rblk * sizeof(int64_t), (void**)&blk_total));
+        int64_t* rec_base;
         SRX_TRY(scratch(ctx, "pca_brbase", (g.n_rblk + 4) * sizeof(int64_t), (void**)&rec_base));
-        hipLaunchKernelGGL(k_rec_count, dim3((unsigned)g.n_rblk), dim3(256), 0, ctx->stream, (const int64_t*)rm.ptr, N, g.rblk, blk_total);
-        hipLaunchKernelGGL(k_rec_scan, dim3(1), dim3(1024), 0, ctx->stream, (const int64_t*)blk_total, g.n_rblk, rec_base,
-                           (const int64_t*)d_total);
-        SRX_HIP(ctx, hipGetLastError());
+        SRX_TRY(scan_exclusive_recs(ctx, cntrow, N, rm.ptr, &d_total, g.rblk, g.n_rblk, rec_base));
         d_nrecs = rec_base + g.n_rblk;
+    } else {
+        SRX_TRY(scan_exclusive(ctx, cntrow, N, rm.ptr, &d_total));
     }
     int64_t total = 0;
     {
         int64_t both[2] = {0, 0};
         SRX_TRY(d2h_begin(ctx, d_nrecs ? (const void*)d_nrecs : (const void*)d_total, d_nrecs ? sizeof both : sizeof(int64_t)));
         rm.n_rows = N;
-        SRX_TRY(build_row_order(ctx, rm));
+        SRX_TRY(build_row_order(ctx, rm, len_set, list));
         SRX_TRY(d2h_end(ctx, both, d_nrecs ? sizeof both : sizeof(int64_t)));
         if (d_nrecs) {
             rm.n_recs = both[0];
@@ -354,6 +364,35 @@
 
 }
 
+extern "C" int32_t srx_scan_counts(srx_ctx* ctx, const int64_t* counts, uint64_t n, uint32_t rblk, uint32_t spin_limit, int64_t* ptr_out,
+                                   int64_t* rec_base_out) {
+    using namespace srx;
+    if (!ctx || (!counts && n) || !ptr_out || (rec_base_out && rblk == 0)) return fail(ctx, SRX_E_ARG, "srx_scan_counts: bad arguments");
+    SRX_HIP(ctx, hipSetDevice(ctx->device));
+    const uint64_t n_rblk = rec_base_out ? (n + rblk - 1) / rblk : 0;
+    int64_t *d_in, *d_out, *d_rec = nullptr, *d_total;
+    SRX_TRY(scratch(ctx, "scan_api_in", at_least_one(n) * sizeof(int64_t), (void**)&d_in));
+    SRX_TRY(scratch(ctx, "scan_api_out", (n + 1) * sizeof(int64_t), (void**)&d_out));
+    if (rec_base_out) SRX_TRY(scratch(ctx, "scan_api_rec", (n_rblk + 4) * sizeof(int64_t), (void**)&d_rec));
+    if (n) SRX_TRY(h2d(ctx, d_in, counts, n * sizeof(int64_t)));
+    SRX_TRY(scan_exclusive_recs(ctx, d_in, n, d_out, &d_total, rblk, n_rblk, d_rec, spin_limit));
+    SRX_TRY(d2h(ctx, ptr_out, d_out, (n + 1) * sizeof(int64_t)));
+    if (rec_base_out) SRX_TRY(d2h(ctx, rec_base_out, d_rec, (n_rblk + 2) * sizeof(int64_t)));
+    return SRX_OK;
+}
+
+extern "C" int32_t srx_row_order_last(srx_ctx* ctx, uint64_t n_rows, uint32_t* hist_out, uint32_t* perm_out) {
+    using namespace srx;
+    if (!ctx) return fail(ctx, SRX_E_ARG, "srx_row_order_last: null context");
+    SRX_HIP(ctx, hipSetDevice(ctx->device));
+    auto it = ctx->scratch.find("pca_rm_perm");
+    if (!ctx->len_hist_last || it == ctx->scratch.end() || it->second.bytes < n_rows * sizeof(uint32_t))
+        return fail(ctx, SRX_E_ARG, "srx_row_order_last: no row order of %llu rows on this context", (unsigned long long)n_rows);
+    if (hist_out) SRX_TRY(d2h(ctx, hist_out, ctx->len_hist_last, kLenBins * sizeof(uint32_t)));
+    if (perm_out && n_rows) SRX_TRY(d2h(ctx, perm_out, it->second.p, n_rows * sizeof(uint32_t)));
+    return SRX_OK;
+}
+
 extern "C" int32_t srx_gram_mode_info(srx_ctx* ctx, int32_t* mode_out) {
     using namespace srx;
     if (!ctx || !mode_out) return fail(ctx, SRX_E_ARG, "srx_gram_mode_info: null argument");
diff --git a/singlerust_amd/csrc/pca_internal.hpp b/singlerust_amd/csrc/pca_internal.hpp
--- a/singlerust_amd/csrc/pca_internal.hpp
+++ b/singlerust_amd/csrc/pca_internal.hpp
@@ -155,7 +155,9 @@
 int32_t launch_gram(srx_ctx* ctx, const RowMajor& rm, double* Gp, bool* reduce = nullptr, bool zero_first = false);
 inline size_t gram_packed_count(int k) { return (size_t)k * (size_t)(k + 1) / 2; }
 
-int32_t build_row_order(srx_ctx* ctx, RowMajor& r);
+constexpr int kLenBins = 512;
+int32_t len_sets(srx_ctx* ctx, uint32_t** mine, uint32_t** other);
+int32_t build_row_order(srx_ctx* ctx, RowMajor& r, uint32_t* const* sets = nullptr, bool hist_made = false);
 int scores_ld(int n_pc);
 void result_layout(uint64_t n_rows, int k, int n_pc, int dim, size_t& score_bytes, size_t& small_doubles,
                    std::vector<int>* plan_a_out = nullptr, std::vector<int>* plan_b_out = nullptr);
diff --git a/singlerust_amd/csrc/pca_solve.hip b/singlerust_amd/csrc/pca_solve.hip
--- a/singlerust_amd/csrc/pca_solve.hip
+++ b/singlerust_amd/csrc/pca_solve.hip
@@ -85,16 +85,32 @@
     return SRX_OK;
 }
 
-int32_t build_row_order(srx_ctx* ctx, RowMajor& r) {
-    uint32_t* hist;
-    SRX_TRY(scratch(ctx, "pca_rm_lenhist", kLenBins * sizeof(uint32_t), (void**)&hist));
+int32_t len_sets(srx_ctx* ctx, uint32_t** mine, uint32_t** other) {
+    uint32_t* p;
+    const size_t had = ctx->scratch["pca_rm_lenhist"].bytes;
+    SRX_TRY(scratch(ctx, "pca_rm_lenhist", 4 * kLenBins * sizeof(uint32_t), (void**)&p));
+    if (ctx->scratch["pca_rm_lenhist"].bytes != had) SRX_HIP(ctx, hipMemsetAsync(p, 0, 4 * kLenBins * sizeof(uint32_t), ctx->stream));
+    const uint32_t turn = ctx->len_turn++ & 1u;
+    *mine = p + turn * 2 * kLenBins;
+    *other = p + (turn ^ 1u) * 2 * kLenBins;
+    return SRX_OK;
+}
+
+int32_t build_row_order(srx_ctx* ctx, RowMajor& r, uint32_t* const* sets, bool hist_made) {
+    uint32_t *mine, *other;
+    if (sets) {
+        mine = sets[0];
+        other = sets[1];
+    } else {
+        SRX_TRY(len_sets(ctx, &mine, &other));
+        hist_made = false;
+    }
     SRX_TRY(scratch(ctx, "pca_rm_perm", (r.n_rows ? r.n_rows : 1) * sizeof(uint32_t), (void**)&r.perm));
-    SRX_HIP(ctx, hipMemsetAsync(hist, 0, kLenBins * sizeof(uint32_t), ctx->stream));
     const unsigned g = (unsigned)((r.n_rows + kLenRowsPerWg - 1) / kLenRowsPerWg + (r.n_rows ? 0 : 1));
-    hipLaunchKernelGGL(k_len_hist, dim3(g), dim3(256), 0, ctx->stream, r.ptr, r.n_rows, hist);
-    hipLaunchKernelGGL(k_len_scan, dim3(1), dim3(kLenBins), 0, ctx->stream, hist);
-    hipLaunchKernelGGL(k_len_scatter, dim3(g), dim3(256), 0, ctx->stream, r.ptr, r.n_rows, hist, r.perm);
+    if (!hist_made) hipLaunchKernelGGL(k_len_hist, dim3(g), dim3(256), 0, ctx->stream, r.ptr, r.n_rows, mine);
+    hipLaunchKernelGGL(k_len_order, dim3(g), dim3(256), 0, ctx->stream, r.ptr, r.n_rows, (const uint32_t*)mine, mine + kLenBins, other, r.perm);
     SRX_HIP(ctx, hipGetLastError());
+    ctx->len_hist_last = mine;
     return SRX_OK;
 }
 
diff --git a/singlerust_amd/csrc/rows.hip b/singlerust_amd/csrc/rows.hip
--- a/singlerust_amd/csrc/rows.hip
+++ b/singlerust_amd/csrc/rows.hip
@@ -102,10 +102,13 @@
 
 template <typename T>
 __global__ __launch_bounds__(256) void k_row_sum(const int64_t* __restrict__ indptr, const T* __restrict__ vals,
-                                                 uint64_t n_rows, double* __restrict__ out) {
-    const uint64_t wave = global_wave_id();
-    const uint64_t n_waves = ((uint64_t)gridDim.x * blockDim.x) / kWave;
-    const int lane = lane_id();
+                                                 uint64_t n_rows, double* __restrict__ out, uint32_t* __restrict__ zero = nullptr,
+                                                 uint64_t n_zero = 0) {
+    const uint64_t wave = global_wave_id();
+    const uint64_t n_waves = ((uint64_t)gridDim.x * blockDim.x) / kWave;
+    const int lane = lane_id();
+    if (zero)
+        for (uint64_t i = (uint64_t)blockIdx.x * blockDim.x + threadIdx.x; i < n_zero; i += (uint64_t)gridDim.x * blockDim.x) zero[i] = 0u;
     for (uint64_t r = wave; r < n_rows; r += n_waves) {
         const int64_t lo = indptr[r], hi = indptr[r + 1];
         double s = 0.0;
@@ -357,14 +360,18 @@
     if (!out && !m->d_row_sum) SRX_HIP(ctx, dev_malloc(ctx, (void**)&m->d_row_sum, (m->n_rows ? m->n_rows : 1) * sizeof(double)));
     double* const dst = out ? out : m->d_row_sum;
     const int g = row_grid(m);
+    uint32_t* d_poison = nullptr;
+    const uint64_t n_poison = out ? 0 : at_least_one(m->n_cols);
+    if (!out) SRX_TRY(poison_buffer(ctx, m->n_cols, &d_poison, nullptr));
     ProfScope ps(ctx, SRX_K_ROWSUM, (double)m->nnz * val_bytes(m) + (double)(m->n_rows + 1) * 8.0 + (double)m->n_rows * 8.0);
     if (is_f32(m))
         hipLaunchKernelGGL((k_row_sum<float>), dim3(g), dim3(256), 0, ctx->stream, m->d_indptr, (const float*)m->d_values,
-                           m->n_rows, dst);
+                           m->n_rows, dst, d_poison, n_poison);
     else
         hipLaunchKernelGGL((k_row_sum<double>), dim3(g), dim3(256), 0, ctx->stream, m->d_indptr, (const double*)m->d_values,
-                           m->n_rows, dst);
-    SRX_HIP(ctx, hipGetLastError());
+                           m->n_rows, dst, d_poison, n_poison);
+    SRX_HIP(ctx, hipGetLastError());
+    if (!out) ctx->poison_clean_words = n_poison;
     return SRX_OK;
 }
 
diff --git a/singlerust_amd/csrc/select.hip b/singlerust_amd/csrc/select.hip
--- a/singlerust_amd/csrc/select.hip
+++ b/singlerust_amd/csrc/select.hip
@@ -121,10 +121,8 @@
             uint32_t at = 0;
             if (lane == 0 && m) at = atomicAdd(&s_cnt, (uint32_t)__popcll(m));
             at = __shfl(at, 0, 64);
-            if (in) {
-                cand[at + (uint32_t)__popcll(m & ((1ull << lane) - 1ull))] = j;
-                rank_out[j] = 0u;
-            }
+            if (in) cand[at + (uint32_t)__popcll(m & ((1ull << lane) - 1ull))] = j;
+            if (j < G) rank_out[j] = in ? 0u : 0xffffffffu;
         }
     }
     __syncthreads();
@@ -312,13 +310,17 @@
     const uint64_t take = n < G ? n : G;
     double* d_var;
     uint32_t* d_rank;
-    SRX_TRY(scratch(ctx, "hvg_var", at_least_one(G) * sizeof(double), (void**)&d_var));
+    SRX_TRY(gene_var_buffer(ctx, G, &d_var));
     SRX_TRY(sel_buffers(ctx, G, take, out, &d_rank));
+    const bool have_var = ctx->gene_var_of == m && ctx->gene_var_version == m->version && m->moments_version == m->version;
     const unsigned gb = (unsigned)at_least_one((G + 255) / 256);
     const unsigned gy = (unsigned)at_least_one((G + kRankTile - 1) / kRankTile);
     static const bool full_rank = getenv("SRX_HVG_FULL_RANK") != nullptr;
     const bool all = full_rank || take == 0 || G < (uint64_t)kRankSample;
-    hipLaunchKernelGGL(k_gene_var, dim3(gb), dim3(256), 0, ctx->stream, m->d_cnt, m->d_sum, m->d_sq, G, d_var, d_rank, all ? 0u : 0xffffffffu);
+    if (all || !have_var) {
+        hipLaunchKernelGGL(k_gene_var, dim3(gb), dim3(256), 0, ctx->stream, m->d_cnt, m->d_sum, m->d_sq, G, d_var, d_rank, all ? 0u : 0xffffffffu);
+        if (!have_var) ctx->gene_var_of = nullptr;
+    }
     if (all) {
         hipLaunchKernelGGL(k_hvg_rank, dim3(gb, gy), dim3(256), 0, ctx->stream, d_var, (uint32_t)G, d_rank);
     } else {
```

Result: no change. 133.8 million, median of 6 (+0.4%).
